# wns349/tensorflow-yolo

Measured on AMD Instinct MI355X. Metric: images/sec at 1/2/4/8 MI355X + post-NMS box-set match vs CPU ref, higher is better.
Workload: dtype f16; 1 GPU; v3-608-b32-fp16; network=v3, batch_per_gpu=32, global_batch=32, weights=seeded synthetic Darknet stream (random-init), streams=1

## Files before the change

include/yolo_hip.h:

```cpp
#ifndef YOLO_HIP_H
#define YOLO_HIP_H

#include <stddef.h>
#include <stdint.h>

#ifdef __cplusplus
extern "C" {
#endif

#define YOLO_HIP_ABI_VERSION 7

enum yolo_status {
    YOLO_OK = 0,
    YOLO_ERR_ARG = 1,
    YOLO_ERR_PLAN = 2,
    YOLO_ERR_HIP = 3,
    YOLO_ERR_WEIGHTS = 4,
    YOLO_ERR_STATE = 5,
    YOLO_ERR_OVERFLOW = 6
};

enum yolo_op {
    YOLO_OP_INPUT = 0,
    YOLO_OP_CONV = 1,
    YOLO_OP_MAXPOOL = 2,
    YOLO_OP_ROUTE = 3,
    YOLO_OP_REORG = 4,
    YOLO_OP_SHORTCUT = 5,
    YOLO_OP_UPSAMPLE = 6,
    YOLO_OP_YOLO = 7,
    YOLO_OP_DETECTION = 8
};

enum yolo_dtype { YOLO_DTYPE_F32 = 0, YOLO_DTYPE_F16 = 1, YOLO_DTYPE_MXF8 = 2 };

enum yolo_nms_mode {
    YOLO_NMS_AGNOSTIC = 0,
    YOLO_NMS_PER_CLASS = 1
};

#define YOLO_MAX_SRC 4
#define YOLO_MAX_ANCHORS 8
#define YOLO_MAX_SCALES 4

typedef struct yolo_layer_desc {
    int32_t op;
    int32_t n_src;
    int32_t src[YOLO_MAX_SRC];
    int32_t filters, ksize, stride;
    int32_t batch_norm;
    int32_t leaky;
    int32_t h, w, c;
    int32_t n_anchors;
    double anchors[2 * YOLO_MAX_ANCHORS];
} yolo_layer_desc;

typedef struct yolo_net_options {
    int32_t dtype;
    int32_t max_batch;
    int32_t keep_all;
    int32_t cand_capacity;
    int32_t max_boxes;
    int32_t streams;
    int32_t force_tile;
    int32_t guard_bytes;
    int32_t f32_products;
} yolo_net_options;

typedef struct yolo_box {
    float x, y, w, h;
    float prob;
    int32_t class_idx;
} yolo_box;

typedef struct yolo_head_desc {
    int32_t version;
    int32_t n_classes;
    int32_t n_scales;
    int32_t h[YOLO_MAX_SCALES], w[YOLO_MAX_SCALES], n_anchors[YOLO_MAX_SCALES];
    double anchors[YOLO_MAX_SCALES][2 * YOLO_MAX_ANCHORS];
} yolo_head_desc;

typedef struct yolo_net yolo_net;

int yolo_hip_abi_version(void);
const char *yolo_last_error(void);

int yolo_net_create(const yolo_layer_desc *layers, int n_layers, const yolo_net_options *opt, yolo_net **out);
void yolo_net_destroy(yolo_net *net);

size_t yolo_net_weight_count(const yolo_net *net);
size_t yolo_net_weights_bytes(const yolo_net *net);
size_t yolo_net_workspace_bytes(const yolo_net *net);
size_t yolo_net_output_count(const yolo_net *net);
double yolo_net_flops_per_image(const yolo_net *net);
int yolo_net_head_desc(const yolo_net *net, yolo_head_desc *out);
int yolo_net_set_head(yolo_net *net, const yolo_head_desc *head);
int yolo_net_num_kernels(const yolo_net *net);
int yolo_net_num_streams(const yolo_net *net);
int yolo_net_tune_streams(yolo_net *net, const float *in_dev, int batch, void *stream);
int yolo_net_set_streams(yolo_net *net, int parts);
typedef struct yolo_ws_region {
    char name[32];
    uint64_t offset, used_bytes, region_bytes;
} yolo_ws_region;
int yolo_net_workspace_regions(const yolo_net *net, yolo_ws_region *out, int cap);
size_t yolo_net_describe(const yolo_net *net, char *buf, size_t cap);

int yolo_net_load_weights(yolo_net *net, const float *host_weights, size_t n, void *dev_weights, size_t dev_bytes);
int yolo_net_bind_workspace(yolo_net *net, void *dev_workspace, size_t dev_bytes);

int yolo_net_forward(yolo_net *net, const float *in_dev, int batch, float *out_dev, void *stream);

int yolo_net_forward_u8(yolo_net *net, const uint8_t *in_dev, int batch, float *out_dev, void *stream);
int yolo_net_tune_streams_u8(yolo_net *net, const uint8_t *in_dev, int batch, void *stream);
int yolo_u8_unit_table(float *out256);

struct yolo_launch_caps {
    int32_t tap_stream_workgroups, stem_workgroups, first_mfma_workgroups, aux_work_items, decode_rows;
};
int yolo_launch_caps(struct yolo_launch_caps *out);

int yolo_net_autotune(yolo_net *net, const float *in_dev, int batch, void *stream);

int yolo_net_detect(yolo_net *net, const float *in_dev, int batch, double threshold, double iou_threshold,
                    int nms_mode, yolo_box *boxes_dev, int32_t *counts_dev, int32_t *status_dev, void *stream);

int yolo_net_detect_u8(yolo_net *net, const uint8_t *in_dev, int batch, double threshold, double iou_threshold,
                       int nms_mode, yolo_box *boxes_dev, int32_t *counts_dev, int32_t *status_dev, void *stream);

typedef struct yolo_kernel_info {
    int32_t kind;
    int32_t layer;
    int32_t variant;
    int32_t ksize, stride, cin, cout, out_h, out_w;
    double flops;
    double bytes;
    double weight_bytes;
    char name[64];
    char symbol[160];
} yolo_kernel_info;
int yolo_net_kernel_info(const yolo_net *net, int kernel, yolo_kernel_info *out);

int yolo_net_forward_timed(yolo_net *net, const float *in_dev, int batch, float *out_dev, void *stream, float *ms_host);

int yolo_net_forward_timed_u8(yolo_net *net, const uint8_t *in_dev, int batch, float *out_dev, void *stream, float *ms_host);

int yolo_net_read_layer(yolo_net *net, int layer, int batch, float *host_out, size_t n);

int yolo_mx_quantize(const void *src_f16_dev, int rows, int channels, uint8_t *q_dev, uint8_t *scale_dev, void *stream);
int yolo_mx_quantize_host(const float *src, int rows, int channels, uint8_t *q, uint8_t *scale);

size_t yolo_decode_scratch_bytes(const yolo_head_desc *head, int batch, int cand_capacity);
int yolo_decode_nms(const yolo_head_desc *head, const float *logits_dev, int batch, double threshold,
                    double iou_threshold, int nms_mode, int cand_capacity, int max_boxes, void *scratch_dev,
                    size_t scratch_bytes, yolo_box *boxes_dev, int32_t *counts_dev, int32_t *status_dev,
                    void *stream);

int yolo_preprocess_resize(const uint8_t *src_dev, int src_h, int src_w, int src_row_bytes, float *dst_dev, int dst_h, int dst_w,
                           int swap_rb, void *stream);

int yolo_preprocess_resize_u8(const uint8_t *src_dev, int src_h, int src_w, int src_row_bytes, uint8_t *dst_dev, int dst_h, int dst_w,
                              int swap_rb, void *stream);

typedef struct yolo_frame {
    const uint8_t *pixels_dev;
    int32_t h, w, row_bytes, swap_rb;
} yolo_frame;

enum yolo_resize_mode {
    YOLO_RESIZE_STRETCH = 0,
    YOLO_RESIZE_LETTERBOX = 1
};

int yolo_letterbox_geometry(int src_h, int src_w, int dst_h, int dst_w, int mode, int32_t *new_h, int32_t *new_w, int32_t *off_y,
                            int32_t *off_x);

int yolo_preprocess_frames_u8(const yolo_frame *frames_host, int n, int mode, uint8_t *dst_dev, int dst_h, int dst_w, void *stream);
int yolo_preprocess_frames(const yolo_frame *frames_host, int n, int mode, float *dst_dev, int dst_h, int dst_w, void *stream);

int yolo_boxes_to_frames(yolo_box *boxes_dev, const int32_t *counts_dev, int batch, int max_boxes, const yolo_frame *frames_host, int mode,
                         int net_h, int net_w, void *stream);

int yolo_net_detect_frames_u8(yolo_net *net, const yolo_frame *frames_host, int batch, int mode, uint8_t *batch_dev, double threshold,
                              double iou_threshold, int nms_mode, yolo_box *boxes_dev, int32_t *counts_dev, int32_t *status_dev,
                              void *stream);

typedef struct yolo_gt {
    float x, y, w, h;
    int32_t class_idx;
    int32_t difficult;
} yolo_gt;

enum yolo_eval_verdict { YOLO_EVAL_FP = 0, YOLO_EVAL_TP = 1, YOLO_EVAL_IGNORED = 2 };

enum yolo_eval_status {
    YOLO_EVAL_OVERFLOW = 1,
    YOLO_EVAL_UNSORTED = 2,
    YOLO_EVAL_BAD_CLASS = 4,
    YOLO_EVAL_BAD_COUNT = 8
};

#define YOLO_EVAL_MAX_GT 1024
#define YOLO_EVAL_MAX_DET_CAPACITY (1 << 20)
#define YOLO_EVAL_MAX_CLASSES 65536

typedef struct yolo_eval_desc {
    int32_t n_classes;
    int32_t det_capacity;
    int32_t max_gt;
    int32_t pad_;
    double match_iou;
} yolo_eval_desc;

typedef struct yolo_eval_record {
    double best_iou;
    float prob;
    int32_t class_idx;
    uint32_t seq;
    int32_t verdict;
    int32_t best_gt;
    int32_t pad_;
} yolo_eval_record;

typedef struct yolo_eval_class {
    double ap_voc12, ap_voc07;
    int32_t n_gt, n_det, tp, fp, ignored, pad_;
} yolo_eval_class;

typedef struct yolo_eval_result {
    double map_voc12, map_voc07;
    int32_t n_records;
    int32_t status;
    int32_t n_classes, pad_;
} yolo_eval_result;

typedef struct yolo_eval_layout {
    uint64_t status_offset, n_gt_offset, records_offset, sorted_offset, ctp_offset, cfp_offset, total_bytes;
} yolo_eval_layout;

size_t yolo_eval_state_bytes(const yolo_eval_desc *desc);
size_t yolo_eval_result_bytes(const yolo_eval_desc *desc);
int yolo_eval_state_layout(const yolo_eval_desc *desc, yolo_eval_layout *out);
int yolo_eval_reset(const yolo_eval_desc *desc, void *state_dev, size_t state_bytes, void *stream);
int yolo_eval_add(const yolo_eval_desc *desc, void *state_dev, const yolo_box *boxes_dev, const int32_t *counts_dev, int batch, int max_boxes,
                  const yolo_gt *gt_dev, const int32_t *gt_counts_dev, int64_t image_base, void *stream);
int yolo_eval_finish(const yolo_eval_desc *desc, void *state_dev, void *result_dev, void *stream);

enum yolo_loss_status {
    YOLO_LOSS_OUT_OF_GRID = 1,
    YOLO_LOSS_BAD_BOX = 2,
    YOLO_LOSS_BAD_CLASS = 4,
    YOLO_LOSS_BAD_COUNT = 8
};

#define YOLO_LOSS_MAX_CELLS 4096

typedef struct yolo_loss_image {
    double xy, wh, obj, noobj, cls;
    int32_t n_assigned;
    int32_t n_truths;
    int32_t status;
    int32_t pad_;
} yolo_loss_image;

typedef struct yolo_loss_result {
    double loss, loss_xy, loss_wh, loss_obj, loss_noobj, loss_class;
    int32_t n_assigned, n_truths;
    int32_t status;
    int32_t pad_;
} yolo_loss_result;

int yolo_v2_loss(const yolo_head_desc *head, const float *logits_dev, int batch, const yolo_gt *gt_dev, const int32_t *gt_counts_dev,
                 int max_gt, yolo_loss_image *images_dev, int32_t *assign_dev, yolo_loss_result *result_dev, void *stream);
// ... 248 lines not shown
```

tensorflow-yolo_amd/_hip.py:

```python
import ctypes as C
import os

_HERE = os.path.dirname(os.path.abspath(__file__))
LIB_PATH = os.environ.get("YOLO_HIP_LIB") or os.path.join(_HERE, "libyolo_hip.so")

ABI_VERSION = 7

OP_INPUT, OP_CONV, OP_MAXPOOL, OP_ROUTE, OP_REORG, OP_SHORTCUT, OP_UPSAMPLE, OP_YOLO, OP_DETECTION = range(9)
DTYPE_F32, DTYPE_F16, DTYPE_MXF8 = 0, 1, 2
NMS_AGNOSTIC, NMS_PER_CLASS = 0, 1
RESIZE_STRETCH, RESIZE_LETTERBOX = 0, 1
RESIZE_MODES = {"stretch": RESIZE_STRETCH, "letterbox": RESIZE_LETTERBOX}
EVAL_FP, EVAL_TP, EVAL_IGNORED = 0, 1, 2
EVAL_OVERFLOW, EVAL_UNSORTED, EVAL_BAD_CLASS, EVAL_BAD_COUNT = 1, 2, 4, 8
EVAL_MAX_GT, EVAL_MAX_DET_CAPACITY, EVAL_MAX_CLASSES = 1024, 1 << 20, 65536
LOSS_OUT_OF_GRID, LOSS_BAD_BOX, LOSS_BAD_CLASS, LOSS_BAD_COUNT = 1, 2, 4, 8
LOSS_MAX_CELLS = 4096
ANCHOR_EUCLIDEAN, ANCHOR_IOU = 0, 1
ANCHOR_DISTANCES = {"euclidean": ANCHOR_EUCLIDEAN, "iou": ANCHOR_IOU}
ANCHOR_BAD_BOX, ANCHOR_EMPTY_CLUSTER, ANCHOR_DEGENERATE, ANCHOR_MAX_ITER = 1, 2, 4, 8
ANCHOR_MAX_K, ANCHOR_MAX_INIT, ANCHOR_MAX_N, ANCHOR_ITER_LIMIT = 32, 64, 1 << 22, 10000
FRAMES_PER_LAUNCH = 64
MAX_SRC, MAX_ANCHORS, MAX_SCALES = 4, 8, 4
DEFAULT_MAX_BOXES = 1024
# ... 63 lines not shown
class LossResult(C.Structure):
    _fields_ = [("loss", C.c_double), ("loss_xy", C.c_double), ("loss_wh", C.c_double), ("loss_obj", C.c_double), ("loss_noobj", C.c_double),
                ("loss_class", C.c_double), ("n_assigned", C.c_int32), ("n_truths", C.c_int32), ("status", C.c_int32), ("pad_", C.c_int32)]


class LaunchCaps(C.Structure):
    _fields_ = [("tap_stream_workgroups", C.c_int32), ("stem_workgroups", C.c_int32), ("first_mfma_workgroups", C.c_int32),
                ("aux_work_items", C.c_int32), ("decode_rows", C.c_int32)]


class WgradPlan(C.Structure):
    _fields_ = [("tile_cout", C.c_int32), ("tile_cin", C.c_int32), ("tile_positions", C.c_int32), ("tiles_cout", C.c_int32),
                ("tiles_cin", C.c_int32), ("positions_per_chunk", C.c_int32), ("n_chunks", C.c_int32), ("pad_", C.c_int32),
                ("scratch_bytes", C.c_uint64)]


class Conv3x3WgradPlan(C.Structure):
    _fields_ = [("tile_cout", C.c_int32), ("tile_cin", C.c_int32), ("tile_positions", C.c_int32), ("tiles_cout", C.c_int32),
                ("tiles_cin", C.c_int32), ("positions_per_chunk", C.c_int32), ("n_chunks", C.c_int32), ("halo_rows", C.c_int32),
                ("scratch_bytes", C.c_uint64)]


class Conv3x3WgradF16Plan(C.Structure):
    _fields_ = [("tile_cout", C.c_int32), ("tile_cin", C.c_int32), ("tile_positions", C.c_int32), ("tiles_cout", C.c_int32),
                ("tiles_cin", C.c_int32), ("positions_per_chunk", C.c_int32), ("n_chunks", C.c_int32), ("halo_rows", C.c_int32),
                ("db_groups", C.c_int32), ("db_positions", C.c_int32), ("record_offset", C.c_uint64), ("scratch_bytes", C.c_uint64)]


class TensorView(C.Structure):
    _fields_ = [("offset", C.c_uint64), ("image_stride", C.c_int64), ("ld", C.c_int32), ("coff", C.c_int32), ("dtype", C.c_int32),
                ("cin", C.c_int32), ("h", C.c_int32), ("w", C.c_int32)]


class HeadTrainLayout(C.Structure):
    _fields_ = [(n, C.c_uint64) for n in ("w_offset", "b_offset", "m_w_offset", "v_w_offset", "m_b_offset", "v_b_offset", "dw_offset",
                                          "db_offset", "grad_offset", "assign_offset", "images_offset", "scratch_offset", "scratch_bytes",
                                          "total_bytes")] + [("cin", C.c_int32), ("cout", C.c_int32)]


class TailTrainLayout(C.Structure):
    _fields_ = [(n, C.c_uint64) for n in ("w_offset", "b_offset", "m_w_offset", "v_w_offset", "m_b_offset", "v_b_offset", "dw_offset",
                                          "db_offset", "w3_offset", "beta_offset", "m_w3_offset", "v_w3_offset", "m_beta_offset",
                                          "v_beta_offset", "dw3_offset", "dbeta_offset", "scale64_offset", "scale32_offset", "mean_offset",
                                          "d_offset", "grad_offset", "assign_offset", "images_offset", "scratch_offset", "scratch_bytes",
                                          "total_bytes", "block_src", "head_src")] + [(n, C.c_int32) for n in ("cin", "cout", "cin3", "cout3")]


class HeadTrainV3Layout(C.Structure):
    _fields_ = ([("n_scales", C.c_int32), ("pad_", C.c_int32), ("cin", C.c_int32 * MAX_SCALES), ("cout", C.c_int32 * MAX_SCALES)] +
                [(n, C.c_uint64 * MAX_SCALES) for n in ("w_offset", "b_offset", "m_w_offset", "v_w_offset", "m_b_offset", "v_b_offset",
                                                        "dw_offset", "db_offset", "bias_src")] +
                [(n, C.c_uint64) for n in ("grad_offset", "assign_offset", "parts_offset", "images_offset", "scratch_offset",
                                           "scratch_bytes", "total_bytes")])


class BlocksTrainV3Layout(C.Structure):
    _fields_ = ([("n_scales", C.c_int32), ("pad_", C.c_int32)] + [(n, C.c_int32 * MAX_SCALES) for n in ("cin", "cout", "cin3", "cout3")] +
                [(n, C.c_uint64 * MAX_SCALES) for n in ("w_offset", "b_offset", "m_w_offset", "v_w_offset", "m_b_offset", "v_b_offset",
                                                        "dw_offset", "db_offset", "w3_offset", "beta_offset", "m_w3_offset", "v_w3_offset",
                                                        "m_beta_offset", "v_beta_offset", "dw3_offset", "dbeta_offset", "scale64_offset",
                                                        "scale32_offset", "mean_offset", "bias_src", "block_src")] +
                [(n, C.c_uint64) for n in ("d_offset", "grad_offset", "assign_offset", "parts_offset", "images_offset", "scratch_offset",
                                           "scratch_bytes", "total_bytes")])


class V3WgradPlan(C.Structure):
    _fields_ = ([(n, C.c_int32) for n in ("n_scales", "threads", "channels_per_thread", "min_chunk", "win_tile_cin", "win_tile_rows", "reduce_tile_chunks", "pad_")] +
                [(n, C.c_int32 * MAX_SCALES) for n in ("positions", "positions_per_chunk", "n_chunks", "threads_per_chunk", "obj_workgroups",
                                                       "win_workgroups")] +
                [(n, C.c_uint64 * MAX_SCALES) for n in ("slab_offset", "slab_bytes")] +
                [(n, C.c_uint64) for n in ("slot_offset", "slot_bytes", "scratch_bytes")])


class V3WgradView(C.Structure):
    _fields_ = [("x_dev", C.c_void_p), ("image_stride", C.c_int64), ("ld", C.c_int32), ("coff", C.c_int32), ("dtype", C.c_int32),
                ("cin", C.c_int32)]


class V3DgradPlan(C.Structure):
    _fields_ = [(n, C.c_int32) for n in ("threads", "channels_per_thread", "tile_cin", "tiles_cin", "threads_per_position",
                                         "positions_per_round", "rounds", "positions_per_workgroup", "workgroups", "loops", "positions",
                                         "lds_bytes")]


class AugmentImage(C.Structure):
    _fields_ = [("enabled", C.c_int32), ("flip_lr", C.c_int32), ("flip_ud", C.c_int32), ("radius", C.c_int32), ("taps", C.c_uint16 * 10),
                ("drop_thr", C.c_uint32), ("noise_q", C.c_int32 * 2), ("noise_loc", C.c_int32 * 2), ("tx", C.c_int32), ("key", C.c_uint32 * 2)]


class AnchorDesc(C.Structure):
    _fields_ = [("k", C.c_int32), ("n_init", C.c_int32), ("max_iter", C.c_int32), ("distance", C.c_int32), ("tolerate", C.c_double),
                ("seed", C.c_uint64)]


class AnchorPlan(C.Structure):
    _fields_ = [(n, C.c_int32) for n in ("chunk", "n_chunks", "period", "threads")] + \
               [(n, C.c_uint64) for n in ("prep_offset", "pick_offset", "state_offset", "q_offset", "label_offset", "label_stride",
                                          "sums_offset", "scratch_bytes", "header_offset", "restarts_offset", "best_offset", "result_bytes")]


class AnchorHeader(C.Structure):
    _fields_ = [("status", C.c_uint32)] + [(n, C.c_int32) for n in ("best_restart", "n_valid", "n_bad", "k", "n_init", "distance", "pad_")]


class AnchorRestart(C.Structure):
    _fields_ = [("n_iter", C.c_int32), ("status", C.c_uint32), ("inertia_q", C.c_uint64), ("iou_q", C.c_uint64),
                ("seeds", C.c_int32 * ANCHOR_MAX_K)]


class AnchorBest(C.Structure):
    _fields_ = [("centres", (C.c_double * 2) * ANCHOR_MAX_K), ("counts", C.c_int64 * ANCHOR_MAX_K), ("sum_q", (C.c_uint64 * 2) * ANCHOR_MAX_K),
                ("inertia_q", C.c_uint64), ("iou_q", C.c_uint64), ("inertia", C.c_double), ("avg_iou", C.c_double)]


class WsRegion(C.Structure):
    _fields_ = [("name", C.c_char * 32), ("offset", C.c_uint64), ("used_bytes", C.c_uint64), ("region_bytes", C.c_uint64)]


class KernelInfo(C.Structure):
    _fields_ = [("kind", C.c_int32), ("layer", C.c_int32), ("variant", C.c_int32), ("ksize", C.c_int32),
                ("stride", C.c_int32), ("cin", C.c_int32), ("cout", C.c_int32), ("out_h", C.c_int32), ("out_w", C.c_int32),
                ("flops", C.c_double), ("bytes", C.c_double), ("weight_bytes", C.c_double), ("name", C.c_char * 64),
                ("symbol", C.c_char * 160)]


SIGNATURES = {
    "yolo_hip_abi_version": (C.c_int, []),
    "yolo_last_error": (C.c_char_p, []),
    "yolo_net_create": (C.c_int, [C.POINTER(LayerDesc), C.c_int, C.POINTER(NetOptions), C.POINTER(C.c_void_p)]),
    "yolo_net_destroy": (None, [C.c_void_p]),
    "yolo_net_weight_count": (C.c_size_t, [C.c_void_p]),
    "yolo_net_weights_bytes": (C.c_size_t, [C.c_void_p]),
    "yolo_net_workspace_bytes": (C.c_size_t, [C.c_void_p]),
    "yolo_net_output_count": (C.c_size_t, [C.c_void_p]),
    "yolo_net_flops_per_image": (C.c_double, [C.c_void_p]),
    "yolo_net_head_desc": (C.c_int, [C.c_void_p, C.POINTER(HeadDesc)]),
    "yolo_net_set_head": (C.c_int, [C.c_void_p, C.POINTER(HeadDesc)]),
    "yolo_net_num_kernels": (C.c_int, [C.c_void_p]),
    "yolo_net_num_streams": (C.c_int, [C.c_void_p]),
    "yolo_net_describe": (C.c_size_t, [C.c_void_p, C.c_char_p, C.c_size_t]),
    "yolo_net_load_weights": (C.c_int, [C.c_void_p, C.c_void_p, C.c_size_t, C.c_void_p, C.c_size_t]),
    "yolo_net_bind_workspace": (C.c_int, [C.c_void_p, C.c_void_p, C.c_size_t]),
    "yolo_net_forward": (C.c_int, [C.c_void_p, C.c_void_p, C.c_int, C.c_void_p, C.c_void_p]),
    "yolo_net_detect": (C.c_int, [C.c_void_p, C.c_void_p, C.c_int, C.c_double, C.c_double, C.c_int,
                                  C.c_void_p, C.c_void_p, C.c_void_p, C.c_void_p]),
    "yolo_net_forward_u8": (C.c_int, [C.c_void_p, C.c_void_p, C.c_int, C.c_void_p, C.c_void_p]),
    "yolo_net_detect_u8": (C.c_int, [C.c_void_p, C.c_void_p, C.c_int, C.c_double, C.c_double, C.c_int,
                                     C.c_void_p, C.c_void_p, C.c_void_p, C.c_void_p]),
    "yolo_net_forward_timed_u8": (C.c_int, [C.c_void_p, C.c_void_p, C.c_int, C.c_void_p, C.c_void_p, C.c_void_p]),
    "yolo_net_tune_streams_u8": (C.c_int, [C.c_void_p, C.c_void_p, C.c_int, C.c_void_p]),
    "yolo_preprocess_resize_u8": (C.c_int, [C.c_void_p, C.c_int, C.c_int, C.c_int, C.c_void_p, C.c_int, C.c_int, C.c_int, C.c_void_p]),
    "yolo_u8_unit_table": (C.c_int, [C.c_void_p]),
    "yolo_launch_caps": (C.c_int, [C.POINTER(LaunchCaps)]),
    "yolo_net_autotune": (C.c_int, [C.c_void_p, C.c_void_p, C.c_int, C.c_void_p]),
    "yolo_net_tune_streams": (C.c_int, [C.c_void_p, C.c_void_p, C.c_int, C.c_void_p]),
    "yolo_net_set_streams": (C.c_int, [C.c_void_p, C.c_int]),
    "yolo_net_workspace_regions": (C.c_int, [C.c_void_p, C.POINTER(WsRegion), C.c_int]),
    "yolo_net_kernel_info": (C.c_int, [C.c_void_p, C.c_int, C.POINTER(KernelInfo)]),
    "yolo_net_forward_timed": (C.c_int, [C.c_void_p, C.c_void_p, C.c_int, C.c_void_p, C.c_void_p, C.c_void_p]),
    "yolo_net_read_layer": (C.c_int, [C.c_void_p, C.c_int, C.c_int, C.c_void_p, C.c_size_t]),
    "yolo_mx_quantize": (C.c_int, [C.c_void_p, C.c_int, C.c_int, C.c_void_p, C.c_void_p, C.c_void_p]),
    "yolo_mx_quantize_host": (C.c_int, [C.c_void_p, C.c_int, C.c_int, C.c_void_p, C.c_void_p]),
    "yolo_decode_scratch_bytes": (C.c_size_t, [C.POINTER(HeadDesc), C.c_int, C.c_int]),
    "yolo_decode_nms": (C.c_int, [C.POINTER(HeadDesc), C.c_void_p, C.c_int, C.c_double, C.c_double, C.c_int,
                                  C.c_int, C.c_int, C.c_void_p, C.c_size_t, C.c_void_p, C.c_void_p, C.c_void_p,
                                  C.c_void_p]),
    "yolo_preprocess_resize": (C.c_int, [C.c_void_p, C.c_int, C.c_int, C.c_int, C.c_void_p, C.c_int, C.c_int, C.c_int, C.c_void_p]),
    "yolo_letterbox_geometry": (C.c_int, [C.c_int, C.c_int, C.c_int, C.c_int, C.c_int, C.POINTER(C.c_int32), C.POINTER(C.c_int32),
                                          C.POINTER(C.c_int32), C.POINTER(C.c_int32)]),
    "yolo_preprocess_frames_u8": (C.c_int, [C.POINTER(Frame), C.c_int, C.c_int, C.c_void_p, C.c_int, C.c_int, C.c_void_p]),
    "yolo_preprocess_frames": (C.c_int, [C.POINTER(Frame), C.c_int, C.c_int, C.c_void_p, C.c_int, C.c_int, C.c_void_p]),
    "yolo_boxes_to_frames": (C.c_int, [C.c_void_p, C.c_void_p, C.c_int, C.c_int, C.POINTER(Frame), C.c_int, C.c_int, C.c_int, C.c_void_p]),
    "yolo_net_detect_frames_u8": (C.c_int, [C.c_void_p, C.POINTER(Frame), C.c_int, C.c_int, C.c_void_p, C.c_double, C.c_double, C.c_int,
                                            C.c_void_p, C.c_void_p, C.c_void_p, C.c_void_p]),
    "yolo_eval_state_bytes": (C.c_size_t, [C.POINTER(EvalDesc)]),
    "yolo_eval_result_bytes": (C.c_size_t, [C.POINTER(EvalDesc)]),
    "yolo_eval_state_layout": (C.c_int, [C.POINTER(EvalDesc), C.POINTER(EvalLayout)]),
    "yolo_eval_reset": (C.c_int, [C.POINTER(EvalDesc), C.c_void_p, C.c_size_t, C.c_void_p]),
    "yolo_eval_add": (C.c_int, [C.POINTER(EvalDesc), C.c_void_p, C.c_void_p, C.c_void_p, C.c_int, C.c_int, C.c_void_p, C.c_void_p,
                                C.c_int64, C.c_void_p]),
    "yolo_eval_finish": (C.c_int, [C.POINTER(EvalDesc), C.c_void_p, C.c_void_p, C.c_void_p]),
    "yolo_v2_loss": (C.c_int, [C.POINTER(HeadDesc), C.c_void_p, C.c_int, C.c_void_p, C.c_void_p, C.c_int, C.c_void_p, C.c_void_p, C.c_void_p,
                               C.c_void_p]),
    "yolo_net_loss": (C.c_int, [C.c_void_p, C.c_void_p, C.c_int, C.c_void_p, C.c_void_p, C.c_int, C.c_void_p, C.c_void_p, C.c_void_p,
                                C.c_void_p]),
    "yolo_net_loss_u8": (C.c_int, [C.c_void_p, C.c_void_p, C.c_int, C.c_void_p, C.c_void_p, C.c_int, C.c_void_p, C.c_void_p, C.c_void_p,
                                   C.c_void_p]),
    "yolo_loss_reduce": (C.c_int, [C.c_void_p, C.c_int, C.c_int, C.c_int, C.c_void_p, C.c_void_p]),
    "yolo_v2_loss_grad": (C.c_int, [C.POINTER(HeadDesc), C.c_void_p, C.c_int, C.c_void_p, C.c_void_p, C.c_int, C.c_void_p, C.c_void_p, C.c_void_p,
                                    C.c_void_p, C.c_void_p]),
    "yolo_v3_loss_rows": (C.c_int, [C.POINTER(HeadDesc), C.POINTER(C.c_int64), C.POINTER(C.c_int32)]),
    "yolo_v3_loss": (C.c_int, [C.POINTER(HeadDesc), C.c_void_p, C.c_int, C.c_void_p, C.c_void_p, C.c_int, C.c_double, C.c_void_p, C.c_void_p,
                               C.c_void_p, C.c_void_p, C.c_void_p]),
    "yolo_v3_loss_grad": (C.c_int, [C.POINTER(HeadDesc), C.c_void_p, C.c_int, C.c_void_p, C.c_void_p, C.c_int, C.c_double, C.c_void_p, C.c_void_p,
                                    C.c_void_p, C.c_void_p, C.c_void_p, C.c_void_p]),
    "yolo_net_loss_v3": (C.c_int, [C.c_void_p, C.c_void_p, C.c_int, C.c_void_p, C.c_void_p, C.c_int, C.c_double, C.c_void_p, C.c_void_p,
                                   C.c_void_p, C.c_void_p, C.c_void_p]),
    "yolo_net_loss_v3_u8": (C.c_int, [C.c_void_p, C.c_void_p, C.c_int, C.c_void_p, C.c_void_p, C.c_int, C.c_double, C.c_void_p, C.c_void_p,
                                      C.c_void_p, C.c_void_p, C.c_void_p]),
    "yolo_wgrad_plan": (C.c_int, [C.c_int64, C.c_int, C.c_int, C.c_int, C.POINTER(WgradPlan)]),
    "yolo_conv1x1_wgrad": (C.c_int, [C.c_void_p, C.c_int, C.c_int, C.c_int, C.c_int64, C.c_int, C.c_int, C.c_int, C.c_void_p, C.c_int,
                                     C.c_void_p, C.c_void_p, C.c_void_p, C.c_size_t, C.c_void_p]),
    "yolo_adam_step": (C.c_int, [C.c_void_p] * 8 + [C.c_int64, C.c_int64, C.c_float, C.c_float, C.c_float, C.c_float, C.c_void_p]),
    "yolo_net_head_input": (C.c_int, [C.c_void_p, C.POINTER(TensorView)]),
    "yolo_net_head_train_layout": (C.c_int, [C.c_void_p, C.POINTER(HeadTrainLayout)]),
    "yolo_net_head_train_bytes": (C.c_size_t, [C.c_void_p]),
    "yolo_net_head_train_init": (C.c_int, [C.c_void_p, C.c_void_p, C.c_size_t, C.c_void_p, C.c_void_p]),
    "yolo_net_head_train_read": (C.c_int, [C.c_void_p, C.c_void_p, C.c_void_p, C.c_void_p]),
    "yolo_net_train_head_step": (C.c_int, [C.c_void_p, C.c_void_p, C.c_int, C.c_void_p, C.c_void_p, C.c_int, C.c_void_p, C.c_float,
                                           C.c_void_p, C.c_void_p]),
    "yolo_net_train_head_step_u8": (C.c_int, [C.c_void_p, C.c_void_p, C.c_int, C.c_void_p, C.c_void_p, C.c_int, C.c_void_p, C.c_float,
                                              C.c_void_p, C.c_void_p]),
    "yolo_v3_head_wgrad_plan": (C.c_int, [C.POINTER(HeadDesc), C.POINTER(C.c_int32), C.c_int, C.c_int, C.POINTER(V3WgradPlan)]),
    "yolo_v3_head_wgrad": (C.c_int, [C.POINTER(HeadDesc), C.POINTER(V3WgradView), C.c_int, C.c_void_p, C.c_void_p, C.c_int,
                                     C.POINTER(C.c_void_p), C.POINTER(C.c_void_p), C.c_void_p, C.c_size_t, C.c_void_p]),
    "yolo_net_head_inputs_v3": (C.c_int, [C.c_void_p, C.POINTER(TensorView), C.POINTER(C.c_int32)]),
    "yolo_net_head_train_v3_layout": (C.c_int, [C.c_void_p, C.POINTER(HeadTrainV3Layout)]),
    "yolo_net_head_train_v3_bytes": (C.c_size_t, [C.c_void_p]),
    "yolo_net_head_train_v3_init": (C.c_int, [C.c_void_p, C.c_void_p, C.c_size_t, C.POINTER(C.c_void_p), C.POINTER(C.c_void_p)]),
    "yolo_net_head_train_v3_read": (C.c_int, [C.c_void_p, C.c_void_p, C.POINTER(C.c_void_p), C.POINTER(C.c_void_p)]),
    "yolo_net_train_head_step_v3": (C.c_int, [C.c_void_p, C.c_void_p, C.c_int, C.c_void_p, C.c_void_p, C.c_int, C.c_double, C.c_void_p,
                                              C.c_float, C.c_void_p, C.c_void_p]),
    "yolo_net_train_head_step_v3_u8": (C.c_int, [C.c_void_p, C.c_void_p, C.c_int, C.c_void_p, C.c_void_p, C.c_int, C.c_double, C.c_void_p,
                                                 C.c_float, C.c_void_p, C.c_void_p]),
    "yolo_conv1x1_dgrad": (C.c_int, [C.c_void_p, C.c_int, C.c_void_p, C.c_int, C.c_void_p, C.c_int, C.c_int, C.c_int, C.c_int64, C.c_int,
                                     C.c_int, C.c_float, C.c_void_p, C.c_void_p]),
    "yolo_conv3x3_wgrad_plan": (C.c_int, [C.c_int, C.c_int, C.c_int, C.c_int, C.c_int, C.c_int, C.POINTER(Conv3x3WgradPlan)]),
    "yolo_conv3x3_wgrad": (C.c_int, [C.c_void_p, C.c_int, C.c_int, C.c_int, C.c_int64, C.c_int, C.c_int, C.c_int, C.c_int, C.c_void_p,
                                     C.c_int, C.c_void_p, C.c_void_p, C.c_void_p, C.c_void_p, C.c_size_t, C.c_void_p]),
    "yolo_conv3x3_wgrad_f16_plan": (C.c_int, [C.c_int, C.c_int, C.c_int, C.c_int, C.c_int, C.POINTER(Conv3x3WgradF16Plan)]),
    "yolo_conv3x3_wgrad_f16": (C.c_int, [C.c_void_p, C.c_int, C.c_int, C.c_int, C.c_int64, C.c_int, C.c_int, C.c_int, C.c_int, C.c_void_p,
                                         C.c_int, C.c_void_p, C.c_void_p, C.c_void_p, C.c_void_p, C.c_size_t, C.c_void_p]),
    "yolo_net_train_wgrad_f16_bytes": (C.c_size_t, [C.c_void_p]),
    "yolo_net_train_set_wgrad_f16": (C.c_int, [C.c_void_p, C.c_void_p, C.c_size_t]),
    "yolo_net_tail_inputs": (C.c_int, [C.c_void_p, C.POINTER(TensorView), C.POINTER(TensorView)]),
    "yolo_net_tail_train_layout": (C.c_int, [C.c_void_p, C.POINTER(TailTrainLayout)]),
    "yolo_net_tail_train_bytes": (C.c_size_t, [C.c_void_p]),
    "yolo_net_tail_train_init": (C.c_int, [C.c_void_p, C.c_void_p, C.c_size_t, C.c_void_p, C.c_void_p, C.c_void_p]),
    "yolo_net_tail_train_read": (C.c_int, [C.c_void_p, C.c_void_p, C.c_void_p, C.c_void_p, C.c_void_p, C.c_void_p]),
    "yolo_net_train_tail_step": (C.c_int, [C.c_void_p, C.c_void_p, C.c_int, C.c_void_p, C.c_void_p, C.c_int, C.c_void_p, C.c_float,
                                           C.c_void_p, C.c_void_p]),
    "yolo_net_train_tail_step_u8": (C.c_int, [C.c_void_p, C.c_void_p, C.c_int, C.c_void_p, C.c_void_p, C.c_int, C.c_void_p, C.c_float,
                                              C.c_void_p, C.c_void_p]),
    "yolo_v3_head_dgrad_plan": (C.c_int, [C.POINTER(HeadDesc), C.c_int, C.c_int, C.c_int, C.POINTER(V3DgradPlan)]),
    "yolo_v3_head_dgrad": (C.c_int, [C.POINTER(HeadDesc), C.c_int, C.c_void_p, C.c_void_p, C.c_int, C.c_int, C.c_void_p, C.c_int, C.c_void_p,
                                     C.c_int, C.c_int, C.c_int, C.c_int64, C.c_float, C.c_void_p, C.c_void_p]),
    "yolo_net_block_inputs_v3": (C.c_int, [C.c_void_p, C.POINTER(TensorView), C.POINTER(TensorView), C.POINTER(C.c_int32)]),
    "yolo_net_blocks_train_v3_layout": (C.c_int, [C.c_void_p, C.POINTER(BlocksTrainV3Layout)]),
    "yolo_net_blocks_train_v3_bytes": (C.c_size_t, [C.c_void_p]),
    "yolo_net_blocks_train_v3_init": (C.c_int, [C.c_void_p, C.c_void_p, C.c_size_t, C.POINTER(C.c_void_p), C.POINTER(C.c_void_p),
                                                C.POINTER(C.c_void_p)]),
    "yolo_net_blocks_train_v3_read": (C.c_int, [C.c_void_p, C.c_void_p, C.POINTER(C.c_void_p), C.POINTER(C.c_void_p), C.POINTER(C.c_void_p),
                                                C.POINTER(C.c_void_p)]),
    "yolo_net_train_blocks_step_v3": (C.c_int, [C.c_void_p, C.c_void_p, C.c_int, C.c_void_p, C.c_void_p, C.c_int, C.c_double, C.c_void_p,
                                                C.c_float, C.c_void_p, C.c_void_p]),
    "yolo_net_train_blocks_step_v3_u8": (C.c_int, [C.c_void_p, C.c_void_p, C.c_int, C.c_void_p, C.c_void_p, C.c_int, C.c_double, C.c_void_p,
                                                   C.c_float, C.c_void_p, C.c_void_p]),
    "yolo_augment_check": (C.c_int, [C.POINTER(AugmentImage), C.c_int, C.c_int]),
    "yolo_augment_u8": (C.c_int, [C.c_void_p, C.c_void_p, C.c_int, C.c_int, C.c_int, C.POINTER(AugmentImage), C.c_void_p]),
    "yolo_augment_truths_host": (C.c_int, [C.c_void_p, C.c_int, C.POINTER(AugmentImage), C.c_int, C.c_int, C.c_void_p, C.POINTER(C.c_int32)]),
    "yolo_augment_tile": (C.c_int, [C.POINTER(C.c_int32), C.POINTER(C.c_int32), C.POINTER(C.c_int32)]),
    "yolo_anchor_plan": (C.c_int, [C.POINTER(AnchorDesc), C.c_int64, C.POINTER(AnchorPlan)]),
    "yolo_anchor_kmeans": (C.c_int, [C.POINTER(AnchorDesc), C.c_void_p, C.c_int64, C.c_void_p, C.c_void_p, C.c_size_t, C.c_void_p, C.c_size_t,
                                     C.c_void_p, C.c_void_p]),
    "yolo_nms_host": (C.c_int, [C.c_void_p, C.c_void_p, C.c_void_p, C.c_int, C.c_double, C.c_int,
                                C.c_void_p, C.POINTER(C.c_int32)]),
}

_lib = None


class YoloHipError(RuntimeError):
    """A libyolo_hip call returned a non-zero status (message from yolo_last_error)."""


def lib():
    global _lib
    if _lib is not None:
        return _lib
    if not os.path.exists(LIB_PATH):
        raise ImportError(
            "libyolo_hip.so not found at %s: the HIP extension is the only compute path of this package "
            "(no CPU fallback). Build it with `python __graft_entry__.py` or `make -C tensorflow-yolo_amd/csrc`."
            % LIB_PATH)
    import torch
    handle = C.CDLL(LIB_PATH)
    for name, (res, args) in SIGNATURES.items():
        fn = getattr(handle, name)
        fn.restype = res
        fn.argtypes = args
    v = handle.yolo_hip_abi_version()
    if v != ABI_VERSION:
        raise ImportError("libyolo_hip.so ABI version %d, binding expects %d: rebuild the library" % (v, ABI_VERSION))
    _lib = handle
    return _lib


def resize_mode(name):
    key = str(name).strip().lower()
    if key not in RESIZE_MODES:
        raise ValueError("resize must be stretch or letterbox, got %r" % (name,))
    return RESIZE_MODES[key]


def letterbox_geometry(src_h, src_w, dst_h, dst_w, mode):
    out = [C.c_int32() for _ in range(4)]
# ... 76 lines not shown
```

tensorflow-yolo_amd/csrc/api.cpp:

```cpp
#include <cstdio>
#include <cstring>
#include <new>

#include <cmath>
#include "yolo_internal.h"

using namespace yolo;

extern "C" {

int yolo_hip_abi_version(void) { return YOLO_HIP_ABI_VERSION; }

int yolo_mx_quantize(const void *src_f16_dev, int rows, int channels, uint8_t *q_dev, uint8_t *scale_dev, void *stream) {
    if (!src_f16_dev || !q_dev || !scale_dev || rows <= 0 || channels <= 0 || channels % 32)
        return fail(YOLO_ERR_ARG, "yolo_mx_quantize: null pointer, or rows / channels not positive, or channels not a multiple of 32");
    if ((uintptr_t)src_f16_dev % 16 || (uintptr_t)q_dev % 16)
        return fail(YOLO_ERR_ARG, "yolo_mx_quantize: source and element buffers must be 16-byte aligned");
    const hipError_t e = launch_mx_quantize(src_f16_dev, rows, channels, q_dev, scale_dev, reinterpret_cast<hipStream_t>(stream));
    if (e != hipSuccess) return fail(YOLO_ERR_HIP, std::string("yolo_mx_quantize: ") + hipGetErrorString(e));
    return YOLO_OK;
}
int yolo_mx_quantize_host(const float *src, int rows, int channels, uint8_t *q, uint8_t *scale) {
    if (!src || !q || !scale || rows <= 0 || channels <= 0 || channels % 32)
        return fail(YOLO_ERR_ARG, "yolo_mx_quantize_host: null pointer, or rows / channels not positive, or channels not a multiple of 32");
    const size_t blocks = (size_t)rows * (size_t)(channels / 32);
    for (size_t b = 0; b < blocks; ++b) scale[b] = mx_quant_block_host(src + 32 * b, q + 32 * b);
    return YOLO_OK;
}
const char *yolo_last_error(void) { return get_error(); }

int yolo_net_create(const yolo_layer_desc *layers, int n_layers, const yolo_net_options *opt, yolo_net **out) {
    if (!layers || !opt || !out || n_layers <= 0) return fail(YOLO_ERR_ARG, "yolo_net_create: null argument");
    if (opt->dtype != YOLO_DTYPE_F16 && opt->dtype != YOLO_DTYPE_F32 && opt->dtype != YOLO_DTYPE_MXF8)
        return fail(YOLO_ERR_ARG, "yolo_net_create: bad dtype");
    if (opt->max_batch <= 0) return fail(YOLO_ERR_ARG, "yolo_net_create: max_batch must be positive");
    yolo_net *net = new (std::nothrow) yolo_net();
    if (!net) return fail(YOLO_ERR_ARG, "out of host memory");
    net->opt = *opt;
    if (opt->dtype == YOLO_DTYPE_MXF8) {
        net->opt.dtype = YOLO_DTYPE_F16;
        net->mx = true;
    }
    if (net->opt.cand_capacity <= 0) net->opt.cand_capacity = 4096;
    if (net->opt.max_boxes <= 0) net->opt.max_boxes = 256;
    if (net->opt.cand_capacity > 65536) {
        delete net;
        return fail(YOLO_ERR_ARG, "cand_capacity above 65536 (16-bit sort indices)");
    }
    std::string err;
    int rc = YOLO_ERR_PLAN;
    try {
        rc = plan_network(net, layers, n_layers, err);
    } catch (const std::exception &e) {
        err = e.what();
    }
    if (rc != YOLO_OK) {
        delete net;
        return fail(rc, "yolo_net_create: " + err);
    }
    int n_mx = 0;
    for (Kernel &k : net->kernels) {
        k.mx = mx_eligible(net, k) ? 1 : 0;
        n_mx += k.mx;
    }
    if (net->opt.force_tile == kMxTile + 1 && (!net->mx || !n_mx)) {
        delete net;
        return fail(YOLO_ERR_ARG, "yolo_net_create: tile 24 (the MXFP8 3x3 kernel; yolo_net_options.force_tile = 25) needs dtype MXF8 and a "
                                  "3x3 / stride-1 conv with Cin % 128 == 0 and W <= 100");
    }
    if (net->opt.force_tile > 0 && net->opt.force_tile != kMxTile + 1)
        for (Kernel &k : net->kernels)
            if (conv_dispatched(k) && conv_tile_valid(net, k, net->opt.force_tile - 1)) k.tile = net->opt.force_tile - 1;
    net->splitk_bytes = splitk_slab_bytes(net) * (size_t)net->arenas;
    if (net->splitk_bytes) net->tail.push_back({"split-K tickets + slabs", net->splitk_off, net->splitk_bytes, net->splitk_bytes});
    net->workspace_bytes = net->splitk_off + net->splitk_bytes;
    *out = net;
    return YOLO_OK;
}

void yolo_net_destroy(yolo_net *net) {
    if (!net) return;
    destroy_streams(net);
    delete net;
}

size_t yolo_net_weight_count(const yolo_net *net) { return net ? net->weight_count : 0; }
size_t yolo_net_weights_bytes(const yolo_net *net) { return net ? net->weights_bytes : 0; }
size_t yolo_net_workspace_bytes(const yolo_net *net) { return net ? net->workspace_bytes : 0; }
size_t yolo_net_output_count(const yolo_net *net) { return net ? net->out_count : 0; }
double yolo_net_flops_per_image(const yolo_net *net) { return net ? net->flops_per_image : 0.0; }
int yolo_net_num_kernels(const yolo_net *net) { return net ? (int)net->kernels.size() : 0; }
int yolo_net_num_streams(const yolo_net *net) { return net ? net->parts : 0; }

int yolo_net_head_desc(const yolo_net *net, yolo_head_desc *out) {
    if (!net || !out) return fail(YOLO_ERR_ARG, "yolo_net_head_desc: null argument");
    *out = net->head;
    return YOLO_OK;
}

int yolo_net_set_head(yolo_net *net, const yolo_head_desc *head) {
    if (!net || !head) return fail(YOLO_ERR_ARG, "yolo_net_set_head: null argument");
    std::string err;
    int rc = check_head(head, net->out_count, err);
    if (rc) return fail(rc, "yolo_net_set_head: " + err);
    net->head = *head;
    return YOLO_OK;
}

int yolo_net_workspace_regions(const yolo_net *net, yolo_ws_region *out, int cap) {
    if (!net) return 0;
    int n = 0;
    auto add = [&](const std::string &name, size_t off, size_t used, size_t region) {
        if (out && n < cap) {
            memset(&out[n], 0, sizeof out[n]);
            snprintf(out[n].name, sizeof out[n].name, "%s", name.c_str());
            out[n].offset = off; out[n].used_bytes = used; out[n].region_bytes = region;
        }
        ++n;
    };
    for (int a = 0; a < net->arenas; ++a)
        for (size_t b = 0; b < net->buffers.size(); ++b) {
            const Buffer &B = net->buffers[b];
            if (!B.bytes) continue;
            add("tensor " + std::to_string(b) + " arena " + std::to_string(a), (size_t)a * net->arena_bytes + B.offset, B.used, B.bytes);
        }
    for (const WsRegion &r : net->tail) add(r.name, r.offset, r.used, r.bytes);
    return n;
}

size_t yolo_net_describe(const yolo_net *net, char *buf, size_t cap) {
    if (!net) return 0;
    std::string s = describe(net);
    if (buf && cap) {
        size_t n = s.size() < cap - 1 ? s.size() : cap - 1;
        memcpy(buf, s.data(), n);
        buf[n] = 0;
    }
    return s.size() + 1;
}

int yolo_net_load_weights(yolo_net *net, const float *host_weights, size_t n, void *dev_weights, size_t dev_bytes) {
    if (!net || !dev_weights || (!host_weights && n)) return fail(YOLO_ERR_ARG, "yolo_net_load_weights: null argument");
    if (dev_bytes < net->weights_bytes) return fail(YOLO_ERR_ARG, "yolo_net_load_weights: device buffer too small");
    if ((uintptr_t)dev_weights % 256) return fail(YOLO_ERR_ARG, "yolo_net_load_weights: device buffer must be 256-byte aligned");
    std::vector<unsigned char> blob;
    std::string err;
    int rc = pack_weights(net, host_weights, n, blob, err);
    if (rc) return fail(rc, "yolo_net_load_weights: " + err);
    HIP_TRY(hipMemcpy(dev_weights, blob.data(), blob.size(), hipMemcpyHostToDevice));
    net->dev_weights = static_cast<unsigned char *>(dev_weights);
    net->weights_loaded = true;
    return YOLO_OK;
}

int yolo_net_bind_workspace(yolo_net *net, void *ws, size_t bytes) {
    if (!net || !ws) return fail(YOLO_ERR_ARG, "yolo_net_bind_workspace: null argument");
    if (bytes < net->workspace_bytes) return fail(YOLO_ERR_ARG, "yolo_net_bind_workspace: workspace too small");
    if ((uintptr_t)ws % 256) return fail(YOLO_ERR_ARG, "yolo_net_bind_workspace: workspace must be 256-byte aligned");
    net->dev_ws = static_cast<unsigned char *>(ws);
    net->cand_clean = 0;
    net->dev_ws_bytes = bytes;
    return zero_pair_counters(net);
}

}

namespace yolo {

int check_head(const yolo_head_desc *h, size_t out_count, std::string &err) {
    if (h->version != 2 && h->version != 3) { err = "head version must be 2 or 3"; return YOLO_ERR_ARG; }
    if (h->n_scales < 1 || h->n_scales > YOLO_MAX_SCALES || h->n_classes < 1) { err = "bad head geometry"; return YOLO_ERR_ARG; }
    size_t rows = 0;
    for (int s = 0; s < h->n_scales; ++s) {
        if (h->n_anchors[s] < 1 || h->n_anchors[s] > YOLO_MAX_ANCHORS || h->h[s] < 1 || h->w[s] < 1) { err = "bad head scale"; return YOLO_ERR_ARG; }
        rows += (size_t)h->h[s] * h->w[s] * h->n_anchors[s];
    }
    if (out_count && rows * (5 + h->n_classes) != out_count) { err = "head geometry does not match the network output size"; return YOLO_ERR_ARG; }
    return YOLO_OK;
}

int check_ready(yolo_net *net, const void *in, int batch, const char *who) {
    if (!net || !in) return fail(YOLO_ERR_ARG, std::string(who) + ": null argument");
    if (batch <= 0 || batch > net->opt.max_batch) return fail(YOLO_ERR_ARG, std::string(who) + ": batch outside 1..max_batch");
    if (!net->weights_loaded && net->weight_count) return fail(YOLO_ERR_STATE, std::string(who) + ": weights not loaded");
    if (!net->dev_ws) return fail(YOLO_ERR_STATE, std::string(who) + ": workspace not bound");
    return YOLO_OK;
}

int check_loss_args(const yolo_head_desc *head, const void *gt_dev, const void *gt_counts_dev, int max_gt, const void *images_dev,
                    const void *result_dev, const char *who) {
    if (!head || !gt_dev || !gt_counts_dev || !images_dev || !result_dev) return fail(YOLO_ERR_ARG, std::string(who) + ": null argument");
    if (max_gt < 1 || max_gt > YOLO_EVAL_MAX_GT) return fail(YOLO_ERR_ARG, std::string(who) + ": max_gt must be 1.." + std::to_string(YOLO_EVAL_MAX_GT));
    if (head->version != 2 || head->n_scales != 1)
        return fail(YOLO_ERR_ARG, std::string(who) + ": the head must be version 2 with one scale (the reference has a loss for YOLOv2 only)");
    std::string err;
    int rc = check_head(head, 0, err);
    if (rc) return fail(rc, std::string(who) + ": " + err);
    if ((long long)head->h[0] * head->w[0] > YOLO_LOSS_MAX_CELLS)
        return fail(YOLO_ERR_ARG, std::string(who) + ": h * w must be at most " + std::to_string(YOLO_LOSS_MAX_CELLS));
    return YOLO_OK;
}

static int run_loss(const yolo_head_desc &h, const float *logits, int batch, const yolo_gt *gt, const int32_t *gt_counts, int max_gt,
                    yolo_loss_image *images, int32_t *assign, yolo_loss_result *result, hipStream_t s) {
    LossParams p;
    memset(&p, 0, sizeof p);
    p.logits = logits; p.gt = gt; p.gt_counts = gt_counts; p.max_gt = max_gt;
    p.h = h.h[0]; p.w = h.w[0]; p.na = h.n_anchors[0]; p.n_classes = h.n_classes;
    for (int a = 0; a < p.na; ++a) {
        p.aw[a] = h.anchors[0][2 * a]; p.ah[a] = h.anchors[0][2 * a + 1];
        p.awf[a] = (float)p.aw[a]; p.ahf[a] = (float)p.ah[a];
    }
    p.images = images; p.assign = assign;
    HIP_TRY(launch_loss_images(p, batch, s));
    HIP_TRY(launch_loss_finish(LossFinishParams{images, batch, 0, batch, result}, s));
    return YOLO_OK;
}

int run_loss_grad(const yolo_head_desc &h, const float *logits, int batch, const yolo_gt *gt, const int32_t *gt_counts, int max_gt,
                  yolo_loss_image *images, int32_t *assign, yolo_loss_result *result, float *grad, hipStream_t s) {
    int rc = run_loss(h, logits, batch, gt, gt_counts, max_gt, images, assign, result, s);
    if (rc) return rc;
    LossGradParams p;
    memset(&p, 0, sizeof p);
    p.logits = logits; p.gt = gt; p.assign = assign; p.grad = grad; p.batch = batch; p.max_gt = max_gt;
    p.h = h.h[0]; p.w = h.w[0]; p.na = h.n_anchors[0]; p.n_classes = h.n_classes;
    for (int a = 0; a < p.na; ++a) { p.awf[a] = (float)h.anchors[0][2 * a]; p.ahf[a] = (float)h.anchors[0][2 * a + 1]; }
    HIP_TRY(launch_loss_grad(p, s));
    return YOLO_OK;
}

int run_loss3(const Loss3Geometry &geo, const float *logits, int batch, const yolo_gt *gt, const int32_t *gt_counts, int max_gt,
              double ignore_thresh, yolo_loss_image *parts, yolo_loss_image *images, int32_t *assign, yolo_loss_result *result, float *grad,
              hipStream_t s) {
    Loss3Params p;
    memset(&p, 0, sizeof p);
    p.logits = logits; p.gt = gt; p.gt_counts = gt_counts; p.batch = batch; p.max_gt = max_gt; p.ignore_thresh = ignore_thresh; p.geo = geo;
    p.parts = parts; p.images = images; p.assign = assign; p.result = result; p.grad = grad;
    HIP_TRY(launch_loss3(p, s));
    if (grad) HIP_TRY(launch_loss3_grad(p, s));
    return YOLO_OK;
}

}

namespace {

void fill_decode(const yolo_head_desc &h, DecodeParams &dp) {
    dp.version = h.version;
    dp.n_classes = h.n_classes;
    dp.n_scales = h.n_scales;
    int row0 = 0;
    for (int s = 0; s < h.n_scales; ++s) {
        dp.sc[s].row0 = row0; dp.sc[s].h = h.h[s]; dp.sc[s].w = h.w[s]; dp.sc[s].na = h.n_anchors[s];
        for (int a = 0; a < h.n_anchors[s]; ++a) { dp.sc[s].aw[a] = h.anchors[s][2 * a]; dp.sc[s].ah[a] = h.anchors[s][2 * a + 1]; }
        row0 += h.h[s] * h.w[s] * h.n_anchors[s];
    }
    dp.rows = row0;
}

int run_decode_nms(const yolo_head_desc &h, const float *logits, int batch, double thr, double iou, int mode, int cap,
                   int max_boxes, unsigned char *cand, int *cand_count, yolo_box *boxes, int32_t *counts, int32_t *status,
                   int32_t *keep_idx, hipStream_t s, unsigned char *nms_scratch = nullptr, const float *obj = nullptr, int *counters_clean = nullptr) {
    DecodeParams dp;
    memset(&dp, 0, sizeof dp);
    fill_decode(h, dp);
    dp.logits = logits;
    dp.obj = obj;
    dp.threshold = (float)thr;
    dp.cap = cap;
    dp.cand = cand;
    dp.cand_count = cand_count;
    dp.total_rows = (long long)batch * dp.rows;
    const int clean_n = counters_clean ? *counters_clean : 0;
    const bool need_clear = batch > clean_n;
    if (counters_clean) *counters_clean = 0;
    HIP_TRY(launch_decode(dp, batch, s, need_clear));
    NmsParams np;
    np.cand = reinterpret_cast<const Candidate *>(cand);
    np.cand_count = cand_count;
    np.cap = cap; np.max_boxes = max_boxes; np.mode = mode;
    np.iou_threshold = iou;
    np.boxes = boxes; np.counts = counts; np.status = status; np.keep_idx = keep_idx;
    np.scratch = nms_scratch; np.scratch_stride = nms_scratch_bytes(cap);
    np.reset_count = counters_clean ? cand_count : nullptr;
    HIP_TRY(launch_nms(np, batch, s));
    if (counters_clean) *counters_clean = need_clear ? batch : clean_n;
    return YOLO_OK;
}

}

extern "C" {

static int forward_any(yolo_net *net, const NetIn in, int batch, float *out_dev, void *stream, const char *who) {
    int rc = check_ready(net, in.ptr, batch, who);
    if (rc) return rc;
    if (!out_dev) return fail(YOLO_ERR_ARG, std::string(who) + ": null output");
    return run_forward(net, in, batch, out_dev, static_cast<hipStream_t>(stream));
}
int yolo_net_forward(yolo_net *net, const float *in_dev, int batch, float *out_dev, void *stream) {
    return forward_any(net, NetIn{in_dev, false}, batch, out_dev, stream, "yolo_net_forward");
}
int yolo_net_forward_u8(yolo_net *net, const uint8_t *in_dev, int batch, float *out_dev, void *stream) {
    return forward_any(net, NetIn{in_dev, true}, batch, out_dev, stream, "yolo_net_forward_u8");
}

static int forward_timed_any(yolo_net *net, const NetIn in_dev, int batch, float *out_dev, void *stream, float *ms_host, const char *who) {
    int rc = check_ready(net, in_dev.ptr, batch, who);
    if (rc) return rc;
    if (!out_dev || !ms_host) return fail(YOLO_ERR_ARG, std::string(who) + ": null output");
    return run_forward_timed(net, in_dev, batch, out_dev, static_cast<hipStream_t>(stream), ms_host);
}
int yolo_net_forward_timed(yolo_net *net, const float *in_dev, int batch, float *out_dev, void *stream, float *ms_host) {
    return forward_timed_any(net, NetIn{in_dev, false}, batch, out_dev, stream, ms_host, "yolo_net_forward_timed");
// ... 629 lines not shown
```

tensorflow-yolo_amd/csrc/conv_dispatch.cpp:

```cpp
#include <cstdio>
#include <cstdlib>
#include <cstring>

#include "conv_tiles.h"
#include "yolo_internal.h"

namespace yolo {

static void conv_vec_flags(const yolo_net *net, const Kernel &k, bool out_f32, int &vec_out, int &vec_res) {
    const int epc = net->epc;
    const int ch = k.cfg == CFG_N32 ? 8 : 16;
    const int oepc = out_f32 ? 4 : epc;
    vec_out = (k.cout % ch == 0) && view_chunk_aligned(k.out, oepc);
    vec_res = k.has_res && (k.cout % ch == 0) && view_chunk_aligned(k.in2, epc);
}

void conv_shape_params(const yolo_net *net, const Kernel &k, int batch, ConvParams &p) {
    memset(&p, 0, sizeof p);
    const yolo_layer_desc &d = net->layers[k.src_layer].d;
    p.H = k.in.H; p.W = k.in.W; p.in_ld = k.in.ld; p.in_coff = k.in.coff; p.in_img_stride = k.in.img_stride;
    p.Ho = net->layers[k.src_layer].H; p.Wo = net->layers[k.src_layer].W; p.HoWo = p.Ho * p.Wo;
    p.M = (int)((long long)batch * p.HoWo);
    p.Cout = k.cout;
    p.out_ld = k.out.ld;
    p.out_img_stride = k.out.img_stride;
    p.f32 = net->opt.dtype == YOLO_DTYPE_F32;
    p.out_f32 = k.out.f32 || p.f32;
    {
        const long long ob = (long long)batch * k.out.img_stride * (p.out_f32 ? 4 : net->esize);
        p.out_bytes = ob > 0 && ob <= 0x7ffffff0LL ? (uint32_t)ob : 0u;
    }
    p.wgt_bytes = (uint32_t)k.w_bytes;
    p.ksize = d.ksize; p.stride = d.stride; p.pad = (d.ksize - 1) / 2; p.taps = d.ksize * d.ksize;
    p.ktiles = k.ktiles;
    p.tiles_per_tap = k.perchunk ? 1 : k.cpt / 8;
    p.cin_chunks = k.cpt;
    p.cpt_shift = k.cpt == 1 ? 0 : k.cpt == 2 ? 1 : 2;
    p.wrow_bytes = (uint32_t)k.ktiles * 128;
    p.leaky = k.leaky; p.outmode = k.outmode; p.has_res = k.has_res;
    conv_vec_flags(net, k, p.out_f32 != 0, p.vec_out, p.vec_res);
    if (k.has_res) {
        p.res_ld = k.in2.ld;
        p.res_img_stride = k.in2.img_stride;
        const long long rb = (long long)batch * k.in2.img_stride * net->esize;
        p.res_bytes = rb > 0 && rb <= 0x7ffffff0LL ? (uint32_t)rb : 0u;
    }
}

bool dma_eligible(const yolo_net *net, const Kernel &k) {
    if (k.cpt % 4) return false;
    return net->opt.dtype == YOLO_DTYPE_F16 || (k.ksize == 3 && k.stride == 1);
}
bool conv_tile_valid(const yolo_net *net, const Kernel &k, int tile) {
    if (tile < 0 || tile >= kNumTiles) return false;
    const ConvTile &t = conv_tile(tile);
    if (k.outmode == OUT_POOL2 && !t.has(CAP_POOL)) return false;
    if (tile == TILE_4WAVE) return true;
    if (net->opt.dtype == YOLO_DTYPE_F32 && !t.f32_ok()) return false;
    if (t.image_aligned() && k.in.H != k.in.W) return false;
    if (t.stride2() && ((k.in.H & 1) || net->opt.dtype != YOLO_DTYPE_F16)) return false;
    return dma_eligible(net, k) && dma_cfg_valid(tile, k.cout, k.cpt, true, k.ksize, k.stride, k.in.W);
}

namespace {

long long tap_blocks(const ConvParams &p, int tile) {
    const ConvTile &t = conv_tile(tile);
    const long long images = p.M / p.HoWo, mq = images * (p.H + 1) * (p.W + 1);
    return (t.image_aligned() ? images : (mq + t.nb() - 1) / t.nb()) * ((p.Cout + t.na() - 1) / t.na());
}
size_t pair_slab_bytes(int tile, long long tiles, int ks) { return (size_t)tiles * (size_t)ks * 128 * (size_t)conv_tile(tile).nb() * 4; }
size_t reduce_slab_bytes(const ConvParams &p, long long ks) { return (size_t)ks * (size_t)p.M * (size_t)((p.Cout + 127) / 128 * 128) * 4; }

int choose_ksplit(const Kernel &k, const ConvParams &p, int tile, size_t slab_bytes, int &ku) {
    ku = 0;
    if (!slab_bytes || p.M <= 0) return 1;
    long long blocks;
    int units, min_units;
    if (tile == TILE_4WAVE) {
        const int na = k.cfg == CFG_N128 ? 128 : k.cfg == CFG_N64 ? 64 : 32, nb = k.cfg == CFG_N128 ? 128 : 256;
        blocks = ((long long)p.M + nb - 1) / nb * ((p.Cout + na - 1) / na);
        units = p.ktiles;
        min_units = 2;
    } else if (conv_tile(tile).has(CAP_SPLITK)) {
        blocks = tap_blocks(p, tile);
        units = p.cin_chunks >> 2;
        min_units = 2;
    } else {
        return 1;
    }
    if (blocks > 128 || units < 2 * min_units) return 1;
    const long long kmax = units / min_units < 32 ? units / min_units : 32;
    long long ks = 512 / blocks;
    if (ks > kmax) ks = 256 / blocks;
    if (ks > kmax) ks = kmax;
    const size_t wbytes = (size_t)p.Cout * (size_t)p.taps * (size_t)p.cin_chunks * 16;
    const size_t small_cap = (size_t)(p.taps == 1 ? 24 : (p.f32 || units >= 8) ? 16 : 8) << 20;
    while (ks >= 2 && (reduce_slab_bytes(p, ks) > slab_bytes || reduce_slab_bytes(p, ks) > (2 * wbytes > small_cap ? 2 * wbytes : small_cap))) --ks;
    if (ks < 2) return 1;
    ku = (int)((units + ks - 1) / ks);
    return (units + ku - 1) / ku;
}

}

ConvLaunch resolve_conv(const yolo_net *net, size_t ki, const ConvParams &p, int tile_req, size_t slab_bytes) {
    const Kernel &k = net->kernels[ki];
    int tile = tile_req;
    if (!dma_eligible(net, k) || (tile > 0 && !conv_tile_valid(net, k, tile))) tile = 0;
    else if (tile < 0) {
        tile = choose_dma_cfg(p.M, k.cout, k.cpt, p.taps, k.has_res, true, k.stride, k.in.W, net->opt.dtype == YOLO_DTYPE_F32);
        auto or_else = [&](int a, int b) { return conv_tile_valid(net, k, a) ? a : b; };
        if (tile == TILE_TAPIMG_128x384 && !conv_tile_valid(net, k, tile)) tile = or_else(TILE_TAP_256x224, TILE_TAP_128x256);
        if (tile == TILE_TAPIMG_128x192 && !conv_tile_valid(net, k, tile)) tile = or_else(TILE_TAP_128x192, TILE_TAP_128x256);
        if ((tile == TILE_TAPS2_128x256 || tile == TILE_TAPS2IMG_128x384) && !conv_tile_valid(net, k, tile)) tile = or_else(TILE_TAPS2_128x256, or_else(TILE_DMA_256x128_K32, TILE_4WAVE));
        if (tile == TILE_TAPS2_128x256_WIDE && !conv_tile_valid(net, k, tile)) tile = or_else(TILE_DMA_128x256_K32, TILE_4WAVE);
    }
    ConvLaunch r{tile, 1, 0, 0, 0, 0};
    const bool tap_by_rule = conv_tile(tile).is_tap() && tile_req <= 0;
    const int units = p.cin_chunks >> 2;
    static const bool no_pair = getenv("YOLO_NO_PAIR_SPLIT") != nullptr;
    const bool pair_ok = tap_by_rule && !no_pair && units >= 8 && p.HoWo > 0;
    auto pair_on = [&](int t, long long lo, long long hi) {
        if (!pair_ok || !conv_tile_valid(net, k, t)) return false;
        const long long tiles = tap_blocks(p, t);
        if (tiles < lo || tiles > hi || pair_slab_bytes(t, tiles, 2) > slab_bytes) return false;
        r.tile = t; r.ks = 2; r.ku = (units + 1) / 2; r.pair = 1;
        return true;
    };
    const bool wide_pair = !p.f32 && (pair_on(TILE_TAPIMG_128x192, 64, 128) || pair_on(TILE_TAP_128x256, 64, 128));
    if (!wide_pair) {
        r.ks = choose_ksplit(k, p, tile, slab_bytes, r.ku);
        if (r.ks <= 1 && tap_by_rule && tile != TILE_TAP_128x128 && conv_tile_valid(net, k, TILE_TAP_128x128)) {
            int ku11 = 0;
            const int ks11 = choose_ksplit(k, p, TILE_TAP_128x128, slab_bytes, ku11);
            if (ks11 > 1) { r.tile = TILE_TAP_128x128; r.ks = ks11; r.ku = ku11; }
        }
        if (r.ks <= 1) pair_on(TILE_TAP_128x128, 129, 256);
        static const bool no_inl = getenv("YOLO_NO_INLAUNCH_SPLITK") != nullptr;
        if (r.ks > 1 && r.ks <= 8 && !r.pair && r.tile == TILE_TAP_128x128 && !no_inl) {
            const long long tiles = tap_blocks(p, r.tile);
            if (tiles * 128 <= (long long)kPairCounterBytes && pair_slab_bytes(r.tile, tiles, r.ks) <= slab_bytes) r.pair = 1;
        }
    }
    if (r.pair) r.slab_need = pair_slab_bytes(r.tile, tap_blocks(p, r.tile), r.ks);
    else if (r.ks > 1) r.slab_need = reduce_slab_bytes(p, r.ks);
    const ConvTile &rt = conv_tile(r.tile);
    if (k.fuse2_next && ki + 1 < net->kernels.size() && net->kernels[ki + 1].fuse2_prev && rt.has(CAP_FUSE2) &&
        r.ks <= 1 && conv_fast_epilogue_ok(p) && rt.has(CAP_FUSE2_RES) == (p.has_res != 0) && p.HoWo > 0) {
        const long long ob = (long long)(p.M / p.HoWo) * net->kernels[ki + 1].out.img_stride * net->esize;
        r.fuse2 = ob > 0 && ob <= 0x7ffffff0LL;
    }
    return r;
}

size_t splitk_slab_bytes(const yolo_net *net) {
    const int per = net->arena_full ? net->opt.max_batch : (net->opt.max_batch + net->arenas - 1) / net->arenas;
    size_t need = 0;
    for (size_t ki = 0; ki < net->kernels.size(); ++ki) {
        const Kernel &k = net->kernels[ki];
        if (!conv_dispatched(k)) continue;
        for (int b = 1; b <= per; ++b) {
            ConvParams p;
            conv_shape_params(net, k, b, p);
            const size_t bytes = resolve_conv(net, ki, p, k.tile, kSplitkSlabMax).slab_need;
            if (bytes > need) need = bytes;
        }
    }
    return need ? kPairCounterBytes + (need + 4095) / 4096 * 4096 : 0;
}

bool pass_splits_k(const yolo_net *net, int batch) {
    for (size_t ki = 0; ki < net->kernels.size(); ++ki) {
        const Kernel &k = net->kernels[ki];
        if (!conv_dispatched(k)) continue;
        ConvParams p;
        conv_shape_params(net, k, batch, p);
        if (resolve_conv(net, ki, p, k.tile, arena_slab_data_bytes(net)).ks > 1) return true;
    }
    return false;
}

void conv_kernel_info(const yolo_net *net, int kernel, yolo_kernel_info *out) {
    const Kernel &k = net->kernels[kernel];
    const char *t = dtype_tag(net);
    const LayerInfo &li = net->layers[k.src_layer];
    out->variant = k.cfg + 4 * k.perchunk;
    out->ksize = k.ksize; out->stride = k.stride; out->cin = k.cin; out->cout = k.cout; out->out_h = li.H; out->out_w = li.W;
    out->flops = 2.0 * li.H * li.W * k.cout * k.ksize * k.ksize * k.cin;
    out->bytes = (double)k.in.H * k.in.W * k.cin * net->esize + view_elems(k.out) * view_esz(net, k.out) + (k.has_res ? view_elems(k.in2) * net->esize : 0.0);
    out->weight_bytes = (double)k.cout * k.ksize * k.ksize * k.cin * net->esize + 4.0 * k.cout;
    if (k.stem == STEM_TAIL) {
        out->flops = 0; out->bytes = 0; out->weight_bytes = 0;
        snprintf(out->name, sizeof out->name, "conv_igemm<fused into conv_stem>");
        return;
    }
    if (k.stem == STEM_HOST) {
        const Kernel &f = net->kernels[kernel - 1];
        out->flops += 2.0 * f.out.H * f.out.W * f.cout * 27;
        out->bytes = (double)f.in.H * f.in.W * 3 * 4 + view_elems(k.out) * view_esz(net, k.out);
        out->weight_bytes += 28.0 * f.cout * 4;
        snprintf(out->name, sizeof out->name, "conv_stem<f16,3-32-64>");
        set_symbol(out, "yolo::stem_v3_kernel(yolo::StemParams)");
        if (kernel + 1 < (int)net->kernels.size() && net->kernels[kernel + 1].stem == STEM_TAIL) {
            const Kernel &t3 = net->kernels[kernel + 1];
            out->flops += 2.0 * li.H * li.W * t3.cout * t3.cin;
            out->bytes += view_elems(t3.out) * view_esz(net, t3.out);
            out->weight_bytes += (double)t3.cout * t3.cin * net->esize + 4.0 * t3.cout;
            snprintf(out->name, sizeof out->name, "conv_stem<f16,3-32-64-32>");
        }
        return;
    }
    if (k.mx) {
        ConvParams mp;
        conv_shape_params(net, k, part_batch(net), mp);
        out->variant = 8 + kMxTile;
        out->weight_bytes = (double)k.cout * k.ksize * k.ksize * k.cin * (1.0 + 1.0 / 32) + 4.0 * k.cout;
        snprintf(out->name, sizeof out->name, "conv_mx<mxf8,128x256>");
        set_symbol(out, conv_mx_symbol(conv_fast_epilogue_ok(mp)));
        return;
    }
    ConvParams sp;
    const int per_arena = part_batch(net);
    if (k.fuse2_prev && kernel > 0) {
        conv_shape_params(net, net->kernels[kernel - 1], per_arena, sp);
        if (resolve_conv(net, (size_t)kernel - 1, sp, net->kernels[kernel - 1].tile, arena_slab_data_bytes(net)).fuse2) {
            out->flops = 0; out->bytes = 0; out->weight_bytes = 0;
            snprintf(out->name, sizeof out->name, "conv_igemm<fused into the conv in front>");
            return;
        }
    }
    conv_shape_params(net, k, per_arena, sp);
    const ConvLaunch pk = resolve_conv(net, (size_t)kernel, sp, k.tile, arena_slab_data_bytes(net));
    const bool fused2 = pk.fuse2 != 0;
    if (fused2) {
        const Kernel &b2 = net->kernels[kernel + 1];
        out->flops += 2.0 * li.H * li.W * b2.cout * b2.cin;
        out->bytes += view_elems(b2.out) * view_esz(net, b2.out);
        out->weight_bytes += (double)b2.cout * b2.cin * net->esize + 4.0 * b2.cout;
    }
    const int tile = pk.tile;
    if (tile > 0) {
        out->variant = 8 + tile;
        snprintf(out->name, sizeof out->name, "conv_igemm_dma<%s,%s>", t, conv_tile(tile).name);
        sp.ksplit = pk.ks; sp.pair = pk.pair; sp.fuse2 = pk.fuse2;
        set_symbol(out, conv_tile_symbol(tile, sp));
    } else {
        const bool emu = conv_f32_emu_rule(net->opt.f32_products, net->opt.dtype, sp, k.cfg, k.perchunk != 0, pk.ks);
        set_symbol(out, conv_symbol(net->opt.dtype, k.cfg, k.perchunk != 0, emu));
        if (emu) snprintf(out->name, sizeof out->name, "conv_igemm_emu<f32 as 9 x bf16,N128>");
        else snprintf(out->name, sizeof out->name, "conv_igemm<%s,N%d,%s>", t, k.cfg == CFG_N128 ? 128 : k.cfg == CFG_N64 ? 64 : 32,
                      k.perchunk ? "perchunk" : "uniform");
    }
    const double part_bytes = (double)pk.ks * (double)li.H * li.W * ((k.cout + 127) / 128 * 128) * 4.0;
    std::string tags;
    if (k.outmode == OUT_POOL2) tags += "+pool";
    if (fused2) tags += "+1x1";
    if (pk.pair) {
        tags += pk.ks == 2 ? "+pairK" : "+splitK" + std::to_string(pk.ks) + ",1launch";
        out->bytes += part_bytes;
    } else if (pk.ks > 1) {
        tags += "+splitK" + std::to_string(pk.ks);
        out->bytes += 2.0 * part_bytes;
    }
    const size_t n = strlen(out->name);
    snprintf(out->name + n, sizeof out->name - n, "%s", tags.c_str());
}

}
```

tensorflow-yolo_amd/csrc/conv_tap.hip:

```cpp
#include "conv_common.h"
#include "conv_tiles.h"
#include <cstdio>
#include <type_traits>
#include <utility>

#ifndef YOLO_TAP_ASM_MFMA
#define YOLO_TAP_ASM_MFMA 1
#endif
#ifndef YOLO_TAP_W_FIRST
#define YOLO_TAP_W_FIRST 1
#endif
#ifndef YOLO_TAP_AH_ALL
#define YOLO_TAP_AH_ALL 1
#endif
#ifndef YOLO_TAP_PIL_RECOMPUTE
#define YOLO_TAP_PIL_RECOMPUTE 0
#endif
#ifndef YOLO_TAP_PIL
#define YOLO_TAP_PIL 1
#endif
#ifndef YOLO_TAP_DBG
#define YOLO_TAP_DBG 0
#endif
#ifndef YOLO_TAP_RECOMPUTE_ADDR
#define YOLO_TAP_RECOMPUTE_ADDR 1
#endif
#ifndef YOLO_TAP_LATE_FROM
#define YOLO_TAP_LATE_FROM 4
#endif
#ifndef YOLO_TAP_STAGGER
#define YOLO_TAP_STAGGER 1
#endif

namespace yolo {

namespace {

typedef __attribute__((address_space(3))) void tap_lds_void;

__device__ __forceinline__ void tap_dma16(__amdgpu_buffer_rsrc_t rsrc, unsigned char *lds_dst, uint32_t voff, uint32_t soff) {
#if defined(__HIP_DEVICE_COMPILE__)
    __builtin_amdgcn_raw_ptr_buffer_load_lds(rsrc, (tap_lds_void *)lds_dst, 16, voff, soff, 0, 0);
#else
    (void)rsrc; (void)lds_dst; (void)voff; (void)soff;
#endif
}

template <typename T>
__device__ __forceinline__ void tap_mfma(float4v &acc, const uint4v &a, const uint4v &b) {
#if YOLO_TAP_ASM_MFMA && defined(__HIP_DEVICE_COMPILE__)
    if constexpr (sizeof(T) == 2) {
        asm volatile("v_mfma_f32_16x16x32_f16 %0, %1, %2, %0" : "+v"(acc) : "v"(a), "v"(b));
        return;
    }
#endif
    acc = mma_chunk<T>(a, b, acc);
}

template <int TM, int TP>
__device__ __forceinline__ void tap_mfma_drain(float4v (&acc)[TM][TP]) {
#if YOLO_TAP_ASM_MFMA && defined(__HIP_DEVICE_COMPILE__)
    asm volatile("s_nop 15\n\ts_nop 15" : "+v"(acc[0][0]));
#pragma unroll
    for (int a = 0; a < TM; ++a)
#pragma unroll
        for (int b = 0; b < TP; ++b) asm volatile("" : "+v"(acc[a][b]));
#endif
}

template <int N>
__device__ __forceinline__ void tap_wait_vm() {
    asm volatile("s_waitcnt vmcnt(%0)" ::"n"(N) : "memory");
}

__device__ __forceinline__ int tap_swz_w(int r) { return (0x78 >> (2 * ((r >> 2) & 3))) & 3; }

constexpr int kTapStreamBiasFloats = 512;

}

template <bool F32, int WM, int WN, int TM, int TP, int PRG, int OCC, int MODE, bool SPLITK, bool FAST = false, bool FUSE2 = false>
__global__ void __launch_bounds__(WM * WN * 64, OCC) conv3x3_tap_kernel(const ConvParams p) {
    typedef typename std::conditional<F32, float, _Float16>::type T;
    constexpr bool TWO_D = MODE == 2 || MODE == 3;
    constexpr bool S2 = MODE == 4;
    constexpr int PADQ = TWO_D ? 2 : 1;
    constexpr int NW = WM * WN;
    constexpr int S = 3;
    constexpr bool STAG = YOLO_TAP_STAGGER != 0 && !F32 && !SPLITK && TM % 2 == 0 && NW == 8 && MODE == 4 && OCC == 4;
    constexpr int TMH = TM / 2;
    constexpr bool PIL = YOLO_TAP_PIL != 0 && MODE == 1 && !F32;
    constexpr int PL = (PRG * 16) / TP;
    constexpr int ROWB = 64;
    constexpr int NA = WM * TM * 16;
    constexpr int NB = WN * TP * 16;
    constexpr int JA_TOT = NA / 16;
    constexpr int JA = (JA_TOT + NW - 1) / NW;
    constexpr int PW = (TWO_D && OCC >= 6) ? 18 : 24;
    constexpr int FROW = TWO_D ? PW : 16;
    constexpr int JP = (PRG + NW - 1) / NW;
    constexpr int CH = 4 * TM;
    constexpr int A_BYTES = NA * ROWB;
    constexpr int P_BYTES = PRG * 1024;
    static_assert(NW == 8, "eight waves");
    static_assert(JA_TOT % NW == 0 || JA_TOT < NW, "weight tile must split evenly over the waves (or be smaller than them)");
    static_assert(!TWO_D || PRG * 16 >= (NB / 16 + 2) * PW, "patch buffer too small for the 2-D tile");
    if constexpr (F32 && (TP > 2 || OCC >= 6)) return;
    if constexpr (SPLITK && !(WM == 2 && WN == 4 && TM == 4 && (TP == 2 || ((TP == 4 || TP == 3) && !F32)) && MODE == 1)) return;
    if constexpr (MODE == 3 && (TP % 2 != 0 || SPLITK)) return;
    static_assert(!FAST || (!F32 && !SPLITK && MODE != 3), "the lean epilogue: fp16, whole K, plain output");
    static_assert(!S2 || JA_TOT % NW == 0, "stride 2: every wave carries weights");
    if constexpr (S2 && (F32 || SPLITK)) return;
    static_assert(!FUSE2 || (FAST && WM == 2 && WN == 4 && TM == 4 && TP == 4), "back-to-back 1x1: the 128 x 256 tiles (eight waves)");
    constexpr int LDS_BYTES = FUSE2 && kFuse2LdsBytes > S * A_BYTES + 2 * P_BYTES ? kFuse2LdsBytes : S * A_BYTES + 2 * P_BYTES;
    __shared__ __attribute__((aligned(16))) unsigned char smem[LDS_BYTES];
    unsigned char *const smemP = smem + S * A_BYTES;

    const int tid = threadIdx.x;
#ifdef YOLO_EXPERIMENT
    const unsigned long long t_start = p.trace ? wall_clock64() : 0ull;
    const unsigned long long c_start = p.trace ? (unsigned long long)clock64() : 0ull;
    if ((p.dbg & 64) && ((__builtin_amdgcn_s_getreg(0xF804) >> 16) & 1u)) __builtin_amdgcn_s_setprio(3);
    if ((p.dbg >> 8) > 0 && ((__builtin_amdgcn_s_getreg(0xF804) >> 16) & 1u)) {
        const unsigned long long until = wall_clock64() + (unsigned long long)(p.dbg >> 8) * 25ull;
        while (wall_clock64() < until) __builtin_amdgcn_s_sleep(4);
    }
#endif
    const int lane = tid & 63;
    const int wave = __builtin_amdgcn_readfirstlane(tid >> 6);
    const int wm = wave / WN, wn = wave % WN;

    const int bid = xcd_remap(blockIdx.x, p.n_blocks);
    const int mt = (int)fdiv((uint32_t)bid, p.dtiles_n);
    const int nt = bid - mt * p.n_tiles_n;
    const int n0 = nt * NA;
    const int q0 = mt * p.q_stride;
    const bool has_a = JA_TOT % NW == 0 || wave < JA_TOT;

    const __amdgpu_buffer_rsrc_t rs_in = __builtin_amdgcn_make_buffer_rsrc(const_cast<void *>(p.in), 0, p.in_bytes, 0x00020000);
    const __amdgpu_buffer_rsrc_t rs_w = __builtin_amdgcn_make_buffer_rsrc(const_cast<void *>(p.wgt), 0, p.wgt_bytes, 0x00020000);

    const int lrow = lane >> 2;
    uint32_t a_off[JA];
#pragma unroll
    for (int j = 0; j < JA; ++j) {
        const int r = (j * NW + wave) * 16 + lrow;
        const int ws = r / (TM * 16), R = r % (TM * 16);
        const int tm = R >> 4, g4 = (R >> 2) & 3, jj = R & 3;
        const int ch = ws * (TM * 16) + g4 * CH + 4 * tm + jj;
        a_off[j] = (uint32_t)(n0 + ch) * p.wrow_bytes + (uint32_t)(((lane & 3) ^ tap_swz_w(lrow)) << 4);
    }
    const int c_begin = SPLITK ? (int)blockIdx.y * p.kunits : 0;
    const int C = SPLITK ? ((c_begin + p.kunits < (p.cin_chunks >> 2)) ? c_begin + p.kunits : (p.cin_chunks >> 2)) : (p.cin_chunks >> 2);
    const int KT = 9 * C;
    auto issue_weights = [&](int tap, int c, int slot) {
        const uint32_t ka = (uint32_t)(tap * p.cin_chunks + 4 * c) * 16;
        if (has_a) {
#pragma unroll
            for (int j = 0; j < JA; ++j) tap_dma16(rs_w, smem + slot * A_BYTES + (j * NW + wave) * 1024, a_off[j], ka);
        }
    };
    constexpr bool W_FIRST = YOLO_TAP_W_FIRST != 0 && YOLO_TAP_PIL != 0 && MODE == 1 && !F32;
    if constexpr (W_FIRST) {
        issue_weights(0, c_begin, 0);
        issue_weights(1, c_begin, 1);
        __builtin_amdgcn_sched_barrier(0);
    }
    constexpr int JP_FULL = PRG - (JP - 1) * NW;
    const bool jp_full = wave < JP_FULL;
    uint32_t b_off[JP];
    const uint32_t csw_p = (uint32_t)(((lane & 3) ^ (((lrow >> 2) & 1) << 1)) << 4);
    int t2_n = 0, t2_y0 = 0, t2_x0 = 0;
    if (TWO_D) {
        t2_n = (int)fdiv((uint32_t)mt, p.dqHW);
        const int r = mt - t2_n * p.qHW;
        const int ty = (int)fdiv((uint32_t)r, p.dqW);
        t2_y0 = ty * (NB / 16);
        t2_x0 = (r - ty * p.qW) * 16;
    }
#pragma unroll
    for (int j = 0; j < JP; ++j) {
        const int g = j * NW + wave;
        bool ok;
        int n, y, x;
        if (TWO_D) {
            const int R = g * 16 + lrow;
            const int pr = R / PW, pc = R - pr * PW;
            n = t2_n; y = t2_y0 - 1 + pr; x = t2_x0 - 1 + pc;
            ok = g < PRG && pc < 18 && pr < NB / 16 + 2 && t2_n * p.HoWo < p.M && (unsigned)y < (unsigned)p.H && (unsigned)x < (unsigned)p.W;
        } else {
            int Rp = g * 16 + lrow;
            bool in_planes = true;
            if constexpr (PIL) {
                const int plane = Rp / PL, idx = Rp - plane * PL;
                in_planes = plane < TP;
                Rp = idx * TP + plane;
            }
            const int q = q0 - (p.qW + 1) + Rp;
            ok = g < PRG && in_planes && q >= 0 && q < p.Mq;
            const int qq = ok ? q : 0;
            n = (int)fdiv((uint32_t)qq, p.dqHW);
            const int r = qq - n * p.qHW;
            y = (int)fdiv((uint32_t)r, p.dqW);
            x = r - y * p.qW;
            if (S2) { ok = ok && x < p.Wo && y < p.Ho; y *= 2; x *= 2; }
            else ok = ok && x < p.W && y < p.H;
        }
        const long long e = (long long)n * p.in_img_stride + ((long long)y * p.W + x) * p.in_ld + p.in_coff;
        b_off[j] = ok ? (uint32_t)(e * (long long)sizeof(T)) + csw_p : YOLO_INVALID_OFF;
    }

    auto issue_patch = [&](int c, int buf, uint32_t plane_off = 0u) {
        const uint32_t koff = (uint32_t)c * ROWB + plane_off;
#pragma unroll
        for (int j = 0; j < JP; ++j)
            if (j + 1 < JP || jp_full) tap_dma16(rs_in, smemP + buf * P_BYTES + (j * NW + wave) * 1024, b_off[j], koff);
    };

    float4v acc[TM][TP];
    float4v acc2[F32 ? TM : 1][F32 ? TP : 1];
    const int fr = lane & 15, fq = lane >> 4;
    auto init_acc = [&]() {
        if constexpr (SPLITK) {
            if ((TP != 2 || p.pair) && blockIdx.y == 0) {
                conv_init_acc_bias<TM, TP>(p, acc, n0 + wm * (TM * 16) + fq * CH);
            } else {
#pragma unroll
                for (int a = 0; a < TM; ++a)
#pragma unroll
                    for (int b = 0; b < TP; ++b) acc[a][b] = float4v{0.f, 0.f, 0.f, 0.f};
            }
        } else {
            conv_init_acc_bias<TM, TP>(p, acc, n0 + wm * (TM * 16) + fq * CH);
        }
    };
    if constexpr (!STAG) init_acc();
    if constexpr (F32) {
#pragma unroll
        for (int a = 0; a < TM; ++a)
#pragma unroll
            for (int b = 0; b < TP; ++b) acc2[F32 ? a : 0][F32 ? b : 0] = float4v{0.f, 0.f, 0.f, 0.f};
    }

    const int a_frag = (wm * TM * 16 + fr) * ROWB + (((fq ^ tap_swz_w(fr)) & 3) << 4);
    const int rb = wn * TP * FROW + fr;

    auto compute = [&](int slot, int buf, int shift) {
        const unsigned char *A = smem + slot * A_BYTES + a_frag;
        if constexpr (!TWO_D && YOLO_TAP_RECOMPUTE_ADDR && STAG) asm volatile("" : "+s"(shift));
        const int R = rb + shift;
        const unsigned char *B = smemP + buf * P_BYTES + (R << 6) + ((fq << 4) ^ ((R & 4) << 3));
        uint4v fa[TM], fb[TP];
        if constexpr ((YOLO_TAP_DBG & 64) != 0) {
#pragma unroll
            for (int a = 0; a < TM; ++a) asm volatile("" : "=v"(fa[a]));
#pragma unroll
            for (int b = 0; b < TP; ++b) asm volatile("" : "=v"(fb[b]));
        } else {
#pragma unroll
        for (int a = 0; a < TM; ++a) {
            if constexpr ((YOLO_TAP_DBG & 128) != 0) { if (a == TM - 1) { asm volatile("" : "=v"(fa[a])); continue; } }
            fa[a] = *reinterpret_cast<const uint4v *>(A + a * 16 * ROWB);
        }
#pragma unroll
        for (int b = 0; b < TP; ++b) {
            if constexpr ((YOLO_TAP_DBG & 128) != 0) { if (b == TP - 1) { asm volatile("" : "=v"(fb[b])); continue; } }
            if constexpr (TWO_D && (FROW & 7) != 0) {
                const int Rb = R + b * FROW;
// ... 150 lines not shown
            if constexpr (!((YOLO_TAP_DBG & 16) != 0 || ((YOLO_TAP_DBG & 8) != 0 && tap % 3 != 0))) __builtin_amdgcn_s_barrier();
            auto issue_dma = [&]() {
                {
                    const int t2 = tap + 2 < 9 ? tap + 2 : tap + 2 - 9;
                    const int c2 = tap + 2 < 9 ? c : c + 1;
                    if (c2 < C) issue_weights(t2, c2, (tap + 2) % S);
                }
                if (tap == 0 && more) issue_patch(c + 1, buf ^ 1);
            };
            const int kh = tap / 3, kw = tap - 3 * kh;
            if constexpr (PIL && !LATE) compute_pil(tap % S, buf, kh, kw, tap == 8 ? buf ^ 1 : buf, issue_dma);
            else {
                issue_dma();
                if constexpr (LATE) compute_late(tap % S, buf, TWO_D ? kh * PW + kw : kh * p.qW + kw);
                else compute(tap % S, buf, TWO_D ? kh * PW + kw : kh * p.qW + kw);
            }
        }
    };
    if constexpr (PIL) {
        if (has_a && !W_FIRST) tap_wait_vm<2 * JA>(); else tap_wait_vm<0>();
        __builtin_amdgcn_s_barrier();
#pragma unroll
        for (int b = 0; b < TP; ++b) G[b] = *reinterpret_cast<const uint4v *>(g_ptr(0, wn * (TP * 16) + b));
        __builtin_amdgcn_sched_barrier(0);
    }
    auto run_all = [&](auto latec) {
        if constexpr (STAG) init_acc();
        if constexpr (decltype(latec)::value) {
#pragma unroll
            for (int a = 0; a < TMH; ++a) ha[a] = uint4v{0u, 0u, 0u, 0u};
#pragma unroll
            for (int b = 0; b < TP; ++b) hb[b] = uint4v{0u, 0u, 0u, 0u};
        }
        for (int c = c_begin; c < C; c += 2) {
            if constexpr (S2) {
                run_slice_s2(c, std::integral_constant<int, 0>(), latec);
                if (c + 1 < C) run_slice_s2(c + 1, std::integral_constant<int, 1>(), latec);
            } else {
                run_slice(c, std::integral_constant<int, 0>(), latec);
                if (c + 1 < C) run_slice(c + 1, std::integral_constant<int, 1>(), latec);
            }
            if constexpr (F32) flush_acc<TM, TP>(acc, acc2);
        }
    };
    if constexpr (STAG) {
        if (late) {
            run_all(std::true_type());
            late_finish();
        } else {
            run_all(std::false_type());
        }
    } else {
        run_all(std::false_type());
    }
    if constexpr (!F32) tap_mfma_drain<TM, TP>(acc);
    if constexpr (F32) {
#pragma unroll
        for (int a = 0; a < TM; ++a)
#pragma unroll
            for (int b = 0; b < TP; ++b) acc[a][b] = acc2[a][b];
    }
    (void)KT;
#ifdef YOLO_EXPERIMENT
    const unsigned long long t_loop = p.trace ? wall_clock64() : 0ull;
#endif
    if constexpr (SPLITK) {
        if constexpr (TP == 2) {
            if (!p.pair) {
                conv_store_partial<TM, TP, PADQ, PIL>(p, acc, n0 + wm * (TM * 16) + fq * CH, q0 + wn * (TP * 16), fr, (int)blockIdx.y);
                return;
            }
        }
        constexpr uint32_t SLAB = (uint32_t)NA * NB * 4;
        const __amdgpu_buffer_rsrc_t rs_part = __builtin_amdgcn_make_buffer_rsrc(p.part, 0, p.part_bytes, 0x00020000);
        const uint32_t nsplit = gridDim.y;
        const uint32_t mine = ((uint32_t)blockIdx.x * nsplit + blockIdx.y) * SLAB, other = ((uint32_t)blockIdx.x * nsplit + (1u - blockIdx.y)) * SLAB;
        typedef __attribute__((__vector_size__(4 * sizeof(unsigned int)))) unsigned int u4;
#pragma unroll
        for (int a = 0; a < TM; ++a)
#pragma unroll
            for (int b = 0; b < TP; ++b)
                __builtin_amdgcn_raw_buffer_store_b128(__builtin_bit_cast(u4, acc[a][b]), rs_part,
                                                       mine + (uint32_t)((((wave * TM + a) * TP + b) * 64 + lane) * 16), 0, 16 );
        asm volatile("s_waitcnt vmcnt(0)" ::: "memory");
        __syncthreads();
        int *const flag = reinterpret_cast<int *>(smem);
        if (tid == 0) {
            int *const ticket = p.pair_cnt + (size_t)blockIdx.x * kCandCountStride;
            const int t = __hip_atomic_fetch_add(ticket, 1, __ATOMIC_RELAXED, __HIP_MEMORY_SCOPE_AGENT);
            if (t == (int)nsplit - 1) {
                __hip_atomic_store(ticket, 0, __ATOMIC_RELAXED, __HIP_MEMORY_SCOPE_AGENT);
                __builtin_amdgcn_fence(__ATOMIC_ACQUIRE, "agent");
                asm volatile("s_waitcnt vmcnt(0)" ::: "memory");
            }
            *flag = t;
        }
        __syncthreads();
        if (*flag != (int)nsplit - 1) return;
        if (nsplit > 2) {
#pragma unroll
            for (int a = 0; a < TM; ++a)
#pragma unroll
                for (int b = 0; b < TP; ++b) acc[a][b] = float4v{0.f, 0.f, 0.f, 0.f};
            for (uint32_t sp = 0; sp < nsplit; ++sp) {
                const uint32_t base = ((uint32_t)blockIdx.x * nsplit + sp) * SLAB;
#pragma unroll
                for (int a = 0; a < TM; ++a) {
                    u4 v[TP];
#pragma unroll
                    for (int b = 0; b < TP; ++b)
                        v[b] = __builtin_amdgcn_raw_buffer_load_b128(rs_part, base + (uint32_t)((((wave * TM + a) * TP + b) * 64 + lane) * 16), 0, 16 );
#pragma unroll
                    for (int b = 0; b < TP; ++b) acc[a][b] += __builtin_bit_cast(float4v, v[b]);
                }
            }
            conv_epilogue<T, TM, TP, PADQ, true, PIL>(p, acc, n0 + wm * (TM * 16) + fq * CH, q0 + wn * (TP * 16), fr);
            return;
        }
#pragma unroll
        for (int a = 0; a < TM; ++a) {
            u4 v[TP];
#pragma unroll
            for (int b = 0; b < TP; ++b)
                v[b] = __builtin_amdgcn_raw_buffer_load_b128(rs_part, other + (uint32_t)((((wave * TM + a) * TP + b) * 64 + lane) * 16), 0, 16 );
#pragma unroll
            for (int b = 0; b < TP; ++b) acc[a][b] += __builtin_bit_cast(float4v, v[b]);
            __builtin_amdgcn_sched_barrier(0);
        }
        conv_epilogue<T, TM, TP, PADQ, true, PIL>(p, acc, n0 + wm * (TM * 16) + fq * CH, q0 + wn * (TP * 16), fr);
        return;
    } else {
        if constexpr (MODE == 3) conv_epilogue_pool2<T, TM, TP>(p, acc, n0 + wm * (TM * 16) + fq * CH, q0 + wn * (TP * 16), fr);
        else if constexpr (FUSE2) {
            static_assert(!FUSE2 || 2 * LDS_BYTES <= 163840, "two workgroups per CU");
            if constexpr (S2) conv_epilogue_fused_1x1<PADQ, false>(p, acc, q0, wm, wn, wave, lane, smem);
            else conv_epilogue_fused_1x1<PADQ, true>(p, acc, q0, wm, wn, wave, lane, smem);
        }
        else if constexpr (FAST) conv_epilogue_fast<TM, TP, PADQ, PIL>(p, acc, n0 + wm * (TM * 16) + fq * CH, q0 + wn * (TP * 16), fr);
        else conv_epilogue<T, TM, TP, PADQ, true, PIL>(p, acc, n0 + wm * (TM * 16) + fq * CH, q0 + wn * (TP * 16), fr);
    }
#ifdef YOLO_EXPERIMENT
    if (p.trace && tid == 0) {
        asm volatile("s_waitcnt vmcnt(0)" ::: "memory");
        unsigned long long *r = p.trace + (size_t)blockIdx.x * 8;
        r[0] = t_start; r[1] = t_setup; r[2] = t_loop; r[3] = wall_clock64();
        r[4] = __builtin_amdgcn_s_getreg(0xF804);
        r[5] = __builtin_amdgcn_s_getreg(0xF814);
        r[6] = (unsigned long long)bid;
        r[7] = (unsigned long long)clock64() - c_start;
    }
#endif
}

template <int WM, int WN, int TM, int TP, int PRG, int OCC, int MODE>
__global__ void __launch_bounds__(512, OCC) conv3x3_tap_stream_kernel(const ConvParams p) {
    typedef _Float16 T;
    constexpr int NW = 8, S = 3, ROWB = 64;
    constexpr int NA = WM * TM * 16;
    constexpr int NB = WN * TP * 16;
    constexpr int JA_TOT = NA / 16;
    constexpr int JA = (JA_TOT + NW - 1) / NW;
    constexpr int PW = 24;
    constexpr int FROW = MODE == 2 ? PW : 16;
    constexpr int JP = (PRG + NW - 1) / NW;
    constexpr int CH = 4 * TM;
    constexpr int EPC = 8;
    constexpr int NQ = CH / EPC;
    constexpr int NST = TP * NQ;
    constexpr int A_BYTES = NA * ROWB;
    constexpr int P_BYTES = PRG * 1024;
    constexpr int BIAS_FLOATS = kTapStreamBiasFloats;
    static_assert(WM * WN == NW && (JA_TOT % NW == 0 || JA_TOT < NW), "tile / wave mapping");
    __shared__ __attribute__((aligned(16))) unsigned char smem[S * A_BYTES + 2 * P_BYTES + BIAS_FLOATS * 4];
    unsigned char *const smemP = smem + S * A_BYTES;
    float *const sbias = reinterpret_cast<float *>(smem + S * A_BYTES + 2 * P_BYTES);

    const int tid = threadIdx.x;
    const int lane = tid & 63;
    const int wave = __builtin_amdgcn_readfirstlane(tid >> 6);
    const int wm = wave / WN, wn = wave % WN;
    const bool has_a = JA_TOT % NW == 0 || wave < JA_TOT;
    const int fr = lane & 15, fq = lane >> 4;

    const __amdgpu_buffer_rsrc_t rs_in = __builtin_amdgcn_make_buffer_rsrc(const_cast<void *>(p.in), 0, p.in_bytes, 0x00020000);
    const __amdgpu_buffer_rsrc_t rs_w = __builtin_amdgcn_make_buffer_rsrc(const_cast<void *>(p.wgt), 0, p.wgt_bytes, 0x00020000);
    const __amdgpu_buffer_rsrc_t rs_out = __builtin_amdgcn_make_buffer_rsrc(p.out, 0, p.out_bytes, 0x00020000);
    const __amdgpu_buffer_rsrc_t rs_res = __builtin_amdgcn_make_buffer_rsrc(const_cast<void *>(p.res ? p.res : p.out), 0, p.res ? p.res_bytes : 0u, 0x00020000);

    for (int i = tid; i < p.cout_pad && i < BIAS_FLOATS; i += 512) sbias[i] = p.bias[i];

    const int lrow = lane >> 2;
    uint32_t a_off[JA];
#pragma unroll
    for (int j = 0; j < JA; ++j) {
        const int r = (j * NW + wave) * 16 + lrow;
        const int ws = r / (TM * 16), R = r % (TM * 16);
        const int tm = R >> 4, g4 = (R >> 2) & 3, jj = R & 3;
        const int ch = ws * (TM * 16) + g4 * CH + 4 * tm + jj;
        a_off[j] = (uint32_t)ch * p.wrow_bytes + (uint32_t)(((lane & 3) ^ tap_swz_w(lrow)) << 4);
    }
    constexpr int JP_FULL = PRG - (JP - 1) * NW;
    const bool jp_full = wave < JP_FULL;
    const uint32_t csw_p = (uint32_t)(((lane & 3) ^ (((lrow >> 2) & 1) << 1)) << 4);
    uint32_t b_off[JP];
    auto geometry = [&](int bid, int &q0, int &n0) __attribute__((always_inline)) {
        const int mt = (int)fdiv((uint32_t)bid, p.dtiles_n);
        n0 = (bid - mt * p.n_tiles_n) * NA;
        q0 = mt * NB;
        int t2_n = 0, t2_y0 = 0, t2_x0 = 0;
        if (MODE == 2) {
            t2_n = (int)fdiv((uint32_t)mt, p.dqHW);
            const int r = mt - t2_n * p.qHW;
            const int ty = (int)fdiv((uint32_t)r, p.dqW);
            t2_y0 = ty * (NB / 16);
            t2_x0 = (r - ty * p.qW) * 16;
        }
#pragma unroll
        for (int j = 0; j < JP; ++j) {
            const int g = j * NW + wave;
            bool ok;
            int n, y, x;
            if (MODE == 2) {
                const int R = g * 16 + lrow;
                const int pr = R / PW, pc = R - pr * PW;
                n = t2_n; y = t2_y0 - 1 + pr; x = t2_x0 - 1 + pc;
                ok = g < PRG && pc < 18 && pr < NB / 16 + 2 && t2_n * p.HoWo < p.M && (unsigned)y < (unsigned)p.H && (unsigned)x < (unsigned)p.W;
            } else {
                const int q = q0 - (p.qW + 1) + g * 16 + lrow;
                ok = g < PRG && q >= 0 && q < p.Mq;
                const int qq = ok ? q : 0;
                n = (int)fdiv((uint32_t)qq, p.dqHW);
                const int r = qq - n * p.qHW;
                y = (int)fdiv((uint32_t)r, p.dqW);
                x = r - y * p.qW;
                ok = ok && x < p.W && y < p.H;
            }
            const long long e = (long long)n * p.in_img_stride + ((long long)y * p.W + x) * p.in_ld + p.in_coff;
            b_off[j] = ok ? (uint32_t)(e * 2) + csw_p : YOLO_INVALID_OFF;
        }
    };

    const int C = p.cin_chunks >> 2;
    auto issue_patch = [&](int c, int buf) __attribute__((always_inline)) {
        const uint32_t koff = (uint32_t)c * ROWB;
#pragma unroll
        for (int j = 0; j < JP; ++j)
            if (j + 1 < JP || jp_full) tap_dma16(rs_in, smemP + buf * P_BYTES + (j * NW + wave) * 1024, b_off[j], koff);
    };
    auto issue_weights = [&](int tap, int c, int n0, int slot) __attribute__((always_inline)) {
        const uint32_t ka = (uint32_t)(tap * p.cin_chunks + 4 * c) * 16 + (uint32_t)n0 * p.wrow_bytes;
        if (has_a) {
#pragma unroll
            for (int j = 0; j < JA; ++j) tap_dma16(rs_w, smem + slot * A_BYTES + (j * NW + wave) * 1024, a_off[j], ka);
        }
    };

    float4v acc[TM][TP];
    const int a_frag = (wm * TM * 16 + fr) * ROWB + (((fq ^ tap_swz_w(fr)) & 3) << 4);
    const int rb = wn * TP * FROW + fr;
    const int c_lane = wm * (TM * 16) + fq * CH;
    auto compute = [&](int slot, int buf, int shift) __attribute__((always_inline)) {
        const unsigned char *A = smem + slot * A_BYTES + a_frag;
        const int R = rb + shift;
        const unsigned char *B = smemP + buf * P_BYTES + (R << 6) + ((fq << 4) ^ ((R & 4) << 3));
        uint4v fa[TM], fb[TP];
#pragma unroll
        for (int a = 0; a < TM; ++a) fa[a] = *reinterpret_cast<const uint4v *>(A + a * 16 * ROWB);
#pragma unroll
        for (int b = 0; b < TP; ++b) fb[b] = *reinterpret_cast<const uint4v *>(B + b * FROW * ROWB);
#pragma unroll
        for (int a = 0; a < TM; ++a)
#pragma unroll
            for (int b = 0; b < TP; ++b) tap_mfma<T>(acc[a][b], fa[a], fb[b]);
    };
    auto epilogue = [&](int q0, int n0) __attribute__((always_inline)) {
        constexpr int DEPTH = TP > 2 ? 2 : TP;
        const int cbase = n0 + c_lane;
        const bool c_ok = cbase < p.Cout;
        uint32_t ooff[DEPTH];
        uint4v rv[DEPTH][NQ];
        auto request = [&](int b, int slot) __attribute__((always_inline)) {
            int n, rem, oy, ox;
            const bool ok = conv_decode_pixel<MODE>(p, q0 + wn * (TP * 16) + b * 16 + fr, n, rem, oy, ox) && c_ok;
            const long long o = ((long long)n * p.out_img_stride + (long long)rem * p.out_ld + cbase) * 2;
            ooff[slot] = ok ? (uint32_t)o : YOLO_INVALID_OFF;
            if (p.has_res) {
                const long long ro = ((long long)n * p.res_img_stride + (long long)rem * p.res_ld + cbase) * 2;
                const uint32_t roff = ok ? (uint32_t)ro : YOLO_INVALID_OFF;
#pragma unroll
                for (int q = 0; q < NQ; ++q)
                    rv[slot][q] = __builtin_bit_cast(uint4v, __builtin_amdgcn_raw_buffer_load_b128(rs_res, roff, q * 16, 0));
            }
        };
#pragma unroll
        for (int b = 0; b < DEPTH; ++b) request(b, b);
#pragma unroll
        for (int b = 0; b < TP; ++b) {
            const int slot = b % DEPTH;
#pragma unroll
            for (int q = 0; q < NQ; ++q) {
                T t[EPC], r[EPC];
                if (p.has_res) __builtin_memcpy(r, &rv[slot][q], 16);
#pragma unroll
                for (int e = 0; e < EPC; ++e) {
                    const int i = q * EPC + e;
                    float x = acc[i >> 2][b][i & 3];
                    x = p.leaky ? fmaxf(0.1f * x, x) : x;
                    if (p.has_res) x += (float)r[e];
                    t[e] = (T)x;
                }
                uint4v u;
                __builtin_memcpy(&u, t, 16);
                __builtin_amdgcn_raw_buffer_store_b128(__builtin_bit_cast(__attribute__((__vector_size__(4 * sizeof(unsigned int)))) unsigned int, u), rs_out, ooff[slot], q * 16, 0);
            }
            if (b + DEPTH < TP) {
                __builtin_amdgcn_sched_barrier(0);
                request(b + DEPTH, slot);
            }
        }
    };
    auto init_acc = [&](int n0, bool from_lds) __attribute__((always_inline)) {
#pragma unroll
        for (int a = 0; a < TM; ++a) {
            const float4v bv = from_lds ? *reinterpret_cast<const float4v *>(sbias + n0 + c_lane + 4 * a)
                                        : *reinterpret_cast<const float4v *>(p.bias + n0 + c_lane + 4 * a);
#pragma unroll
            for (int b = 0; b < TP; ++b) acc[a][b] = bv;
        }
    };

    int it = blockIdx.x;
    int q0_cur, n0_cur, q0_nxt = 0, n0_nxt = 0;
    geometry(xcd_remap(it, p.n_blocks), q0_cur, n0_cur);
    init_acc(n0_cur, false);
    issue_patch(0, 0);
    issue_weights(0, 0, n0_cur, 0);
    issue_weights(1, 0, n0_cur, 1);
    int c = 0;
    bool after_epi = false;
    bool done = false;

    auto run_item = [&](auto bufc) __attribute__((always_inline)) {
        constexpr int buf = decltype(bufc)::value;
        const bool last_c = c + 1 == C;
        const int it_n = last_c ? it + (int)gridDim.x : it;
        const bool more = !last_c || it_n < p.n_blocks;
        const int c_n = last_c ? 0 : c + 1;
        if (!last_c) { n0_nxt = n0_cur; q0_nxt = q0_cur; }
#pragma unroll
        for (int tap = 0; tap < 9; ++tap) {
            const bool last = !more && tap == 8;
            const bool with_patch = more && (tap == 1 || tap == 2);
            const bool st = after_epi && tap < 2;
            if (last) tap_wait_vm<0>();
            else if (has_a) {
                if (!with_patch) { if (st) tap_wait_vm<JA + NST>(); else tap_wait_vm<JA>(); }
                else if (jp_full) { if (st) tap_wait_vm<JA + JP + NST>(); else tap_wait_vm<JA + JP>(); }
                else { if (st) tap_wait_vm<JA + JP - 1 + NST>(); else tap_wait_vm<JA + JP - 1>(); }
            } else {
                if (!with_patch) { if (st) tap_wait_vm<NST>(); else tap_wait_vm<0>(); }
                else if (jp_full) { if (st) tap_wait_vm<JP + NST>(); else tap_wait_vm<JP>(); }
                else { if (st) tap_wait_vm<JP - 1 + NST>(); else tap_wait_vm<JP - 1>(); }
            }
            __builtin_amdgcn_sched_barrier(0);
            __builtin_amdgcn_s_barrier();
            if (tap == 0 && more) {
                if (last_c) geometry(xcd_remap(it_n, p.n_blocks), q0_nxt, n0_nxt);
            }
            {
                if (tap + 2 < 9) issue_weights(tap + 2, c, n0_cur, (tap + 2) % S);
                else if (more) issue_weights(tap + 2 - 9, c_n, n0_nxt, (tap + 2) % S);
            }
            if (tap == 0 && more) issue_patch(c_n, buf ^ 1);
            const int kh = tap / 3, kw = tap - 3 * kh;
            compute(tap % S, buf, MODE == 2 ? kh * PW + kw : kh * p.qW + kw);
        }
        after_epi = false;
        if (last_c) {
            tap_mfma_drain<TM, TP>(acc);
            epilogue(q0_cur, n0_cur);
            if (!more) { done = true; return; }
            it = it_n; q0_cur = q0_nxt; n0_cur = n0_nxt;
            init_acc(n0_cur, true);
            after_epi = true;
        }
        c = c_n;
    };
    for (;;) {
        run_item(std::integral_constant<int, 0>());
        if (done) break;
        run_item(std::integral_constant<int, 1>());
        if (done) break;
    }
}

bool conv_tap_fits(const ConvTile &t, int W) {
    if (!t.is_tap()) return false;
    if (t.is2d()) return true;
    if (t.stride2()) {
        if (W & 1) return false;
        W >>= 1;
    }
    if (t.image_aligned() && (W * (W + 1) > t.nb() || W * (W + 1) * 5 < t.nb() * 4)) return false;
    if (t.stride2()) return t.nb() + W + 2 <= t.prg * 16;
    const int rows = YOLO_TAP_PIL ? t.prg * 16 / t.tp * t.tp : t.prg * 16;
    return t.nb() + 2 * W + 4 <= rows;
}

static bool tap_stream_ok(const ConvTile &t, const ConvParams &p) {
    if (!t.has(CAP_STREAM)) return false;
    if (p.f32 || p.out_f32 || p.ksplit > 1 || p.outmode != OUT_NORMAL || !p.vec_out || (p.has_res && (!p.vec_res || !p.res_bytes)) || !p.out_bytes) return false;
    return p.Cout % 16 == 0 && (p.Cout + 127) / 128 * 128 <= kTapStreamBiasFloats;
}

static bool tap_lean(const ConvTile &t, const ConvParams &p) {
    static const bool no_fast_epi = getenv("YOLO_NO_FAST_EPI") != nullptr;
    return (!no_fast_epi || p.fuse2) && conv_fast_epilogue_ok(p) && (!t.has(CAP_NO_LEAN) || p.fuse2);
}

static ConvForm tap_form(const ConvTile &t, const ConvParams &p) {
    if (!t.is_tap() || (p.f32 && !t.f32_ok())) return FORM_INVALID;
    if (p.stream && tap_stream_ok(t, p)) return FORM_STREAM;
    if (p.ksplit > 1) return (p.pair ? t.split_occ != 0 : t.has(CAP_SPLITK)) ? FORM_SPLITK : FORM_INVALID;
    if (p.outmode == OUT_POOL2) return t.has(CAP_POOL) ? FORM_POOL : FORM_INVALID;
    if (p.fuse2) return t.has(CAP_FUSE2) && tap_lean(t, p) ? FORM_FUSED : FORM_INVALID;
    return !p.f32 && tap_lean(t, p) ? FORM_LEAN : FORM_GENERIC;
}

struct TapInst { bool f32; int occ, mode; bool splitk, fast, fuse2; };
static constexpr TapInst tap_inst(const ConvTile &t, ConvForm f, bool f32) {
    return {f32, f == FORM_SPLITK ? t.split_occ : t.occ, f == FORM_POOL ? 3 : t.mode, f == FORM_SPLITK, f == FORM_LEAN || f == FORM_FUSED, f == FORM_FUSED};
}

std::string conv_tap_symbol(const ConvTile &t, const ConvParams &p) {
    const ConvForm f = tap_form(t, p);
    if (f == FORM_INVALID) return "";
    char b[192];
    auto tf = [](bool v) { return v ? "true" : "false"; };
    const TapInst i = tap_inst(t, f, p.f32 != 0);
    if (f == FORM_STREAM) snprintf(b, sizeof b, "void yolo::conv3x3_tap_stream_kernel<%d, %d, %d, %d, %d, %d, %d>(yolo::ConvParams)", t.wm, t.wn, t.tm, t.tp, t.prg, t.occ, t.mode);
    else snprintf(b, sizeof b, "void yolo::conv3x3_tap_kernel<%s, %d, %d, %d, %d, %d, %d, %d, %s, %s, %s>(yolo::ConvParams)", tf(i.f32), t.wm, t.wn, t.tm, t.tp, t.prg,
                  i.occ, i.mode, tf(i.splitk), tf(i.fast), tf(i.fuse2));
    return b;
}

template <int ID, ConvForm F, bool F32>
static hipError_t launch_tap_inst(const ConvParams &p, dim3 grid, hipStream_t s) {
    constexpr ConvTile t = kTiles[ID];
    constexpr TapInst i = tap_inst(t, F, F32);
    hipLaunchKernelGGL((conv3x3_tap_kernel<i.f32, t.wm, t.wn, t.tm, t.tp, t.prg, i.occ, i.mode, i.splitk, i.fast, i.fuse2>), grid, dim3(512), 0, s, p);
    return hipGetLastError();
}
template <int ID, ConvForm F, bool HAS_F32>
static hipError_t launch_tap_dtype(const ConvParams &p, dim3 grid, hipStream_t s) {
    if constexpr (HAS_F32) if (p.f32) return launch_tap_inst<ID, F, true>(p, grid, s);
    return launch_tap_inst<ID, F, false>(p, grid, s);
}

template <int ID>
static hipError_t launch_tap_tile(ConvForm f, const ConvParams &p0, dim3 grid, hipStream_t s) {
    constexpr ConvTile t = kTiles[ID];
    if constexpr (t.is_tap()) {
        switch (f) {
        case FORM_GENERIC: return launch_tap_dtype<ID, FORM_GENERIC, true>(p0, grid, s);
        case FORM_LEAN: return launch_tap_inst<ID, FORM_LEAN, false>(p0, grid, s);
        case FORM_SPLITK: if constexpr (t.split_occ != 0) return launch_tap_dtype<ID, FORM_SPLITK, t.f32_ok()>(p0, grid, s); break;
        case FORM_POOL: if constexpr (t.has(CAP_POOL)) return launch_tap_dtype<ID, FORM_POOL, t.f32_ok()>(p0, grid, s); break;
        case FORM_FUSED: if constexpr (t.has(CAP_FUSE2)) return launch_tap_inst<ID, FORM_FUSED, false>(p0, grid, s); break;
        case FORM_STREAM:
            if constexpr (t.has(CAP_STREAM)) {
                ConvParams p = p0;
                p.cout_pad = (p.Cout + 127) / 128 * 128;
                constexpr int slots = kTapStreamCUs * t.per_cu();
                static_assert(slots == kTapStreamGrid, "yolo_launch_caps reports kTapStreamGrid");
                hipLaunchKernelGGL((conv3x3_tap_stream_kernel<t.wm, t.wn, t.tm, t.tp, t.prg, t.occ, t.mode>), dim3((unsigned)(p.n_blocks < slots ? p.n_blocks : slots)), dim3(512), 0, s, p);
                return hipGetLastError();
            }
            break;
        default: break;
        }
    }
    return hipErrorInvalidValue;
}
template <int... ID>
static hipError_t launch_tap_by_id(int id, ConvForm f, const ConvParams &p, dim3 grid, hipStream_t s, std::integer_sequence<int, ID...>) {
    hipError_t e = hipErrorInvalidValue;
    (void)((id == ID && ((e = launch_tap_tile<ID>(f, p, grid, s)), true)) || ...);
    return e;
}

hipError_t launch_conv_tap(const ConvParams &p0, int tile, hipStream_t s) {
    if (tile < 0 || tile >= kNumTiles) return hipErrorInvalidValue;
    const ConvTile &t = conv_tile(tile);
    ConvParams p = p0;
    p.fast_epi = tap_lean(t, p) ? 1 : 0;
    const bool s2 = t.stride2();
    if (p.ksize != 3 || p.stride != (s2 ? 2 : 1) || p.pad != 1 || (p.cin_chunks & 3) || !conv_tap_fits(t, p.W) || (p.f32 && !t.f32_ok()))
        return hipErrorInvalidValue;
    if (s2 ? ((p.H & 1) || (p.W & 1) || p.Ho * 2 != p.H || p.Wo * 2 != p.W || p.f32 || p.ksplit > 1 || (p.fuse2 && !t.has(CAP_FUSE2)) || p.outmode == OUT_POOL2 || p.qW != p.Wo + 1)
           : (p.Ho != p.H || p.Wo != p.W))
        return hipErrorInvalidValue;
    if (t.image_aligned() ? (p.q_stride != p.qHW || p.Ho * (p.Wo + 1) > t.nb()) : (!t.is2d() && p.q_stride != t.nb()))
        return hipErrorInvalidValue;
    if (p.outmode == OUT_POOL2 && (!t.has(CAP_POOL) || (p.H & 1) || (p.W & 1) || p.has_res || p.ksplit > 1 || !p.vec_out || p.Cout % 16))
        return hipErrorInvalidValue;
    const ConvForm f = tap_form(t, p);
    if (f == FORM_SPLITK) {
        if (!p.part || p.kunits < 1 || (long long)p.ksplit * p.kunits < (p.cin_chunks >> 2)) return hipErrorInvalidValue;
        if (p.pair && (p.ksplit < 2 || (p.ksplit > 2 && !t.has(CAP_SPLITK)) || !p.pair_cnt || p.n_blocks > 512 ||
                       (unsigned long long)p.n_blocks * (unsigned long long)p.ksplit * 128ull * t.nb() * 4ull > p.part_bytes))
            return hipErrorInvalidValue;
    }
    if (f == FORM_FUSED && (t.has(CAP_FUSE2_RES) != (p.has_res != 0) || p.n_tiles_n != 1 || p.Cout != 128 || !p.w2 || !p.b2 || !p.out2 || !p.out2_bytes))
        return hipErrorInvalidValue;
    const dim3 grid((unsigned)p.n_blocks, (unsigned)(p.ksplit > 1 ? p.ksplit : 1));
    return launch_tap_by_id(tile, f, p, grid, s, std::make_integer_sequence<int, kNumTiles>());
}

}
```

tensorflow-yolo_amd/csrc/forward.cpp:

```cpp
#include <cstdlib>
#include <cstring>

#include "conv_tiles.h"
#include "yolo_internal.h"

namespace yolo {
namespace {

inline const unsigned char *weights_at(const yolo_net *net, size_t off) { return net->dev_weights ? net->dev_weights + off : nullptr; }
inline const float *floats_at(const yolo_net *net, size_t off) { return reinterpret_cast<const float *>(weights_at(net, off)); }

struct Ptrs {
    yolo_net *net;
    NetIn in;
    float *out;
    int img0 = 0;
    int arena = 0;
    int nb = 0;
    unsigned char *buf_base(int b) const {
        if (b == BUF_USER_IN) return static_cast<unsigned char *>(const_cast<void *>(in.ptr));
        if (b == BUF_USER_OUT) return reinterpret_cast<unsigned char *>(out);
        return net->dev_ws + (size_t)arena * net->arena_bytes + net->buffers[b].offset;
    }
    unsigned char *view_ptr(const View &v) const { return buf_base(v.buf) + (size_t)(v.base + v.coff) * (v.f32 ? 4 : net->esize); }
};

struct Parts { int n = 0; Ptrs p[4]; };
Parts split_parts(yolo_net *net, const NetIn in_dev, float *out_dev, int batch) {
    const yolo_layer_desc &d0 = net->layers[0].d;
    const size_t in_img = (size_t)d0.h * d0.w * d0.c;
    const int per = part_batch(net);
    Parts P;
    for (int img0 = 0; img0 < batch && P.n < 4; img0 += per, ++P.n)
        P.p[P.n] = Ptrs{net, in_dev.at((size_t)img0 * in_img), out_dev + (size_t)img0 * net->out_count, img0, P.n, batch - img0 < per ? batch - img0 : per};
    return P;
}

void view_info(const yolo_net *net, const Kernel &k, const char *what, yolo_kernel_info *out) {
    out->out_h = k.out.H; out->out_w = k.out.W; out->cout = k.out.C; out->cin = k.in.C;
    out->bytes = view_elems(k.in) * (k.in.f32 ? 4.0 : net->esize) + view_elems(k.out) * view_esz(net, k.out) + (k.has_res ? view_elems(k.in2) * net->esize : 0.0);
    snprintf(out->name, sizeof out->name, "%s<%s>", what, dtype_tag(net));
}
void prep_params(const Kernel &k, const Ptrs &P, PrepParams &p) {
    p.in = P.in.ptr;
    p.out = P.view_ptr(k.out);
    p.pixels = (long long)P.nb * k.in.H * k.in.W;
    p.C = k.in.C; p.Cpad = k.out.ld;
}
int first_params(const yolo_net *net, const Kernel &k, const Ptrs &P, FirstParams &p) {
    if (!view_chunk_aligned(k.out, net->epc)) return fail(YOLO_ERR_PLAN, "first-layer kernel needs a 16-byte aligned output view");
    p.in = P.in.ptr; p.out = P.view_ptr(k.out);
    p.wgt = floats_at(net, k.w_off); p.bias = floats_at(net, k.b_off);
    p.H = k.in.H; p.W = k.in.W; p.Cout = k.cout; p.out_ld = k.out.ld; p.leaky = k.leaky;
    p.pool = k.pool_fused;
    p.round_half = net->opt.dtype == YOLO_DTYPE_F16;
    p.out_img_stride = k.out.img_stride;
    p.total = (long long)P.nb * k.in.H * k.in.W;
    return YOLO_OK;
}
void first_info(const yolo_net *net, const Kernel &k, yolo_kernel_info *out) {
    out->ksize = 3; out->stride = 1; out->cin = 3; out->cout = k.cout; out->out_h = k.out.H; out->out_w = k.out.W;
    out->flops = 2.0 * k.out.H * k.out.W * k.cout * 27;
    out->bytes = (double)k.in.H * k.in.W * 3 * 4 + view_elems(k.out) * view_esz(net, k.out);
    out->weight_bytes = 28.0 * k.cout * 4;
    snprintf(out->name, sizeof out->name, k.pool_fused ? "conv_first_pool<%s,%d>" : "conv_first<%s,%d>", dtype_tag(net), k.cout);
    if (k.pool_fused) { out->out_h = k.in.H; out->out_w = k.in.W; out->flops = 2.0 * k.in.H * k.in.W * k.cout * 27; }
    set_symbol(out, first_symbol(net->opt.dtype, k.cout, k.pool_fused != 0));
    if (k.stem == STEM_FIRST_FOLDED) {
        out->symbol[0] = 0;
        out->flops = 0; out->bytes = 0; out->weight_bytes = 0;
        snprintf(out->name, sizeof out->name, "conv_first<fused into conv_stem>");
    }
}
void stem_params(const yolo_net *net, size_t ki, const Ptrs &P, StemParams &p) {
    const Kernel &f = net->kernels[ki - 1], &k = net->kernels[ki];
    memset(&p, 0, sizeof p);
    p.in = P.in.ptr;
    p.w1 = floats_at(net, f.w_off); p.b1 = floats_at(net, f.b_off);
    p.w2 = weights_at(net, k.w_off); p.b2 = floats_at(net, k.b_off);
    p.w2_bytes = (uint32_t)k.w_bytes;
    p.wrow2 = (uint32_t)k.ktiles * 128;
    p.out = P.view_ptr(k.out);
    p.H = f.in.H; p.W = f.in.W; p.Ho = k.out.H; p.Wo = k.out.W;
    p.out_ld = k.out.ld; p.out_img_stride = k.out.img_stride;
    p.in_img_stride = (long long)f.in.H * f.in.W * 3;
    if (ki + 1 < net->kernels.size() && net->kernels[ki + 1].stem == STEM_TAIL) {
        const Kernel &t = net->kernels[ki + 1];
        p.w3 = weights_at(net, t.w_off); p.b3 = floats_at(net, t.b_off);
        p.out3 = P.view_ptr(t.out);
        p.out3_ld = t.out.ld; p.out3_img_stride = t.out.img_stride;
    }
}
int conv_params(yolo_net *net, const Kernel &k, const Ptrs &P, ConvParams &p) {
    const int batch = P.nb;
    const long long in_bytes = (long long)batch * k.in.img_stride * net->esize;
    if (in_bytes > 0x7ffffff0LL) return fail(YOLO_ERR_ARG, "conv input tensor exceeds 2 GiB (32-bit buffer addressing): lower the batch");
    if ((long long)batch * net->layers[k.src_layer].H * net->layers[k.src_layer].W > 0x7fffffffLL)
        return fail(YOLO_ERR_ARG, "too many output pixels for one launch");
    conv_shape_params(net, k, batch, p);
    p.in = P.buf_base(k.in.buf);
    p.in_bytes = (uint32_t)in_bytes;
    p.wgt = weights_at(net, k.w_off);
    p.bias = floats_at(net, k.b_off);
    p.out = P.view_ptr(k.out);
    p.vec_out = p.vec_out && ((uintptr_t)P.buf_base(k.out.buf) % 16 == 0);
    if (k.head && net->obj_bytes && net->head.n_classes > 0 && !p.vec_out && p.out_f32 && k.outmode == OUT_NORMAL && !k.has_res) {
        const int width = 5 + net->head.n_classes;
        const long long base = k.out.base + k.out.coff;
        const size_t rows = net->out_count / (size_t)width;
        if (k.out.ld % width == 0 && base % width == 0 && rows * width == net->out_count && (size_t)batch * rows * 4 <= net->obj_bytes) {
            p.obj_out = reinterpret_cast<float *>(net->dev_ws + net->obj_off) + (size_t)P.img0 * rows;
            p.obj_width = width; p.obj_rows = (int)rows; p.obj_row0 = (int)(base / width); p.obj_na = k.out.ld / width;
            p.obj_min = net->obj_min_logit;
        }
    }
    if (k.has_res) p.res = P.view_ptr(k.in2);
    return YOLO_OK;
}

void attach_fuse2(const yolo_net *net, const Kernel &b, const Ptrs &P, ConvParams &p) {
    p.fuse2 = 1;
    p.w2 = weights_at(net, b.w_off);
    p.w2_bytes = (uint32_t)b.w_bytes;
    p.wrow2_bytes = (uint32_t)b.ktiles * 128;
    p.b2 = floats_at(net, b.b_off);
    p.out2 = P.view_ptr(b.out);
    p.out2_bytes = (uint32_t)((long long)P.nb * b.out.img_stride * net->esize);
    p.out2_ld = b.out.ld;
    p.out2_img_stride = b.out.img_stride;
    p.leaky2 = b.leaky;
}

hipError_t launch_conv_any(const yolo_net *net, const Kernel &k, const ConvParams &p0, const ConvLaunch &L, hipStream_t s, int arena = 0) {
    const int tile = L.tile, ks = L.ks;
    ConvParams p = p0;
    if (ks > 1) {
        p.ksplit = ks; p.kunits = L.ku;
        p.cout_pad = (p.Cout + 127) / 128 * 128;
        unsigned char *base = net->dev_ws + net->splitk_off + (size_t)arena * arena_slab_bytes(net);
        p.part = reinterpret_cast<float *>(base + kPairCounterBytes);
        if (L.pair) {
            const size_t data_bytes = arena_slab_data_bytes(net);
            p.pair = 1;
            p.pair_cnt = reinterpret_cast<int *>(base);
            p.part_bytes = (uint32_t)(data_bytes < 0x7ffffff0u ? data_bytes : 0x7ffffff0u);
        }
    }
    if (tile <= 0) p.f32_emu = conv_f32_emu_rule(net->opt.f32_products, net->opt.dtype, p, k.cfg, k.perchunk != 0, ks) ? 1 : 0;
    hipError_t e = tile > 0 ? launch_conv_dma(p, tile, s) : launch_conv(p, net->opt.dtype, k.cfg, k.perchunk != 0, s);
    if (e != hipSuccess || ks <= 1 || L.pair) return e;
    return launch_splitk_reduce(reduce_params(p), s);
}
void pool_params(const Kernel &k, const Ptrs &P, PoolParams &p) {
    p.in = P.view_ptr(k.in);
    p.out = P.view_ptr(k.out);
    p.H = k.in.H; p.W = k.in.W; p.C = k.in.C; p.in_ld = k.in.ld;
    p.Ho = k.out.H; p.Wo = k.out.W; p.out_ld = k.out.ld; p.stride = k.pool_stride;
    p.in_img_stride = k.in.img_stride; p.out_img_stride = k.out.img_stride;
    p.total = (long long)P.nb * k.out.H * k.out.W;
    p.ksize = k.pool_k;
}
void spp_params(const Kernel &k, const Ptrs &P, SppParams &p) {
    memset(&p, 0, sizeof p);
    p.in = P.view_ptr(k.in);
    p.H = k.in.H; p.W = k.in.W; p.chunks = k.in.C / 8;
    p.in_ld = k.in.ld; p.in_img_stride = k.in.img_stride;
    const View *ov[3] = {&k.out, &k.out2, &k.out3};
    for (int l = 0; l < 3; ++l) {
        p.out[l] = P.view_ptr(*ov[l]);
        p.out_ld[l] = ov[l]->ld; p.out_img_stride[l] = ov[l]->img_stride;
    }
}
void pool_info(const yolo_net *net, const Kernel &k, yolo_kernel_info *out) {
    view_info(net, k, "pool", out);
    const char *t = dtype_tag(net);
    const int epc = net->epc;
    const bool vec = pool_vec_strides(k.in.C, k.in.ld, k.out.ld, k.in.img_stride, k.out.img_stride, epc) && (k.in.base + k.in.coff) % epc == 0 && (k.out.base + k.out.coff) % epc == 0;
    set_symbol(out, aux_symbol(K_POOL, net->opt.dtype, vec));
    if (k.spp) {
        out->ksize = k.pool_k; out->stride = 1;
        out->bytes += view_elems(k.out2) * view_esz(net, k.out2) + view_elems(k.out3) * view_esz(net, k.out3);
        snprintf(out->name, sizeof out->name, "spp_pool<%s,%d-%d-%d>", t, k.pool_k, 2 * k.pool_k - 1, 3 * k.pool_k - 2);
        set_symbol(out, spp_pool_symbol((k.pool_k - 1) / 2));
    } else if (k.pool_k != 2) {
        out->ksize = k.pool_k; out->stride = 1;
        snprintf(out->name, sizeof out->name, "pool_same<%s,%dx%d>", t, k.pool_k, k.pool_k);
        set_symbol(out, pool_same_symbol(net->opt.dtype, vec));
    }
}
void eltwise_params(const yolo_net *net, const Kernel &k, const Ptrs &P, EltParams &p) {
    memset(&p, 0, sizeof p);
    p.a = P.view_ptr(k.in);
    p.a_f32 = k.in.f32;
    p.b = k.has_res ? P.view_ptr(k.in2) : nullptr;
    p.out = P.view_ptr(k.out);
    p.H = k.in.H; p.W = k.in.W; p.C = k.in.C;
    p.a_ld = k.in.ld; p.b_ld = k.in2.ld; p.out_ld = k.out.ld;
    p.outmode = k.outmode;
    p.out_f32 = k.out.f32 || net->opt.dtype == YOLO_DTYPE_F32;
    p.a_img_stride = k.in.img_stride; p.b_img_stride = k.in2.img_stride; p.out_img_stride = k.out.img_stride;
    p.total = (long long)P.nb * k.in.H * k.in.W * k.in.C;
}
bool create_streams(std::vector<hipStream_t> &st, size_t ns, std::vector<hipEvent_t> &fork, size_t nf, std::vector<hipEvent_t> &join, size_t nj) {
    st.assign(ns, nullptr); fork.assign(nf, nullptr); join.assign(nj, nullptr);
    bool ok = true;
    for (hipStream_t &x : st) ok = ok && hipStreamCreateWithFlags(&x, hipStreamNonBlocking) == hipSuccess;
    for (std::vector<hipEvent_t> *ev : {&fork, &join})
        for (hipEvent_t &x : *ev) ok = ok && hipEventCreateWithFlags(&x, hipEventDisableTiming) == hipSuccess;
    return ok;
}
int side_streams(yolo_net *net) {
    StreamPool &sp = net->streams;
    if (sp.side.empty() && !create_streams(sp.side, (size_t)net->parts - 1, sp.fork, 1, sp.join, (size_t)net->parts - 1))
        return fail(YOLO_ERR_HIP, "multi-stream forward: stream/event creation failed");
    return YOLO_OK;
}
int branch_streams(yolo_net *net, int arena) {
    StreamPool &sp = net->streams;
    const size_t n = (size_t)(net->arenas > 0 ? net->arenas : 1);
    if (sp.branch.empty() && !create_streams(sp.branch, n, sp.bfork, 4 * n, sp.bjoin, n))
        return fail(YOLO_ERR_HIP, "branch tail: stream / event creation failed");
    return (size_t)arena < sp.branch.size() ? YOLO_OK : fail(YOLO_ERR_STATE, "branch tail: arena out of range");
}

bool branch_tails_ok(yolo_net *net, int batch) {
    static const bool off = getenv("YOLO_NO_BRANCH_STREAM") != nullptr;
    if (off || net->side_chains <= 0 || net->opt.keep_all || batch <= 0 || batch > net->opt.max_batch) return false;
    if (net->side_ok.size() != (size_t)net->opt.max_batch + 1) net->side_ok.assign((size_t)net->opt.max_batch + 1, -1);
    signed char &memo = net->side_ok[(size_t)batch];
    if (memo < 0) memo = pass_splits_k(net, batch) ? 0 : 1;
    return memo == 1;
}
int run_forward_pass(const Ptrs &P, hipStream_t s, hipEvent_t *ev, long long *obj_rows_out) {
    yolo_net *net = P.net;
    const int dtype = net->opt.dtype, batch = P.nb, arena = P.arena;
    const bool u8 = P.in.u8;
    long long obj_rows_written = 0;
    bool fused2_done = false;
    const bool use_branch = !ev && branch_tails_ok(net, batch);
    hipStream_t const s_main = s;
    hipStream_t s_branch = nullptr;
    int cur_tail = 0;
    if (use_branch) {
        const int rc = branch_streams(net, arena);
        if (rc) return rc;
        s_branch = net->streams.branch[arena];
    }
    for (size_t ki = 0; ki < net->kernels.size(); ++ki) {
        const Kernel &k = net->kernels[ki];
        hipError_t e = hipSuccess;
        s = s_main;
        if (use_branch && k.side) {
            if (k.side != cur_tail) {
                hipEvent_t ef = net->streams.bfork[(size_t)arena * 4 + (size_t)((k.side - 1) & 3)];
                if (hipEventRecord(ef, s_main) != hipSuccess || hipStreamWaitEvent(s_branch, ef, 0) != hipSuccess)
                    return fail(YOLO_ERR_HIP, "branch tail: fork failed");
                cur_tail = k.side;
            }
            s = s_branch;
        }
        if (ev && hipEventRecord(ev[2 * ki], s) != hipSuccess) return fail(YOLO_ERR_HIP, "hipEventRecord failed");
        bool no_launch = !has_own_launch(k);
        if (k.kind == K_CONV && k.stem == STEM_NONE && k.fuse2_prev && fused2_done) no_launch = true, fused2_done = false;
        if (no_launch) {
        } else if (k.kind == K_PREP) {
            PrepParams p;
            prep_params(k, P, p);
            e = launch_prep(p, dtype, s, u8);
        } else if (k.kind == K_FIRST) {
            FirstParams p;
            const int rc = first_params(net, k, P, p);
            if (rc) return rc;
            e = launch_first(p, dtype, s, u8);
        } else if (k.kind == K_CONV && k.stem == STEM_HOST) {
            StemParams p;
            stem_params(net, ki, P, p);
            e = launch_stem(p, batch, s, net->halves ? kStemGrid / net->parts : kStemGrid, u8);
        } else if (k.kind == K_CONV) {
            ConvParams p;
            const int rc = conv_params(net, k, P, p);
            if (rc) return rc;
            if (k.head && p.obj_out) obj_rows_written += (long long)p.Ho * p.Wo * p.obj_na;
            if (k.mx) {
                e = launch_conv_mx(p, s);
            } else {
                const ConvLaunch L = resolve_conv(net, ki, p, k.tile, arena_slab_data_bytes(net));
                if (L.fuse2) attach_fuse2(net, net->kernels[ki + 1], P, p);
                fused2_done = L.fuse2 != 0;
                e = launch_conv_any(net, k, p, L, s, arena);
            }
        } else if (k.kind == K_POOL && k.spp) {
            SppParams p;
            spp_params(k, P, p);
            e = launch_spp(p, (k.pool_k - 1) / 2, batch, s);
        } else if (k.kind == K_POOL) {
            PoolParams p;
            pool_params(k, P, p);
            e = k.pool_k == 2 ? launch_pool(p, dtype, s) : launch_pool_same(p, dtype, s);
        } else if (k.kind == K_ELTWISE) {
            EltParams p;
            eltwise_params(net, k, P, p);
            e = launch_eltwise(p, dtype, s);
        }
        if (e != hipSuccess) {
            char msg[160];
            snprintf(msg, sizeof msg, "kernel %zu (layer %d) launch failed: %s", ki, k.layer, hipGetErrorString(e));
            return fail(YOLO_ERR_HIP, msg);
        }
        if (ev && hipEventRecord(ev[2 * ki + 1], s) != hipSuccess) return fail(YOLO_ERR_HIP, "hipEventRecord failed");
    }
    if (cur_tail) {
        hipEvent_t ej = net->streams.bjoin[arena];
        if (hipEventRecord(ej, s_branch) != hipSuccess || hipStreamWaitEvent(s_main, ej, 0) != hipSuccess) return fail(YOLO_ERR_HIP, "branch tail: join failed");
    }
    *obj_rows_out = obj_rows_written;
    return YOLO_OK;
}

int run_forward_parts(yolo_net *net, const NetIn in_dev, int batch, float *out_dev, hipStream_t s) {
    const long long rows = net->head.n_classes > 0 ? (long long)(net->out_count / (size_t)(5 + net->head.n_classes)) : -1;
    const Parts parts = split_parts(net, in_dev, out_dev, batch);
    const bool multi = parts.n > 1;
    StreamPool &sp = net->streams;
    if (multi) {
        const int rc = side_streams(net);
        if (rc) return rc;
        HIP_TRY(hipEventRecord(sp.fork[0], s));
    }
    net->halves = multi;
    bool all = true;
    for (int i = 0; i < parts.n; ++i) {
        hipStream_t st = i == 0 ? s : sp.side[i - 1];
        if (i > 0) HIP_TRY(hipStreamWaitEvent(st, sp.fork[0], 0));
        long long w = 0;
        const int rc = run_forward_pass(parts.p[i], st, nullptr, &w);
        if (rc) return rc;
        all = all && w == rows;
    }
    for (int i = 1; i < parts.n; ++i) {
        HIP_TRY(hipEventRecord(sp.join[i - 1], sp.side[i - 1]));
        HIP_TRY(hipStreamWaitEvent(s, sp.join[i - 1], 0));
    }
    net->obj_valid = net->obj_bytes > 0 && rows > 0 && all;
    return YOLO_OK;
}

int forward_failed(yolo_net *net, int rc) {
    const std::string msg = get_error();
    (void)hipGetLastError();
    (void)zero_pair_counters(net);
    set_error(msg);
    return rc;
}

}

int zero_pair_counters(yolo_net *net) {
    if (!net->splitk_bytes || !net->dev_ws) return YOLO_OK;
    const size_t per = net->splitk_bytes / (size_t)net->arenas;
    for (int a = 0; a < net->arenas; ++a)
        HIP_TRY(hipMemset(net->dev_ws + net->splitk_off + (size_t)a * arena_slab_bytes(net), 0, per < kPairCounterBytes ? per : kPairCounterBytes));
    HIP_TRY(hipDeviceSynchronize());
    return YOLO_OK;
}

void destroy_streams(yolo_net *net) {
    StreamPool &sp = net->streams;
    for (std::vector<hipEvent_t> *ev : {&sp.fork, &sp.join, &sp.bfork, &sp.bjoin})
        for (hipEvent_t e : *ev) if (e) (void)hipEventDestroy(e);
    for (std::vector<hipStream_t> *st : {&sp.side, &sp.branch})
        for (hipStream_t x : *st) if (x) (void)hipStreamDestroy(x);
    sp = StreamPool();
}

void aux_kernel_info(const yolo_net *net, int kernel, yolo_kernel_info *out) {
    const Kernel &k = net->kernels[kernel];
    if (k.kind == K_FIRST) return first_info(net, k, out);
    if (k.kind == K_POOL) return pool_info(net, k, out);
    view_info(net, k, k.kind == K_PREP ? "prep" : "eltwise", out);
    set_symbol(out, aux_symbol(k.kind, net->opt.dtype, false));
}

bool all_heads_write_objectness(yolo_net *net, const NetIn in_dev, float *out_dev, int batch) {
    if (!net->obj_bytes || net->head.n_classes <= 0) return false;
    const Ptrs P = split_parts(net, in_dev, out_dev, batch).p[0];
    bool any = false;
    for (const Kernel &k : net->kernels) {
        if (k.kind != K_CONV || !k.head) continue;
        ConvParams p;
        if (conv_params(net, k, P, p) != 0 || !p.obj_out) return false;
        any = true;
    }
    return any;
}

int run_forward(yolo_net *net, const NetIn in_dev, int batch, float *out_dev, hipStream_t s) {
    const int rc = run_forward_parts(net, in_dev, batch, out_dev, s);
    return rc == YOLO_OK ? rc : forward_failed(net, rc);
}

int run_forward_timed(yolo_net *net, const NetIn in_dev, int batch, float *out_dev, hipStream_t s, float *ms_host) {
    const size_t nk = net->kernels.size();
    std::vector<hipEvent_t> ev(2 * nk, nullptr);
    for (auto &e : ev)
        if (hipEventCreate(&e) != hipSuccess) return fail(YOLO_ERR_HIP, "hipEventCreate failed");
    for (size_t k = 0; k < nk; ++k) ms_host[k] = 0.f;
    net->halves = false;
    const Parts parts = split_parts(net, in_dev, out_dev, batch);
    int rc = YOLO_OK;
    for (int i = 0; rc == YOLO_OK && i < parts.n; ++i) {
        long long w = 0;
        rc = run_forward_pass(parts.p[i], s, ev.data(), &w);
        if (rc == YOLO_OK && hipStreamSynchronize(s) != hipSuccess) rc = fail(YOLO_ERR_HIP, "hipStreamSynchronize failed");
        for (size_t k = 0; rc == YOLO_OK && k < nk; ++k) {
            float t = 0.f;
            if (hipEventElapsedTime(&t, ev[2 * k], ev[2 * k + 1]) != hipSuccess) rc = fail(YOLO_ERR_HIP, "hipEventElapsedTime failed");
            ms_host[k] += t;
        }
    }
    net->obj_valid = false;
    if (rc != YOLO_OK) forward_failed(net, rc);
    for (auto &e : ev) (void)hipEventDestroy(e);
    return rc;
}

int tune_streams(yolo_net *net, const NetIn in_dev, int batch, hipStream_t s, const char *who) {
    if (!net->arena_full || batch <= (net->opt.max_batch + 1) / 2) return YOLO_OK;
    float *logits = reinterpret_cast<float *>(net->dev_ws + net->logits_off);
    hipEvent_t e0, e1;
    HIP_TRY(hipEventCreate(&e0));
    if (hipEventCreate(&e1) != hipSuccess) {
        (void)hipEventDestroy(e0);
        return fail(YOLO_ERR_HIP, std::string(who) + ": hipEventCreate failed");
    }
    float best[3] = {0.f, 1e30f, 1e30f};
    int rc = YOLO_OK;
    for (int rep = 0; rep < 5 && rc == YOLO_OK; ++rep)
        for (int parts = 1; parts <= 2 && rc == YOLO_OK; ++parts) {
            net->parts = parts;
            if (hipEventRecord(e0, s) != hipSuccess) rc = fail(YOLO_ERR_HIP, std::string(who) + ": hipEventRecord failed");
            for (int k = 0; k < 3 && rc == YOLO_OK; ++k) rc = run_forward(net, in_dev, batch, logits, s);
            if (rc == YOLO_OK && (hipEventRecord(e1, s) != hipSuccess || hipEventSynchronize(e1) != hipSuccess))
                rc = fail(YOLO_ERR_HIP, std::string(who) + ": event failed");
            float ms = 0.f;
            if (rc == YOLO_OK && hipEventElapsedTime(&ms, e0, e1) == hipSuccess && rep > 0 && ms < best[parts]) best[parts] = ms;
        }
    (void)hipEventDestroy(e0);
    (void)hipEventDestroy(e1);
    net->parts = (rc == YOLO_OK && best[2] < 0.985f * best[1]) ? 2 : (rc == YOLO_OK ? 1 : net->arenas);
    net->parts_tuned = rc == YOLO_OK;
    net->obj_valid = false;
    return rc;
}

int autotune_tiles(yolo_net *net, const NetIn in_dev, int batch, hipStream_t s) {
    float *logits = reinterpret_cast<float *>(net->dev_ws + net->logits_off);
    if (batch > part_batch(net)) batch = part_batch(net);
    int rc = run_forward(net, in_dev, batch, logits, s);
    if (rc) return rc;
    const Ptrs P = split_parts(net, in_dev, logits, batch).p[0];
    hipEvent_t e0, e1;
    HIP_TRY(hipEventCreate(&e0));
    HIP_TRY(hipEventCreate(&e1));
    for (size_t ki = 0; ki < net->kernels.size(); ++ki) {
        Kernel &k = net->kernels[ki];
        if (!conv_dispatched(k) || k.mx || !dma_eligible(net, k)) continue;
        ConvParams p;
        rc = conv_params(net, k, P, p);
        if (rc) break;
        float best = 1e30f;
        int best_tile = -1;
        for (int tile = 0; tile < kNumTiles; ++tile) {
            if (!conv_tile_valid(net, k, tile)) continue;
            const ConvLaunch L = resolve_conv(net, ki, p, tile, arena_slab_data_bytes(net));
            float ms = 1e30f;
            bool ok = true;
            for (int rep = 0; rep < 4 && ok; ++rep) {
                ok = hipEventRecord(e0, s) == hipSuccess && launch_conv_any(net, k, p, L, s) == hipSuccess &&
                     hipEventRecord(e1, s) == hipSuccess && hipEventSynchronize(e1) == hipSuccess;
                float t = 0.f;
                if (ok && rep > 0 && hipEventElapsedTime(&t, e0, e1) == hipSuccess && t < ms) ms = t;
            }
            if (!ok) { rc = fail(YOLO_ERR_HIP, "yolo_net_autotune: launch failed"); break; }
            if (ms < best) { best = ms; best_tile = tile; }
        }
        if (rc) break;
        k.tile = best_tile;
        net->side_ok.clear();
    }
    (void)hipEventDestroy(e0);
    (void)hipEventDestroy(e1);
    return rc;
}

}
```

tensorflow-yolo_amd/csrc/yolo_internal.h:

```cpp
#pragma once
#include <hip/hip_runtime.h>
#include <stdint.h>
#include <cstdio>
#include <string>
#include <vector>

#include "yolo_hip.h"
#include "train_host.h"
#include "train3_host.h"
#include "train_tail_host.h"
#include "train3_tail_host.h"
#include "augment_host.h"
#include "anchor_host.h"
#include "loss3_host.h"

namespace yolo {

enum OutMode { OUT_NORMAL = 0, OUT_UP2 = 1, OUT_REORG2 = 2, OUT_POOL2 = 3 };
enum BufId { BUF_NONE = -1, BUF_USER_OUT = -2, BUF_USER_IN = -3 };
enum ConvCfg { CFG_N128 = 0, CFG_N64 = 1, CFG_N32 = 2 };
enum KernelKind { K_PREP = 0, K_CONV = 1, K_POOL = 2, K_ELTWISE = 3, K_FIRST = 4 };

struct View {
    int buf = BUF_NONE;
    int H = 0, W = 0, C = 0;
    int ld = 0;
    int coff = 0;
    long long img_stride = 0;
    long long base = 0;
    bool f32 = false;
};
inline bool view_chunk_aligned(const View &v, int epc) { return v.ld % epc == 0 && (v.base + v.coff) % epc == 0 && v.img_stride % epc == 0; }

struct Buffer {
    long long elems_per_image = 0;
    int esize = 2;
    int first = 1 << 30, last = -1;
    size_t offset = 0;
    size_t bytes = 0;
    size_t used = 0;
    bool is_concat = false;
};

struct FastDiv {
    uint32_t mul, sh1, sh2, d;
};
inline FastDiv make_fastdiv(uint32_t d) {
    FastDiv f{1, 0, 0, d ? d : 1};
    uint32_t l = 0;
    while ((1ull << l) < f.d) ++l;
    f.mul = (uint32_t)((((1ull << l) - f.d) << 32) / f.d + 1);
    f.sh1 = l < 1 ? l : 1;
    f.sh2 = l > 0 ? l - 1 : 0;
    return f;
}
__host__ __device__ __forceinline__ uint32_t fdiv(uint32_t n, const FastDiv &f) {
#if defined(__HIP_DEVICE_COMPILE__)
    const uint32_t t = __umulhi(f.mul, n);
#else
    const uint32_t t = (uint32_t)(((unsigned long long)f.mul * n) >> 32);
#endif
    return (t + ((n - t) >> f.sh1)) >> f.sh2;
}

__host__ __device__ __forceinline__ float leaky01(float x) {
#if defined(__HIP_DEVICE_COMPILE__)
    float r;
    const float y = 0.1f * x;
    asm("v_max_f32 %0, %1, %2" : "=v"(r) : "v"(y), "v"(x));
    return r;
#else
    return x > 0.1f * x ? x : 0.1f * x;
#endif
}

__host__ __device__ __forceinline__ float u8_unit(unsigned u) {
#pragma clang fp contract(off)
    const float a = (float)u;
    const float rcp = 0x1.010102p-8f;
    const float q = a * rcp;
    return __builtin_fmaf(__builtin_fmaf(-255.f, q, a), rcp, q);
}

constexpr int kCandCountStride = 32;

constexpr int kTapStreamCUs = 256, kTapStreamPerCu = 2;
constexpr int kTapStreamGrid = kTapStreamCUs * kTapStreamPerCu;
constexpr int kStemGrid = 512;
constexpr int kFirstMfmaGrid = 1024;
constexpr int kAuxBlock = 256, kAuxGrid = 256 * 16;
constexpr int kDecodeBlock = 256, kDecodeGrid = 256 * 8;

struct ConvParams {
    const void *in;
    const void *wgt;
    const float *bias;
    const void *res;
    void *out;
    uint32_t in_bytes, wgt_bytes;
    uint32_t out_bytes, res_bytes;
    int H, W, in_ld, in_coff;
    long long in_img_stride;
    int Ho, Wo, HoWo, M;
    int Cout, out_ld;
    long long out_img_stride;
    int res_ld;
    long long res_img_stride;
    int ksize, stride, pad, taps;
    int ktiles, tiles_per_tap, cpt_shift;
    int cin_chunks;
    uint32_t wrow_bytes;
    int leaky, has_res, outmode, out_f32, vec_out, vec_res;
    int f32;
    int n_tiles_n, n_blocks;
    int ksplit, kunits, cout_pad;
    float *part;
    int pair;
    int *pair_cnt;
    uint32_t part_bytes;
    int stream;
    int fast_epi;
    int fuse2;
    const void *w2;
    const float *b2;
    void *out2;
    uint32_t w2_bytes, wrow2_bytes, out2_bytes;
    int out2_ld, leaky2;
    long long out2_img_stride;
    int dbg;
    int f32_emu;
    int qW, qHW, Mq;
    int q_stride;
    int t2_shift;
    float *obj_out;
    int obj_width, obj_rows, obj_row0, obj_na;
    float obj_min;
    unsigned long long *trace;
    FastDiv dHoWo, dWo, dqHW, dqW, dtiles_n, dtpt;
};
inline bool conv_fast_epilogue_ok(const ConvParams &p) {
    return !p.f32 && !p.out_f32 && p.outmode == OUT_NORMAL && p.vec_out && p.out_bytes && p.Cout % 16 == 0 && p.ksplit <= 1 &&
           (!p.has_res || (p.vec_res && p.res_bytes));
}
inline void conv_set_divisors(ConvParams &p, int stages_per_tap) {
    p.dtpt = make_fastdiv((uint32_t)(stages_per_tap > 0 ? stages_per_tap : 1));
    p.dHoWo = make_fastdiv((uint32_t)p.HoWo);
    p.dWo = make_fastdiv((uint32_t)p.Wo);
    p.dqHW = make_fastdiv((uint32_t)(p.qHW > 0 ? p.qHW : 1));
    p.dqW = make_fastdiv((uint32_t)(p.qW > 0 ? p.qW : 1));
    p.dtiles_n = make_fastdiv((uint32_t)(p.n_tiles_n > 0 ? p.n_tiles_n : 1));
}

struct PrepParams {
    const void *in;
    void *out;
    long long pixels;
    int C, Cpad;
};

struct FirstParams {
    const void *in;
    const float *wgt;
    const float *bias;
    void *out;
    int H, W, Cout, out_ld, leaky, round_half;
    long long out_img_stride;
    long long total;
    FastDiv dW, dH, dHW;
    int pool;
    int xblocks;
    FastDiv dXB, dHp;
    int tiles_y, n_tiles;
};

struct StemParams {
    const void *in;
    const float *w1;
    const float *b1;
    const void *w2;
    const float *b2;
    void *out;
    const void *w3;
    const float *b3;
    void *out3;
    int out3_ld;
    long long out3_img_stride;
    uint32_t w2_bytes, wrow2;
    int H, W, Ho, Wo, out_ld;
    long long in_img_stride, out_img_stride;
    int tiles_x, tiles_y, n_tiles;
    FastDiv dtx, dty;
};

struct ResizeParams {
    const unsigned char *src;
    void *dst;
    int src_h, src_w, src_row_bytes, dst_h, dst_w, swap_rb;
};

constexpr int kFramesPerLaunch = 64;
struct FrameGeom {
    const unsigned char *src;
    int src_h, src_w, src_row_bytes, swap_rb;
    int new_h, new_w, off_y, off_x;
};
struct FramesParams {
    FrameGeom f[kFramesPerLaunch];
    void *dst;
    int dst_h, dst_w;
    int wide;
};
struct BoxGeom { int new_h, new_w, off_y, off_x; };
struct RemapParams {
    BoxGeom g[kFramesPerLaunch];
    yolo_box *boxes;
    const int *counts;
    int max_boxes, net_h, net_w;
};

struct PoolParams {
    const void *in;
    void *out;
    int H, W, C, in_ld, Ho, Wo, out_ld, stride;
    long long in_img_stride, out_img_stride;
    long long total;
    int ksize = 2;
};
inline bool pool_vec_strides(int C, int in_ld, int out_ld, long long in_img_stride, long long out_img_stride, int epc) {
    return C % epc == 0 && in_ld % epc == 0 && out_ld % epc == 0 && in_img_stride % epc == 0 && out_img_stride % epc == 0;
}

struct SppParams {
    const void *in;
    void *out[3];
    int H, W, chunks;
    int in_ld, out_ld[3];
    long long in_img_stride, out_img_stride[3];
    int slab, slab_shift;
    int slabs;
    FastDiv dW;
};

struct EltParams {
    const void *a;
    const void *b;
    void *out;
    int H, W, C, a_ld, b_ld, out_ld, outmode, out_f32, a_f32;
    long long a_img_stride, b_img_stride, out_img_stride;
    long long total;
};

struct ReduceParams {
    const float *part;
    const float *bias;
    const void *res;
    void *out;
    float *obj_out;
    int obj_width, obj_rows, obj_row0, obj_na;
    int ksplit, M, Cout, cout_pad, HoWo, Wo;
    int out_ld, res_ld, leaky, outmode, out_f32, f32;
    long long out_img_stride, res_img_stride;
};

struct DecodeScale {
    int row0, h, w, na;
    double aw[YOLO_MAX_ANCHORS], ah[YOLO_MAX_ANCHORS];
};

struct DecodeParams {
    const float *logits;
    const float *obj;
    int version, n_classes, rows, n_scales;
    DecodeScale sc[YOLO_MAX_SCALES];
// ... 163 lines not shown
    int ppc, n_chunks, tiles_cout, tiles_cin, halo_rows;
    int slab_stride;
};
struct TailAdamParams {
    AdamParams a;
    const double *scale64;
    const float *mean;
};
hipError_t launch_tail_adam(const TailAdamParams &p, hipStream_t s);
hipError_t launch_conv1x1_dgrad(const DgradParams &p, int y_dtype, long long tiles, hipStream_t s);
hipError_t launch_conv3x3_wgrad(const Wgrad3x3Params &p, int x_dtype, hipStream_t s);
hipError_t launch_conv3x3_wgrad_f16(const Wgrad3x3Params &p, unsigned int *record, int db_groups, int db_positions, hipStream_t s);

hipError_t launch_head3_dgrad(const Dgrad3Params &p, hipStream_t s);

hipError_t launch_conv(const ConvParams &p, int dtype, int cfg, bool perchunk, hipStream_t s);
struct ConvTile;
int choose_dma_cfg(int M, int cout, int cin_chunks, int taps, int has_res, bool v1_ok, int stride, int W, bool tap_only = false);
bool dma_cfg_valid(int cfg, int cout, int cin_chunks, bool v1_ok, int ksize, int stride, int W);
hipError_t launch_conv_dma(const ConvParams &p, int cfg, hipStream_t s);
hipError_t launch_conv_tap(const ConvParams &p, int tile, hipStream_t s);
bool conv_tap_fits(const ConvTile &t, int W);
std::string conv_tile_symbol(int tile, ConvParams p);
std::string conv_tap_symbol(const ConvTile &t, const ConvParams &p);
constexpr int kMxMaxW = 100;
constexpr int kMxTile = 24;
bool conv_mx_fits(int W);
const char *conv_mx_symbol(bool fast);
hipError_t launch_conv_mx(const ConvParams &p, hipStream_t s);
hipError_t launch_mx_quantize(const void *src, int rows, int channels, unsigned char *q, unsigned char *sc, hipStream_t s);
unsigned char mx_quant_block_host(const float *v, unsigned char *q);
std::string conv_symbol(int dtype, int cfg, bool perchunk, bool f32_emu = false);
bool conv_f32_emu_rule(int f32_products, int dtype, const ConvParams &p, int cfg, bool perchunk, int ksplit);
std::string first_symbol(int dtype, int cout, bool pool);
std::string aux_symbol(int kind, int dtype, bool vec);
std::string pool_same_symbol(int dtype, bool vec);
std::string spp_pool_symbol(int rad);
__attribute__((visibility("hidden"))) ReduceParams reduce_params(const ConvParams &p);
hipError_t launch_splitk_reduce(const ReduceParams &p, hipStream_t s);
hipError_t launch_prep(const PrepParams &p, int dtype, hipStream_t s, bool in_u8 = false);
hipError_t launch_resize(const ResizeParams &p, hipStream_t s, bool dst_u8 = false);
hipError_t launch_frames_resize(const FramesParams &p, int n, hipStream_t s, bool dst_u8);
hipError_t launch_boxes_to_frames(const RemapParams &p, int n, hipStream_t s);
hipError_t launch_augment(const AugmentParams &p, int n, hipStream_t s);
enum AnchorStage { ANCHOR_PREPARE, ANCHOR_INIT, ANCHOR_SEED_SUM, ANCHOR_SEED_PICK, ANCHOR_ASSIGN, ANCHOR_UPDATE, ANCHOR_FINAL, ANCHOR_FINISH, ANCHOR_LABELS };
hipError_t launch_anchor(int stage, const AnchorParams &p, hipStream_t s);
hipError_t launch_first(const FirstParams &p, int dtype, hipStream_t s, bool in_u8 = false);
hipError_t launch_stem(const StemParams &p, int batch, hipStream_t s, int max_grid = kStemGrid, bool in_u8 = false);
hipError_t launch_pool(const PoolParams &p, int dtype, hipStream_t s);
hipError_t launch_pool_same(const PoolParams &p, int dtype, hipStream_t s);
constexpr int kSppMaxSide = 32;
hipError_t launch_spp(const SppParams &p, int rad, int batch, hipStream_t s);
int spp_slab(int H, int W, int chunks, int batch);
hipError_t launch_eltwise(const EltParams &p, int dtype, hipStream_t s);
hipError_t launch_decode(const DecodeParams &p, int batch, hipStream_t s, bool zero_counts = true);
hipError_t launch_nms(const NmsParams &p, int batch, hipStream_t s);
size_t nms_lds_bytes(int cap);
size_t nms_scratch_bytes(int cap);

enum StemRole {
    STEM_NONE = 0,
    STEM_FIRST_FOLDED = 1,
    STEM_HOST = 2,
    STEM_TAIL = 3,
};
struct Kernel {
    int kind = 0;
    int layer = -1;
    int src_layer = -1;
    View in, in2, out;
    int ksize = 0, stride = 0, cout = 0, cin = 0, cin_s = 0, leaky = 0, outmode = 0, has_res = 0;
    int cfg = 0, perchunk = 0, cpt = 0, ktiles = 0;
    int tile = -1;
    int head = 0;
    int pool_fused = 0;
    StemRole stem = STEM_NONE;
    int fuse2_next = 0;
    int fuse2_prev = 0;
    int mx = 0;
    int side = 0;
    size_t w_off = 0, b_off = 0, w_bytes = 0;
    size_t w_src = 0;
    int batch_norm = 0;
    int pool_stride = 0;
    int pool_k = 2;
    int spp = 0;
    int spp_layer[2] = {-1, -1};
    View out2, out3;
    std::string note;
};
inline bool conv_dispatched(const Kernel &k) { return k.kind == K_CONV && k.stem != STEM_HOST && k.stem != STEM_TAIL; }
inline bool has_own_launch(const Kernel &k) { return !(k.kind == K_FIRST && k.stem == STEM_FIRST_FOLDED) && !(k.kind == K_CONV && k.stem == STEM_TAIL); }
inline bool counts_as_conv_launch(const Kernel &k) { return k.kind == K_CONV && k.stem != STEM_TAIL; }

struct LayerInfo {
    yolo_layer_desc d;
    int H = 0, W = 0, C = 0;
    std::vector<int> consumers;
    int fused_into = -1;
    View view;
    bool materialised = false;
};

struct __attribute__((visibility("hidden"))) WsRegion {
    const char *name;
    size_t offset, used, bytes;
};

struct __attribute__((visibility("hidden"))) StreamPool {
    std::vector<hipStream_t> side;
    std::vector<hipEvent_t> fork, join;
    std::vector<hipStream_t> branch;
    std::vector<hipEvent_t> bfork, bjoin;
};

}

struct yolo_net {
    yolo_net_options opt;
    bool mx = false;
    std::vector<yolo::LayerInfo> layers;
    std::vector<yolo::Kernel> kernels;
    std::vector<yolo::Buffer> buffers;
    yolo_head_desc head;
    size_t weight_count = 0;
    size_t weights_bytes = 0;
    size_t act_bytes = 0;
    size_t logits_off = 0, cand_off = 0, count_off = 0, nms_off = 0;
    size_t splitk_off = 0, splitk_bytes = 0;
    std::vector<yolo::WsRegion> tail;
    size_t obj_off = 0, obj_bytes = 0;
    bool obj_valid = false;
    int cand_clean = 0;
    int side_chains = 0;
    std::vector<signed char> side_ok;
    float obj_min_logit = -__builtin_inff();
    yolo::StreamPool streams;
    int arenas = 1;
    bool arena_full = false;
    int parts = 1;
    bool parts_tuned = false;
    size_t arena_bytes = 0;
    bool halves = false;
    size_t workspace_bytes = 0;
    size_t out_count = 0;
    double flops_per_image = 0;
    int esize = 2, epc = 8;
    unsigned char *dev_weights = nullptr;
    unsigned char *dev_ws = nullptr;
    size_t dev_ws_bytes = 0;
    bool weights_loaded = false;
    unsigned char *wgrad_f16_dev = nullptr;
    size_t wgrad_f16_bytes = 0;
};

namespace yolo {
int plan_network(yolo_net *net, const yolo_layer_desc *layers, int n, std::string &err);
bool mx_eligible(const yolo_net *net, const Kernel &k);
int pack_weights(const yolo_net *net, const float *host, size_t n, std::vector<unsigned char> &blob, std::string &err);
std::string describe(const yolo_net *net);
void set_error(const std::string &s);
const char *get_error();
inline int fail(int code, const std::string &msg) {
    set_error(msg);
    return code;
}
#define HIP_TRY(expr)                                                                          \
    do {                                                                                       \
        hipError_t e_ = (expr);                                                                \
        if (e_ != hipSuccess) {                                                                \
            yolo::set_error(std::string(#expr) + ": " + hipGetErrorString(e_));                \
            return YOLO_ERR_HIP;                                                               \
        }                                                                                      \
    } while (0)

inline int part_batch(const yolo_net *net) { return (net->opt.max_batch + net->parts - 1) / net->parts; }
constexpr size_t kPairCounterBytes = 65536;
constexpr size_t kSplitkSlabMax = (size_t)64 << 20;
inline size_t arena_slab_bytes(const yolo_net *net) { return net->splitk_bytes / (size_t)net->arenas / 256 * 256; }
inline size_t arena_slab_data_bytes(const yolo_net *net) {
    const size_t slab = arena_slab_bytes(net);
    return slab > kPairCounterBytes ? slab - kPairCounterBytes : 0;
}
struct ConvLaunch {
    int tile, ks, ku, pair, fuse2;
    size_t slab_need;
};
void conv_shape_params(const yolo_net *net, const Kernel &k, int batch, ConvParams &p);
ConvLaunch resolve_conv(const yolo_net *net, size_t ki, const ConvParams &p, int tile_req, size_t slab_bytes);
bool dma_eligible(const yolo_net *net, const Kernel &k);
bool conv_tile_valid(const yolo_net *net, const Kernel &k, int tile);
size_t splitk_slab_bytes(const yolo_net *net);
bool pass_splits_k(const yolo_net *net, int batch);
void conv_kernel_info(const yolo_net *net, int kernel, yolo_kernel_info *out);
inline double view_elems(const View &v) { return (double)v.H * v.W * v.C; }
inline double view_esz(const yolo_net *net, const View &v) { return v.f32 ? 4.0 : (double)net->esize; }
inline const char *dtype_tag(const yolo_net *net) { return net->opt.dtype == YOLO_DTYPE_F16 ? "f16" : "f32"; }
inline void set_symbol(yolo_kernel_info *out, const std::string &sym) { snprintf(out->symbol, sizeof out->symbol, "%s", sym.c_str()); }

struct NetIn {
    const void *ptr;
    bool u8;
    NetIn at(size_t elems) const { return NetIn{static_cast<const unsigned char *>(ptr) + elems * (u8 ? 1 : 4), u8}; }
};
#pragma GCC visibility push(hidden)
int run_forward(yolo_net *net, NetIn in_dev, int batch, float *out_dev, hipStream_t s);
int run_forward_timed(yolo_net *net, NetIn in_dev, int batch, float *out_dev, hipStream_t s, float *ms_host);
int tune_streams(yolo_net *net, NetIn in_dev, int batch, hipStream_t s, const char *who);
int autotune_tiles(yolo_net *net, NetIn in_dev, int batch, hipStream_t s);
bool all_heads_write_objectness(yolo_net *net, NetIn in_dev, float *out_dev, int batch);
int zero_pair_counters(yolo_net *net);
void destroy_streams(yolo_net *net);
void aux_kernel_info(const yolo_net *net, int kernel, yolo_kernel_info *out);

int check_head(const yolo_head_desc *h, size_t out_count, std::string &err);
int check_ready(yolo_net *net, const void *in, int batch, const char *who);
int check_loss_args(const yolo_head_desc *head, const void *gt_dev, const void *gt_counts_dev, int max_gt, const void *images_dev,
                    const void *result_dev, const char *who);
int run_loss_grad(const yolo_head_desc &h, const float *logits, int batch, const yolo_gt *gt, const int32_t *gt_counts, int max_gt,
                  yolo_loss_image *images, int32_t *assign, yolo_loss_result *result, float *grad, hipStream_t s);
int run_loss3(const Loss3Geometry &geo, const float *logits, int batch, const yolo_gt *gt, const int32_t *gt_counts, int max_gt,
              double ignore_thresh, yolo_loss_image *parts, yolo_loss_image *images, int32_t *assign, yolo_loss_result *result, float *grad,
              hipStream_t s);
#pragma GCC visibility pop
inline size_t align256(size_t bytes) { return (bytes + 255) & ~(size_t)255; }
}
```

Measured before the change: 6369 images/sec.

## Add atomic work-claiming queues to persistent 3x3 tap conv kernel

For large 3x3 tap convolutions at the 76- and 38-wide scales, the kernel now launches a persistent grid of fixed size that pulls tiles dynamically from eight atomic claim queues, replacing the static grid-stride walk. The claim atomic is issued by the spare wave in place of a patch load it would not issue, then published through LDS so the next tile's geometry is known ahead of time. The aim is to reduce tail imbalance and launch overhead across CUs. In exchange it adds per-arena counter buffers, a last-block reset, extra LDS, and register pressure in the merged kernel body.

```diff
diff --git a/include/yolo_hip.h b/include/yolo_hip.h
--- a/include/yolo_hip.h
+++ b/include/yolo_hip.h
@@ -120,6 +120,7 @@
     int32_t tap_stream_workgroups, stem_workgroups, first_mfma_workgroups, aux_work_items, decode_rows;
 };
 int yolo_launch_caps(struct yolo_launch_caps *out);
+int yolo_net_claim_counters(const yolo_net *net, int32_t *host_out, size_t n);
 
 int yolo_net_autotune(yolo_net *net, const float *in_dev, int batch, void *stream);
 
diff --git a/tensorflow-yolo_amd/_hip.py b/tensorflow-yolo_amd/_hip.py
--- a/tensorflow-yolo_amd/_hip.py
+++ b/tensorflow-yolo_amd/_hip.py
@@ -239,6 +239,7 @@
     "yolo_preprocess_resize_u8": (C.c_int, [C.c_void_p, C.c_int, C.c_int, C.c_int, C.c_void_p, C.c_int, C.c_int, C.c_int, C.c_void_p]),
     "yolo_u8_unit_table": (C.c_int, [C.c_void_p]),
     "yolo_launch_caps": (C.c_int, [C.POINTER(LaunchCaps)]),
+    "yolo_net_claim_counters": (C.c_int, [C.c_void_p, C.POINTER(C.c_int32), C.c_size_t]),
     "yolo_net_autotune": (C.c_int, [C.c_void_p, C.c_void_p, C.c_int, C.c_void_p]),
     "yolo_net_tune_streams": (C.c_int, [C.c_void_p, C.c_void_p, C.c_int, C.c_void_p]),
     "yolo_net_set_streams": (C.c_int, [C.c_void_p, C.c_int]),
diff --git a/tensorflow-yolo_amd/csrc/api.cpp b/tensorflow-yolo_amd/csrc/api.cpp
--- a/tensorflow-yolo_amd/csrc/api.cpp
+++ b/tensorflow-yolo_amd/csrc/api.cpp
@@ -81,6 +81,7 @@
 void yolo_net_destroy(yolo_net *net) {
     if (!net) return;
     destroy_streams(net);
+    if (net->claim_dev) (void)hipFree(net->claim_dev);
     delete net;
 }
 
@@ -160,7 +161,21 @@
     net->dev_ws = static_cast<unsigned char *>(ws);
     net->cand_clean = 0;
     net->dev_ws_bytes = bytes;
+    if (!net->claim_dev) {
+        const size_t sets = (size_t)net->arenas * net->kernels.size();
+        HIP_TRY(hipMalloc(reinterpret_cast<void **>(&net->claim_dev), sets * kTapClaimWords * sizeof(int)));
+        net->claim_sets = sets;
+    }
     return zero_pair_counters(net);
+}
+
+int yolo_net_claim_counters(const yolo_net *net, int32_t *host_out, size_t n) {
+    if (!net || !host_out) return fail(YOLO_ERR_ARG, "yolo_net_claim_counters: null argument");
+    const size_t words = net->claim_sets * kTapClaimWords;
+    if (n < words) return fail(YOLO_ERR_ARG, "yolo_net_claim_counters: buffer too small");
+    HIP_TRY(hipDeviceSynchronize());
+    if (words) HIP_TRY(hipMemcpy(host_out, net->claim_dev, words * sizeof(int), hipMemcpyDeviceToHost));
+    return (int)words;
 }
 
 }
diff --git a/tensorflow-yolo_amd/csrc/conv_dispatch.cpp b/tensorflow-yolo_amd/csrc/conv_dispatch.cpp
--- a/tensorflow-yolo_amd/csrc/conv_dispatch.cpp
+++ b/tensorflow-yolo_amd/csrc/conv_dispatch.cpp
@@ -102,6 +102,16 @@
     return (units + ku - 1) / ku;
 }
 
+constexpr bool kClaim76 = true, kClaim38 = true;
+bool tap_claim_rule(const ConvParams &p, int tile, int ks, int fuse2) {
+    static const char *const off = getenv("YOLO_NO_TAP_CLAIM");
+    if (tile != TILE_TAP_128x256 || ks > 1 || fuse2 || p.f32 || !conv_fast_epilogue_ok(p) || p.HoWo <= 0) return false;
+    if (tap_blocks(p, tile) <= kTapStreamGrid) return false;
+    const bool c76 = p.W > 48, c38 = p.W > 24 && p.W <= 48;
+    if (off && (atoi(off) == 1 || (atoi(off) == 76 && c76) || (atoi(off) == 38 && c38))) return false;
+    return (c76 && kClaim76) || (c38 && kClaim38);
+}
+
 }
 
 ConvLaunch resolve_conv(const yolo_net *net, size_t ki, const ConvParams &p, int tile_req, size_t slab_bytes) {
@@ -116,7 +126,7 @@
         if ((tile == TILE_TAPS2_128x256 || tile == TILE_TAPS2IMG_128x384) && !conv_tile_valid(net, k, tile)) tile = or_else(TILE_TAPS2_128x256, or_else(TILE_DMA_256x128_K32, TILE_4WAVE));
         if (tile == TILE_TAPS2_128x256_WIDE && !conv_tile_valid(net, k, tile)) tile = or_else(TILE_DMA_128x256_K32, TILE_4WAVE);
     }
-    ConvLaunch r{tile, 1, 0, 0, 0, 0};
+    ConvLaunch r{tile, 1, 0, 0, 0, 0, 0};
     const bool tap_by_rule = conv_tile(tile).is_tap() && tile_req <= 0;
     const int units = p.cin_chunks >> 2;
     static const bool no_pair = getenv("YOLO_NO_PAIR_SPLIT") != nullptr;
@@ -151,6 +161,7 @@
         const long long ob = (long long)(p.M / p.HoWo) * net->kernels[ki + 1].out.img_stride * net->esize;
         r.fuse2 = ob > 0 && ob <= 0x7ffffff0LL;
     }
+    r.claim = tap_claim_rule(p, r.tile, r.ks, r.fuse2) ? 1 : 0;
     return r;
 }
 
diff --git a/tensorflow-yolo_amd/csrc/conv_tap.hip b/tensorflow-yolo_amd/csrc/conv_tap.hip
--- a/tensorflow-yolo_amd/csrc/conv_tap.hip
+++ b/tensorflow-yolo_amd/csrc/conv_tap.hip
@@ -77,6 +77,14 @@
 
 constexpr int kTapStreamBiasFloats = 512;
 
+}
+
+enum { WALK_STATIC = 0, WALK_CLAIM = 1 };
+constexpr int kTapStreamLdsBytes(int na, int prg, bool claim) { return 3 * na * 64 + 2 * prg * 1024 + kTapStreamBiasFloats * 4 + (claim ? 16 : 0); }
+template <int WM, int WN, int TM, int TP, int PRG, int MODE, int WALK>
+__device__ __forceinline__ void tap_stream_body(const ConvParams &p, unsigned char *const smem);
+constexpr bool tap_claim_inst(bool f32, int wm, int wn, int tm, int tp, int prg, int occ, int mode, bool splitk, bool fast, bool fuse2) {
+    return !f32 && wm == 2 && wn == 4 && tm == 4 && tp == 4 && prg == 26 && occ == 4 && mode == 1 && !splitk && fast && !fuse2;
 }
 
 template <bool F32, int WM, int WN, int TM, int TP, int PRG, int OCC, int MODE, bool SPLITK, bool FAST = false, bool FUSE2 = false>
@@ -112,8 +120,17 @@
     static_assert(!S2 || JA_TOT % NW == 0, "stride 2: every wave carries weights");
     if constexpr (S2 && (F32 || SPLITK)) return;
     static_assert(!FUSE2 || (FAST && WM == 2 && WN == 4 && TM == 4 && TP == 4), "back-to-back 1x1: the 128 x 256 tiles (eight waves)");
-    constexpr int LDS_BYTES = FUSE2 && kFuse2LdsBytes > S * A_BYTES + 2 * P_BYTES ? kFuse2LdsBytes : S * A_BYTES + 2 * P_BYTES;
+    constexpr bool CLAIMS = tap_claim_inst(F32, WM, WN, TM, TP, PRG, OCC, MODE, SPLITK, FAST, FUSE2);
+    constexpr int LDS_BYTES = CLAIMS ? kTapStreamLdsBytes(NA, PRG, true)
+                                     : FUSE2 && kFuse2LdsBytes > S * A_BYTES + 2 * P_BYTES ? kFuse2LdsBytes : S * A_BYTES + 2 * P_BYTES;
+    static_assert(!CLAIMS || (LDS_BYTES >= S * A_BYTES + 2 * P_BYTES && 2 * LDS_BYTES <= 163840), "two workgroups per CU, either body");
     __shared__ __attribute__((aligned(16))) unsigned char smem[LDS_BYTES];
+    if constexpr (CLAIMS) {
+        if (gridDim.x != (unsigned)p.n_blocks) {
+            tap_stream_body<WM, WN, TM, TP, PRG, MODE, WALK_CLAIM>(p, smem);
+            return;
+        }
+    }
     unsigned char *const smemP = smem + S * A_BYTES;
 
     const int tid = threadIdx.x;
@@ -570,9 +587,10 @@
 #endif
 }
 
-template <int WM, int WN, int TM, int TP, int PRG, int OCC, int MODE>
-__global__ void __launch_bounds__(512, OCC) conv3x3_tap_stream_kernel(const ConvParams p) {
+template <int WM, int WN, int TM, int TP, int PRG, int MODE, int WALK>
+__device__ __forceinline__ void tap_stream_body(const ConvParams &p, unsigned char *const smem) {
     typedef _Float16 T;
+    constexpr bool CLAIM = WALK == WALK_CLAIM;
     constexpr int NW = 8, S = 3, ROWB = 64;
     constexpr int NA = WM * TM * 16;
     constexpr int NB = WN * TP * 16;
@@ -589,9 +607,10 @@
     constexpr int P_BYTES = PRG * 1024;
     constexpr int BIAS_FLOATS = kTapStreamBiasFloats;
     static_assert(WM * WN == NW && (JA_TOT % NW == 0 || JA_TOT < NW), "tile / wave mapping");
-    __shared__ __attribute__((aligned(16))) unsigned char smem[S * A_BYTES + 2 * P_BYTES + BIAS_FLOATS * 4];
+    static_assert(kTapStreamLdsBytes(NA, PRG, CLAIM) == S * A_BYTES + 2 * P_BYTES + BIAS_FLOATS * 4 + (CLAIM ? 16 : 0), "LDS of the stream body");
     unsigned char *const smemP = smem + S * A_BYTES;
     float *const sbias = reinterpret_cast<float *>(smem + S * A_BYTES + 2 * P_BYTES);
+    int *const sclaim = reinterpret_cast<int *>(smem + S * A_BYTES + 2 * P_BYTES + BIAS_FLOATS * 4);
 
     const int tid = threadIdx.x;
     const int lane = tid & 63;
@@ -621,10 +640,22 @@
     const bool jp_full = wave < JP_FULL;
     const uint32_t csw_p = (uint32_t)(((lane & 3) ^ (((lrow >> 2) & 1) << 1)) << 4);
     uint32_t b_off[JP];
+    auto lane_now = [&]() __attribute__((always_inline)) {
+        unsigned z = 0u;
+        asm volatile("" : "+s"(z));
+        return (int)__builtin_amdgcn_mbcnt_hi(~0u, __builtin_amdgcn_mbcnt_lo(~0u, z));
+    };
     auto geometry = [&](int bid, int &q0, int &n0) __attribute__((always_inline)) {
         const int mt = (int)fdiv((uint32_t)bid, p.dtiles_n);
         n0 = (bid - mt * p.n_tiles_n) * NA;
         q0 = mt * NB;
+        int lr = lrow;
+        uint32_t csw = csw_p;
+        if constexpr (CLAIM) {
+            const int l = lane_now();
+            lr = l >> 2;
+            csw = (uint32_t)(((l & 3) ^ (((lr >> 2) & 1) << 1)) << 4);
+        }
         int t2_n = 0, t2_y0 = 0, t2_x0 = 0;
         if (MODE == 2) {
             t2_n = (int)fdiv((uint32_t)mt, p.dqHW);
@@ -639,12 +670,12 @@
             bool ok;
             int n, y, x;
             if (MODE == 2) {
-                const int R = g * 16 + lrow;
+                const int R = g * 16 + lr;
                 const int pr = R / PW, pc = R - pr * PW;
                 n = t2_n; y = t2_y0 - 1 + pr; x = t2_x0 - 1 + pc;
                 ok = g < PRG && pc < 18 && pr < NB / 16 + 2 && t2_n * p.HoWo < p.M && (unsigned)y < (unsigned)p.H && (unsigned)x < (unsigned)p.W;
             } else {
-                const int q = q0 - (p.qW + 1) + g * 16 + lrow;
+                const int q = q0 - (p.qW + 1) + g * 16 + lr;
                 ok = g < PRG && q >= 0 && q < p.Mq;
                 const int qq = ok ? q : 0;
                 n = (int)fdiv((uint32_t)qq, p.dqHW);
@@ -654,7 +685,7 @@
                 ok = ok && x < p.W && y < p.H;
             }
             const long long e = (long long)n * p.in_img_stride + ((long long)y * p.W + x) * p.in_ld + p.in_coff;
-            b_off[j] = ok ? (uint32_t)(e * 2) + csw_p : YOLO_INVALID_OFF;
+            b_off[j] = ok ? (uint32_t)(e * 2) + csw : YOLO_INVALID_OFF;
         }
     };
 
@@ -693,13 +724,18 @@
     };
     auto epilogue = [&](int q0, int n0) __attribute__((always_inline)) {
         constexpr int DEPTH = TP > 2 ? 2 : TP;
-        const int cbase = n0 + c_lane;
+        int fr_e = fr, cl_e = c_lane;
+        if constexpr (CLAIM) {
+            const int l = lane_now();
+            fr_e = l & 15; cl_e = wm * (TM * 16) + (l >> 4) * CH;
+        }
+        const int cbase = n0 + cl_e;
         const bool c_ok = cbase < p.Cout;
         uint32_t ooff[DEPTH];
         uint4v rv[DEPTH][NQ];
         auto request = [&](int b, int slot) __attribute__((always_inline)) {
             int n, rem, oy, ox;
-            const bool ok = conv_decode_pixel<MODE>(p, q0 + wn * (TP * 16) + b * 16 + fr, n, rem, oy, ox) && c_ok;
+            const bool ok = conv_decode_pixel<MODE>(p, q0 + wn * (TP * 16) + b * 16 + fr_e, n, rem, oy, ox) && c_ok;
             const long long o = ((long long)n * p.out_img_stride + (long long)rem * p.out_ld + cbase) * 2;
             ooff[slot] = ok ? (uint32_t)o : YOLO_INVALID_OFF;
             if (p.has_res) {
@@ -749,20 +785,63 @@
 
     int it = blockIdx.x;
     int q0_cur, n0_cur, q0_nxt = 0, n0_nxt = 0;
+    int c = 0;
+    bool after_epi = false;
+    bool done = false;
+    constexpr int CW = NW - 1;
+    static_assert(!CLAIM || (JP_FULL <= CW && JA_TOT % NW == 0 && JP >= 2), "the claim rides in the place of a patch request the last wave does not issue");
+    const int nq = gridDim.x < 8u ? (int)gridDim.x : 8;
+    int cq = nq == 8 ? (int)(blockIdx.x & 7u) : (int)blockIdx.x;
+    int cqw = cq;
+    uint32_t claim_v = 0u;
+    auto claim_pos = [&](int q, int v) __attribute__((always_inline)) {
+        const int first = nq == 8 ? (int)((gridDim.x + 7u - (unsigned)q) >> 3) : 1;
+        return v < 0x01000000 ? q + nq * (first + v) : 0x7fffffff;
+    };
+    auto claim_issue = [&]() __attribute__((always_inline)) {
+#if defined(__HIP_DEVICE_COMPILE__)
+        if (lane_now() == 0)
+            asm volatile("s_nop 4\n\tglobal_atomic_add %0, %1, %2, %3 sc0" : "=&v"(claim_v) : "v"((uint32_t)cqw * 128u), "v"(1u), "s"(p.claim) : "memory");
+#endif
+    };
+    auto claim_result = [&]() __attribute__((always_inline)) {
+        asm volatile("" : "+v"(claim_v));
+        return claim_pos(cqw, (int)__builtin_amdgcn_readfirstlane(claim_v));
+    };
+    auto claim_retry = [&]() __attribute__((always_inline)) {
+        if (wave == CW && claim_result() >= p.n_blocks) {
+            cqw = cqw + 1 == nq ? 0 : cqw + 1;
+            claim_issue();
+        }
+    };
+    auto claim_publish = [&]() __attribute__((always_inline)) {
+        if (wave == CW) {
+            const int pos = claim_result();
+            if (lane_now() == 0) {
+                *reinterpret_cast<volatile int *>(sclaim) = pos;
+                *reinterpret_cast<volatile int *>(sclaim + 1) = cqw;
+            }
+            asm volatile("s_waitcnt lgkmcnt(0)" ::: "memory");
+        }
+    };
+
     geometry(xcd_remap(it, p.n_blocks), q0_cur, n0_cur);
     init_acc(n0_cur, false);
+    if (CLAIM && C == 1 && wave == CW) claim_issue();
     issue_patch(0, 0);
     issue_weights(0, 0, n0_cur, 0);
     issue_weights(1, 0, n0_cur, 1);
-    int c = 0;
-    bool after_epi = false;
-    bool done = false;
+    if (CLAIM && C == 1) {
+        if (wave == CW) tap_wait_vm<JP - 1 + 2 * JA>();
+        claim_publish();
+    }
 
     auto run_item = [&](auto bufc) __attribute__((always_inline)) {
         constexpr int buf = decltype(bufc)::value;
         const bool last_c = c + 1 == C;
-        const int it_n = last_c ? it + (int)gridDim.x : it;
-        const bool more = !last_c || it_n < p.n_blocks;
+        int it_n = last_c ? it + (int)gridDim.x : it;
+        bool more = !last_c || it_n < p.n_blocks;
+        bool claim_here = false;
         const int c_n = last_c ? 0 : c + 1;
         if (!last_c) { n0_nxt = n0_cur; q0_nxt = q0_cur; }
 #pragma unroll
@@ -770,18 +849,33 @@
             const bool last = !more && tap == 8;
             const bool with_patch = more && (tap == 1 || tap == 2);
             const bool st = after_epi && tap < 2;
+            const bool jpf = jp_full || (CLAIM && claim_here && wave == CW);
             if (last) tap_wait_vm<0>();
             else if (has_a) {
                 if (!with_patch) { if (st) tap_wait_vm<JA + NST>(); else tap_wait_vm<JA>(); }
-                else if (jp_full) { if (st) tap_wait_vm<JA + JP + NST>(); else tap_wait_vm<JA + JP>(); }
+                else if (jpf) { if (st) tap_wait_vm<JA + JP + NST>(); else tap_wait_vm<JA + JP>(); }
                 else { if (st) tap_wait_vm<JA + JP - 1 + NST>(); else tap_wait_vm<JA + JP - 1>(); }
             } else {
                 if (!with_patch) { if (st) tap_wait_vm<NST>(); else tap_wait_vm<0>(); }
-                else if (jp_full) { if (st) tap_wait_vm<JP + NST>(); else tap_wait_vm<JP>(); }
+                else if (jpf) { if (st) tap_wait_vm<JP + NST>(); else tap_wait_vm<JP>(); }
                 else { if (st) tap_wait_vm<JP - 1 + NST>(); else tap_wait_vm<JP - 1>(); }
+            }
+            if constexpr (CLAIM) {
+                if (claim_here && tap >= 3 && tap < 8) claim_retry();
+                if (claim_here && tap == 8) claim_publish();
             }
             __builtin_amdgcn_sched_barrier(0);
             __builtin_amdgcn_s_barrier();
+            if constexpr (CLAIM) {
+                if (tap == 0) {
+                    if (last_c) {
+                        it_n = __builtin_amdgcn_readfirstlane(*reinterpret_cast<volatile int *>(sclaim));
+                        cq = __builtin_amdgcn_readfirstlane(*reinterpret_cast<volatile int *>(sclaim + 1));
+                        more = it_n < p.n_blocks;
+                    }
+                    claim_here = C == 1 ? more : c + 2 == C;
+                }
+            }
             if (tap == 0 && more) {
                 if (last_c) geometry(xcd_remap(it_n, p.n_blocks), q0_nxt, n0_nxt);
             }
@@ -790,6 +884,7 @@
                 else if (more) issue_weights(tap + 2 - 9, c_n, n0_nxt, (tap + 2) % S);
             }
             if (tap == 0 && more) issue_patch(c_n, buf ^ 1);
+            if constexpr (CLAIM) { if (tap == 0 && claim_here && wave == CW) { cqw = cq; claim_issue(); } }
             const int kh = tap / 3, kw = tap - 3 * kh;
             compute(tap % S, buf, MODE == 2 ? kh * PW + kw : kh * p.qW + kw);
         }
@@ -810,6 +905,19 @@
         run_item(std::integral_constant<int, 1>());
         if (done) break;
     }
+    if constexpr (CLAIM) {
+        if (tid == CW * 64) {
+            const int t = __hip_atomic_fetch_add(p.claim + 8 * kTapClaimStride, 1, __ATOMIC_RELAXED, __HIP_MEMORY_SCOPE_AGENT);
+            if (t == (int)gridDim.x - 1)
+                for (int q = 0; q < 9; ++q) __hip_atomic_store(p.claim + q * kTapClaimStride, 0, __ATOMIC_RELAXED, __HIP_MEMORY_SCOPE_AGENT);
+        }
+    }
+}
+
+template <int WM, int WN, int TM, int TP, int PRG, int OCC, int MODE>
+__global__ void __launch_bounds__(512, OCC) conv3x3_tap_stream_kernel(const ConvParams p) {
+    __shared__ __attribute__((aligned(16))) unsigned char smem[kTapStreamLdsBytes(WM * TM * 16, PRG, false)];
+    tap_stream_body<WM, WN, TM, TP, PRG, MODE, WALK_STATIC>(p, smem);
 }
 
 bool conv_tap_fits(const ConvTile &t, int W) {
@@ -931,7 +1039,13 @@
     }
     if (f == FORM_FUSED && (t.has(CAP_FUSE2_RES) != (p.has_res != 0) || p.n_tiles_n != 1 || p.Cout != 128 || !p.w2 || !p.b2 || !p.out2 || !p.out2_bytes))
         return hipErrorInvalidValue;
-    const dim3 grid((unsigned)p.n_blocks, (unsigned)(p.ksplit > 1 ? p.ksplit : 1));
+    dim3 grid((unsigned)p.n_blocks, (unsigned)(p.ksplit > 1 ? p.ksplit : 1));
+    static_assert(kTapStreamGrid % 8 == 0, "eight claim queues over the first tiles");
+    if (p.claim && f == FORM_LEAN && tap_claim_inst(false, t.wm, t.wn, t.tm, t.tp, t.prg, t.occ, t.mode, false, true, false) &&
+        t.per_cu() == kTapStreamPerCu && p.n_blocks > kTapStreamGrid && (p.Cout + 127) / 128 * 128 <= kTapStreamBiasFloats) {
+        p.cout_pad = (p.Cout + 127) / 128 * 128;
+        grid.x = (unsigned)kTapStreamGrid;
+    }
     return launch_tap_by_id(tile, f, p, grid, s, std::make_integer_sequence<int, kNumTiles>());
 }
 
diff --git a/tensorflow-yolo_amd/csrc/forward.cpp b/tensorflow-yolo_amd/csrc/forward.cpp
--- a/tensorflow-yolo_amd/csrc/forward.cpp
+++ b/tensorflow-yolo_amd/csrc/forward.cpp
@@ -146,6 +146,8 @@
             p.part_bytes = (uint32_t)(data_bytes < 0x7ffffff0u ? data_bytes : 0x7ffffff0u);
         }
     }
+    if (L.claim && net->claim_dev)
+        p.claim = net->claim_dev + ((size_t)arena * net->kernels.size() + (size_t)(&k - net->kernels.data())) * kTapClaimWords;
     if (tile <= 0) p.f32_emu = conv_f32_emu_rule(net->opt.f32_products, net->opt.dtype, p, k.cfg, k.perchunk != 0, ks) ? 1 : 0;
     hipError_t e = tile > 0 ? launch_conv_dma(p, tile, s) : launch_conv(p, net->opt.dtype, k.cfg, k.perchunk != 0, s);
     if (e != hipSuccess || ks <= 1 || L.pair) return e;
@@ -356,6 +358,10 @@
 }
 
 int zero_pair_counters(yolo_net *net) {
+    if (net->claim_dev) {
+        HIP_TRY(hipMemset(net->claim_dev, 0, net->claim_sets * kTapClaimWords * sizeof(int)));
+        if (!net->splitk_bytes || !net->dev_ws) HIP_TRY(hipDeviceSynchronize());
+    }
     if (!net->splitk_bytes || !net->dev_ws) return YOLO_OK;
     const size_t per = net->splitk_bytes / (size_t)net->arenas;
     for (int a = 0; a < net->arenas; ++a)
diff --git a/tensorflow-yolo_amd/csrc/yolo_internal.h b/tensorflow-yolo_amd/csrc/yolo_internal.h
--- a/tensorflow-yolo_amd/csrc/yolo_internal.h
+++ b/tensorflow-yolo_amd/csrc/yolo_internal.h
@@ -86,6 +86,7 @@
 
 constexpr int kTapStreamCUs = 256, kTapStreamPerCu = 2;
 constexpr int kTapStreamGrid = kTapStreamCUs * kTapStreamPerCu;
+constexpr int kTapClaimStride = 32, kTapClaimWords = 9 * kTapClaimStride;
 constexpr int kStemGrid = 512;
 constexpr int kFirstMfmaGrid = 1024;
 constexpr int kAuxBlock = 256, kAuxGrid = 256 * 16;
@@ -119,6 +120,7 @@
     int *pair_cnt;
     uint32_t part_bytes;
     int stream;
+    int *claim;
     int fast_epi;
     int fuse2;
     const void *w2;
@@ -588,6 +590,8 @@
     bool weights_loaded = false;
     unsigned char *wgrad_f16_dev = nullptr;
     size_t wgrad_f16_bytes = 0;
+    int *claim_dev = nullptr;
+    size_t claim_sets = 0;
 };
 
 namespace yolo {
@@ -621,6 +625,7 @@
 struct ConvLaunch {
     int tile, ks, ku, pair, fuse2;
     size_t slab_need;
+    int claim;
 };
 void conv_shape_params(const yolo_net *net, const Kernel &k, int batch, ConvParams &p);
 ConvLaunch resolve_conv(const yolo_net *net, size_t ki, const ConvParams &p, int tile_req, size_t slab_bytes);
```

Measured after the change: 6144 images/sec. 0.965x the previous value.
